# tsnuk/trade-AId-multimodal-transformer

Measured on AMD Instinct MI355X. Metric: training tokens/sec/GPU, 4-modality 1M-row synthetic, at 1/2/4/8 MI355X, higher is better.
Workload: dtype bf16; 1 GPU; C1: 4-modality 1M-row synthetic, d256 L6 T256 (BASELINE configs[1]); model=multimodal-transformer, global_batch=64, seq_len=256, n_embd=256, n_head=8, n_layer=6, modalities=4, parallelism=dp1

## Files before the change

### include/mmt.h

```cpp
#ifndef MMT_H_
#define MMT_H_
#include <stdint.h>

#ifdef __cplusplus
extern "C" {
#endif

#define MMT_MAX_MODALITIES 8

enum mmt_status {
  MMT_OK = 0,
  MMT_ERR_INVALID = -1,
  MMT_ERR_UNSUPPORTED = -2,
  MMT_ERR_HIP = -3,
  MMT_ERR_STATE = -4
};

typedef struct mmt_config {
  int32_t num_modalities;
  int32_t n_embd;
  int32_t n_head;
  int32_t n_layer;
  int32_t block_size;
  int32_t vocab_sizes[MMT_MAX_MODALITIES];
// ... 126 lines not shown
                    int32_t ldb, const float* bias, void* h1, int32_t ldh1, const float* w2, int32_t hh, void* out,
                    int32_t ld_out);
int mmt_op_gemm_wgrad(void* stream, int32_t M, int32_t N, int32_t K, const void* A, int32_t lda, const void* B,
                      int32_t ldb, float* out, int32_t ldc, float alpha, void* slab, int64_t slab_bytes);
int mmt_op_mlp2(void* stream, int32_t M, int32_t C, const void* x, int32_t ldx, const void* w0, int32_t ldw0,
                const float* b0, const void* w2, int32_t ldw2, const float* b2, void* h, int32_t ldh, const float* resid,
                float* out, void* out16, uint32_t drop_key, uint32_t drop_thr, float drop_scale, const float* lnf_gamma,
                const float* lnf_beta, void* lnf_y, float* lnf_mean, float* lnf_rstd);
int mmt_op_mlp2_bwd(void* stream, int32_t M, int32_t C, const void* dy, int32_t lddy, const void* w2, int32_t ldw2,
                    const void* h, int32_t ldh, float alpha, const void* w0, int32_t ldw0, void* dh, int32_t lddh,
                    float* db0, void* dx);
int mmt_op_layernorm_fwd(void* stream, int32_t R, int32_t C, const float* x, const float* gamma, const float* beta,
                         void* y16, float* mean, float* rstd);
int mmt_op_layernorm_bwd(void* stream, int32_t R, int32_t C, const float* x, const float* gamma, const float* mean,
                         const float* rstd, const float* dy, float* dx, void* dx16, float* dgamma, float* dbeta);
int mmt_op_gemm_ln_bwd(void* stream, int32_t M, int32_t N, int32_t K, const void* A, int32_t lda, const void* B,
                       int32_t ldb, float alpha, const float* x, const float* gamma, const float* mean,
                       const float* rstd, float* dx, void* dx16, float* dgamma, float* dbeta, float* dsum,
                       uint32_t drop_key, uint32_t drop_thr, float drop_scale);
int mmt_op_attention_fwd(void* stream, int32_t B, int32_t T, int32_t H, int32_t hs, int32_t nstreams,
                         const void* q, int32_t q_ld, const void* const* k, const void* const* v, int32_t kv_ld,
                         int32_t kv_hstride, void* o, int32_t o_ld, void* const* oj, float* const* lse);
int mmt_op_attention_bwd(void* stream, int32_t B, int32_t T, int32_t H, int32_t hs, int32_t nstreams,
                         const void* q, int32_t q_ld, const void* const* k, const void* const* v, int32_t kv_ld,
                         int32_t kv_hstride, const void* o, int32_t o_ld, const void* const* oj,
                         const float* const* lse, const void* dout, int32_t dout_ld, float* const* dvec, void* dq,
                         int32_t dq_ld, void* const* dk, void* const* dv, int32_t dkv_ld, int32_t dkv_hstride);
int mmt_op_attention_bwd_ws(void* stream, int32_t B, int32_t T, int32_t H, int32_t hs, int32_t nstreams,
                            const void* q, int32_t q_ld, const void* const* k, const void* const* v, int32_t kv_ld,
                            int32_t kv_hstride, const void* o, int32_t o_ld, const void* const* oj,
                            const float* const* lse, const void* dout, int32_t dout_ld, float* const* dvec, void* dq,
                            int32_t dq_ld, void* const* dk, void* const* dv, int32_t dkv_ld, int32_t dkv_hstride,
                            float* dq32, int32_t dq32_ld);
int mmt_op_qkv2_fwd(void* stream, int32_t R, int32_t nblk, int32_t hs, const void* h1, int32_t ld_h1,
                    const float* w2, void* out, int32_t ld_out);
int mmt_op_qkv2_bwd(void* stream, int32_t R, int32_t nblk, int32_t hs, const void* h1, int32_t ld_h1,
                    const float* w2, const void* dout, int32_t ld_out, void* dh1, float* dw2);
int mmt_op_colsum(void* stream, int32_t R, int32_t N, const void* x, int32_t ld, float* out, float alpha);
int mmt_op_ordered_sum(void* stream, int32_t nparts, int32_t n, const float* parts, int64_t ld, float* dst);
int mmt_op_cross_entropy(void* stream, int32_t R, int32_t V, const float* logits, const int64_t* tgt,
                         void* dlogits, int32_t ld_d, float* loss);
int mmt_op_embedding_fwd(void* stream, int32_t B, int32_t T, int32_t C, int32_t V, const int64_t* idx,
                         const float* tok, const float* pos, float* x);
int mmt_op_embedding_bwd(void* stream, int32_t B, int32_t T, int32_t C, int32_t V, const int64_t* idx,
                         const float* dx, float* dtok, float* dpos);
int mmt_op_embedding_bwd_ws(void* stream, int32_t B, int32_t T, int32_t C, int32_t V, const int64_t* idx,
                            const float* dx, float* dtok, float* dpos, float* scratch);
int mmt_emb_set_sort(int on);
int mmt_qkv2_set_coal(int on);
int mmt_set_relu_bits(int on);
int mmt_set_drop_copy_fuse(int on);
int mmt_set_attn_qkv2(int on);
int mmt_mlp2_set_bm(int bm);

int mmt_op_mx_quant(void* stream, int32_t rows, int32_t cols, const float* src, int32_t ld_src, void* dst8,
                    int32_t ld8, void* s8, int32_t lds8);
int mmt_op_gemm_f8(void* stream, int32_t epi, int32_t M, int32_t N, int32_t K, const void* A8, int32_t lda,
                   const void* sa, int32_t lds_a, const void* B8, int32_t ldb, const void* sb, int32_t lds_b,
                   const float* bias, const float* resid, int32_t ldres, float* o32, int32_t ldc, void* o16,
                   int32_t ldo16, void* o8, int32_t ld8, void* s8, int32_t lds8);
int mmt_op_layernorm_fwd_f8(void* stream, int32_t R, int32_t C, const float* x, const float* gamma, const float* beta,
                            void* y16, float* mean, float* rstd, void* y8, int32_t ld8, void* s8, int32_t lds8);

#ifdef __cplusplus
}
#endif
#endif
```

### trade-aid-multimodal-transformer_amd/csrc/mmt_attn.hip

```cpp
#include <stdlib.h>

#include <algorithm>

#include <type_traits>

#include "mmt_common.h"
#include "mmt_kernels.h"

namespace {

__device__ __forceinline__ bf16x8 zero8() {
  const u32x4 z = {0u, 0u, 0u, 0u};
  return __builtin_bit_cast(bf16x8, z);
}

__device__ __forceinline__ bf16x8 ld8(const bf16_t* p, bool ok) {
  if (!ok) return zero8();
  return *reinterpret_cast<const bf16x8*>(p);
}

template <int HS>
struct Geo {
  static constexpr int NKS = (HS + 15) / 16;
  static constexpr int ND = (HS + 31) / 32;
  static constexpr int W = ND * 32;
  static constexpr int RW = W + 8;
  static constexpr int TW = (W == 64) ? 96 : W;
  static constexpr int CH = HS / 8;
};

__device__ __forceinline__ u32x4 tile_chunk(const bf16_t* base, int64_t rowbase, int r0, int row, int col, int T,
                                            int ld) {
  u32x4 v = {0u, 0u, 0u, 0u};
  if (r0 + row < T) v = *reinterpret_cast<const u32x4*>(base + (rowbase + r0 + row) * ld + col);
  return v;
}

__device__ __forceinline__ bf16x8 tr_frag(const bf16_t* lds, int stride, int dt, int s, int lane) {
  const int g = lane >> 4, i = lane & 15;
  const int q = i >> 2, p = i & 3;
  const int col = dt * 32 + 16 * (g & 1) + 4 * p;
  const int kb = 16 * s + 4 * (g >> 1) + q;
  return join4(lds_tr16(lds + kb * stride + col), lds_tr16(lds + (kb + 8) * stride + col));
}

constexpr int SL_SUB = 1152, SL_SLICE = 2 * SL_SUB;
template <int HS>
struct SliceImg {
  static constexpr bool on = HS == 32;
};
__device__ __forceinline__ int sl_off(int row, int chunk) {
  return (row >> 5) * SL_SLICE + (chunk >> 1) * SL_SUB + (row & 31) * 32 + (((chunk & 1) ^ ((row >> 3) & 1)) << 4);
}
__device__ __forceinline__ bf16x8 sl_row(const bf16_t* img, int row0, int r, int s, int h) {
  const int o = (row0 >> 5) * SL_SLICE + s * SL_SUB + r * 32 + ((h ^ ((r >> 3) & 1)) << 4);
  return *reinterpret_cast<const bf16x8*>(reinterpret_cast<const char*>(img) + o);
}
__device__ __forceinline__ bf16x8 sl_tr(const bf16_t* img, int row0, int s, int lane) {
  const int g = lane >> 4, q = (lane >> 2) & 3, p = lane & 3;
  const int L = (g & 1) * SL_SUB + (p & 1) * 8 + (4 * (g >> 1) + q) * 32;
  const char* b = reinterpret_cast<const char*>(img) + (row0 >> 5) * SL_SLICE + 512 * s;
  return join4(lds_tr16(b + L + ((p >> 1) << 4)), lds_tr16(b + L + 256 + (((p >> 1) ^ 1) << 4)));
}

__device__ __forceinline__ bf16x8 acc_frag(const f32x16& a, int s) {
  const u32x4 v = {pack2bf(a[8 * s], a[8 * s + 1]), pack2bf(a[8 * s + 2], a[8 * s + 3]),
                   pack2bf(a[8 * s + 4], a[8 * s + 5]), pack2bf(a[8 * s + 6], a[8 * s + 7])};
  return __builtin_bit_cast(bf16x8, v);
}

__device__ __forceinline__ void zero16(f32x16& a) {
#pragma unroll
  for (int e = 0; e < 16; ++e) a[e] = 0.f;
}

__device__ __forceinline__ float keep_f(float v, int m) { return __int_as_float(__float_as_int(v) & m); }

__device__ __forceinline__ int key_dword(int r) { return 2 * ((r & 3) + 4 * (r >> 3)) + ((r >> 2) & 1); }

}

template <int HS>
struct Chunk {
  static constexpr int ROWS = (HS <= 32) ? 256 : 128;
  static constexpr int HALF = ROWS * Geo<HS>::CH;
  static constexpr int NSTG = 2 * HALF / 256;
};

template <int HS>
struct Stager {
  u32x4 v[Chunk<HS>::NSTG];
  __device__ __forceinline__ void load(const bf16_t* a, int lda, const bf16_t* b, int ldb, int64_t rowbase, int r0,
                                       int T, int tid) {
    constexpr int CH = Geo<HS>::CH, HALF = Chunk<HS>::HALF;
#pragma unroll
    for (int u = 0; u < Chunk<HS>::NSTG; ++u) {
      const int c = tid + 256 * u;
      const bool isb = c >= HALF;
      const int cc = isb ? c - HALF : c;
      v[u] = tile_chunk(isb ? b : a, rowbase, r0, cc / CH, (cc % CH) * 8, T, isb ? ldb : lda);
    }
  }
  __device__ __forceinline__ void store_a(bf16_t* la, int sa, int tid) const {
    constexpr int CH = Geo<HS>::CH, HALF = Chunk<HS>::HALF;
#pragma unroll
    for (int u = 0; u < Chunk<HS>::NSTG; ++u) {
      const int c = tid + 256 * u;
      if (c < HALF) *reinterpret_cast<u32x4*>(la + (c / CH) * sa + (c % CH) * 8) = v[u];
    }
  }
  __device__ __forceinline__ void store(bf16_t* la, int sa, bf16_t* lb, int sb, int tid) const {
    constexpr int CH = Geo<HS>::CH, HALF = Chunk<HS>::HALF;
#pragma unroll
    for (int u = 0; u < Chunk<HS>::NSTG; ++u) {
      const int c = tid + 256 * u;
      const bool isb = c >= HALF;
      const int cc = isb ? c - HALF : c;
      const int row = cc / CH, col = (cc % CH) * 8;
      *reinterpret_cast<u32x4*>(isb ? lb + row * sb + col : la + row * sa + col) = v[u];
    }
  }
  __device__ __forceinline__ void store_slices(bf16_t* la, bf16_t* lb, int tid) const {
    constexpr int CH = Geo<HS>::CH, HALF = Chunk<HS>::HALF;
    static_assert(CH == 4, "slice images hold 32 columns");
#pragma unroll
    for (int u = 0; u < Chunk<HS>::NSTG; ++u) {
      const int c = tid + 256 * u;
      const bool isb = c >= HALF;
      const int cc = isb ? c - HALF : c;
      *reinterpret_cast<u32x4*>(reinterpret_cast<char*>(isb ? lb : la) + sl_off(cc / CH, cc % CH)) = v[u];
    }
  }
};

template <int HS, int KT_ = Chunk<HS>::ROWS / 32>
struct MaskStager {
  static constexpr int KT = KT_;
  static constexpr int N4 = 8 * KT * 8;
  static constexpr int PER = (N4 + 255) / 256;
  static constexpr int DWORDS = 8 * KT * 32;
  u32x4 v[PER];
  __device__ __forceinline__ void load(const uint32_t* base, int bh, int nt, int b0, int c0, bool blk_q, int tid) {
    const int64_t ntri = (int64_t)nt * (nt + 1) / 2;
#pragma unroll
    for (int u = 0; u < PER; ++u) {
      const int c = tid + 256 * u;
      v[u] = u32x4{0u, 0u, 0u, 0u};
      if (N4 % 256 == 0 || c < N4) {
        const int i = c / (KT * 8), k = (c / 8) % KT, p = c % 8;
        const int qt = blk_q ? b0 + i : c0 + k, kt = blk_q ? c0 + k : b0 + i;
        if (qt < nt && kt <= qt)
          v[u] = *reinterpret_cast<const u32x4*>(base + ((int64_t)bh * ntri + qt * (qt + 1) / 2 + kt) * 32 + p * 4);
      }
    }
  }
  __device__ __forceinline__ void store(uint32_t* lds, int tid) const {
#pragma unroll
    for (int u = 0; u < PER; ++u) {
      const int c = tid + 256 * u;
      if (N4 % 256 == 0 || c < N4) *reinterpret_cast<u32x4*>(lds + 4 * c) = v[u];
    }
  }
};

__device__ __forceinline__ float ex2(float x) { return __builtin_amdgcn_exp2f(x); }


constexpr float kLog2e = 1.4426950408889634f;
constexpr float kTau = 8.0f;

#ifndef MMT_FWD_MINB
#define MMT_FWD_MINB(hs) 2
#endif
#ifndef MMT_DQ_MINB
#define MMT_DQ_MINB(hs) 2
#endif
#ifndef MMT_DKDV1_MINB
#define MMT_DKDV1_MINB(hs) ((hs) <= 32 ? 1 : 2)
#endif

__device__ __forceinline__ float xhalf_max(float v) {
  const auto r = __builtin_amdgcn_permlane32_swap(__float_as_uint(v), __float_as_uint(v), false, false);
  float m;
  asm("v_max_f32 %0, %1, %2" : "=v"(m) : "v"(__uint_as_float(r[0])), "v"(__uint_as_float(r[1])));
  return m;
}
__device__ __forceinline__ float xhalf_sum(float v) {
  const auto r = __builtin_amdgcn_permlane32_swap(__float_as_uint(v), __float_as_uint(v), false, false);
  return __uint_as_float(r[0]) + __uint_as_float(r[1]);
}

typedef short s16x2 __attribute__((ext_vector_type(2)));
__device__ __forceinline__ uint32_t keep_spread(uint32_t w16) { return __builtin_amdgcn_perm(0u, w16, 0x0c010c00u); }
__device__ __forceinline__ uint32_t pair_keep(uint32_t w32, int i) {
  s16x2 v = __builtin_bit_cast(s16x2, w32 << (15 - i));
  v = v >> (s16x2){15, 15};
  return __builtin_bit_cast(uint32_t, v);
}
__device__ __forceinline__ int elem_keep(uint32_t w16, int e) {
  return __builtin_amdgcn_sbfe((int)w16, (e & 1) * 8 + (e >> 1), 1);
}

__device__ __forceinline__ bf16x8 acc_frag_keep(const f32x16& a, int s, uint32_t w32) {
  const u32x4 v = {pack2bf(a[8 * s], a[8 * s + 1]) & pair_keep(w32, 4 * s),
                   pack2bf(a[8 * s + 2], a[8 * s + 3]) & pair_keep(w32, 4 * s + 1),
                   pack2bf(a[8 * s + 4], a[8 * s + 5]) & pair_keep(w32, 4 * s + 2),
                   pack2bf(a[8 * s + 6], a[8 * s + 7]) & pair_keep(w32, 4 * s + 3)};
  return __builtin_bit_cast(bf16x8, v);
}

template <int HS>
struct FwdQ {
  bf16x8 qf[Geo<HS>::NKS];
  f32x16 o[Geo<HS>::ND];
  float m, l;
  int tq;
};

template <int HS, bool diag>
__device__ __forceinline__ void fwd_softmax(f32x16& sacc, FwdQ<HS>& q, int k0, float c2, int h) {
  using G = Geo<HS>;
  float tmax = -INFINITY;
  if (diag) {
#pragma unroll
    for (int e = 0; e < 16; ++e) {
      const int key = k0 + (e & 3) + 8 * (e >> 2) + 4 * h;
      if (key > q.tq) sacc[e] = -INFINITY;
    }
  }
#pragma unroll
  for (int e = 0; e < 16; ++e) tmax = fmaxf(tmax, sacc[e]);
  tmax = xhalf_max(tmax) * c2;
  const bool up = tmax > q.m + kTau;
  if (__builtin_amdgcn_ballot_w64(up)) {
    const float alpha = up ? ex2(q.m - tmax) : 1.f;
    q.m = up ? tmax : q.m;
    q.l *= alpha;
#pragma unroll
    for (int dt = 0; dt < G::ND; ++dt)
#pragma unroll
      for (int e = 0; e < 16; ++e) q.o[dt][e] *= alpha;
  }
  const float nm = -q.m;
#pragma unroll
  for (int e = 0; e < 16; ++e) sacc[e] = ex2(__builtin_fmaf(sacc[e], c2, nm));
  float r0 = sacc[0] + sacc[1], r1 = sacc[2] + sacc[3], r2 = sacc[4] + sacc[5], r3 = sacc[6] + sacc[7];
  r0 += sacc[8] + sacc[9]; r1 += sacc[10] + sacc[11]; r2 += sacc[12] + sacc[13]; r3 += sacc[14] + sacc[15];
  q.l += (r0 + r1) + (r2 + r3);
}

template <int HS, int NQ, bool DA, bool DB, bool DROP>
__device__ __forceinline__ void fwd_step(const bf16_t* ks, const bf16_t* vs, int kl, int k0, FwdQ<HS>& a, FwdQ<HS>& b,
                                         const uint32_t* mta, const uint32_t* mtb, float c2, int lane) {
  using G = Geo<HS>;
  const int r = lane & 31, h = lane >> 5;
  const uint32_t wa = DROP ? keep_spread(reinterpret_cast<const uint16_t*>(mta)[lane]) : 0u;
  const uint32_t wb = (DROP && NQ == 2) ? keep_spread(reinterpret_cast<const uint16_t*>(mtb)[lane]) : 0u;
  f32x16 sa, sb;
  zero16(sa);
  if (NQ == 2) zero16(sb);
#pragma unroll
  for (int s = 0; s < G::NKS; ++s) {
    const bf16x8 kf = *reinterpret_cast<const bf16x8*>(ks + (kl + r) * G::RW + 16 * s + 8 * h);
    sa = mfma32(kf, a.qf[s], sa);
    if (NQ == 2) sb = mfma32(kf, b.qf[s], sb);
  }
  bf16x8 vf[2][G::ND];
#pragma unroll
  for (int s = 0; s < 2; ++s)
#pragma unroll
    for (int dt = 0; dt < G::ND; ++dt) vf[s][dt] = tr_frag(vs + kl * G::TW, G::TW, dt, s, lane);
  fwd_softmax<HS, DA>(sa, a, k0, c2, h);
  if (NQ == 2) fwd_softmax<HS, DB>(sb, b, k0, c2, h);
#pragma unroll
  for (int s = 0; s < 2; ++s) {
    const bf16x8 pa = DROP ? acc_frag_keep(sa, s, wa) : acc_frag(sa, s);
#pragma unroll
    for (int dt = 0; dt < G::ND; ++dt) a.o[dt] = mfma32(vf[s][dt], pa, a.o[dt]);
    if (NQ == 2) {
      const bf16x8 pb = DROP ? acc_frag_keep(sb, s, wb) : acc_frag(sb, s);
#pragma unroll
      for (int dt = 0; dt < G::ND; ++dt) b.o[dt] = mfma32(vf[s][dt], pb, b.o[dt]);
    }
  }
}

template <int HS, bool DROP>
__global__ __launch_bounds__(256, MMT_FWD_MINB(HS)) void attn_fwd_kernel(AttnBatch batch, int T, int H, float scale) {
  using G = Geo<HS>;
  constexpr int ROWS = Chunk<HS>::ROWS;
  constexpr int MKT = ROWS / 32;
  constexpr int MDW = 8 * MKT * 32;
  const AttnProblem& P = batch.p[blockIdx.z];
  const int nb = ((T + 31) / 32 + 7) / 8;
  const int tile = xcd_tile(blockIdx.x, gridDim.x);
  const int bh = tile / nb, b = bh / H, head = bh % H;
  const int bx = tile % nb;
  const int tid = threadIdx.x, lane = tid & 63, w = __builtin_amdgcn_readfirstlane(tid >> 6);
  const int r = lane & 31, h = lane >> 5;
  const int nt = (T + 31) / 32;
  const int qt0 = bx * 8;
  const int qmax = min(qt0 + 7, nt - 1);
  const int nch = (min((qmax + 1) * 32, T) + ROWS - 1) / ROWS;
  const int64_t rowbase = (int64_t)b * T;
  const float c2 = scale * kLog2e;
  __shared__ __attribute__((aligned(16))) bf16_t ks[ROWS * G::RW];
  __shared__ __attribute__((aligned(16))) bf16_t vs[ROWS * G::TW];
  using MS = MaskStager<HS>;
  __shared__ __attribute__((aligned(16))) uint32_t msk[DROP ? MDW : 4];
  const int BH = gridDim.x / nb;
  const int64_t lw_off = (int64_t)BH * (nt * (nt + 1) / 2) * 32;
  Stager<HS> st;
  MS mst;
  if (HS % 32 != 0) {
    for (int q = tid; q < ROWS * G::RW; q += 256) if (q % G::RW >= HS) ks[q] = 0;
    for (int q = tid; q < ROWS * G::TW; q += 256) if (q % G::TW >= HS) vs[q] = 0;
  }
  st.load(P.k[0] + head * P.kv_hstride, P.kv_ld, P.v[0] + head * P.kv_hstride, P.kv_ld, rowbase, 0, T, tid);
// ... 613 lines not shown
}
__device__ __forceinline__ void a_bst16(const ai32x4& rsrc, int voff, f32x4 v) {
  asm volatile("buffer_store_dwordx4 %0, %1, %2, 0 offen" : : "v"(v), "v"(voff), "s"(rsrc) : "memory");
}
__device__ __forceinline__ void a_wait_vm(int n) {
  switch (n) {
    case 0: asm volatile("s_waitcnt vmcnt(0)" ::: "memory"); break;
    case 1: asm volatile("s_waitcnt vmcnt(1)" ::: "memory"); break;
    case 2: asm volatile("s_waitcnt vmcnt(2)" ::: "memory"); break;
    case 3: asm volatile("s_waitcnt vmcnt(3)" ::: "memory"); break;
    case 4: asm volatile("s_waitcnt vmcnt(4)" ::: "memory"); break;
    case 5: asm volatile("s_waitcnt vmcnt(5)" ::: "memory"); break;
    case 6: asm volatile("s_waitcnt vmcnt(6)" ::: "memory"); break;
    case 7: asm volatile("s_waitcnt vmcnt(7)" ::: "memory"); break;
    default: asm volatile("s_waitcnt vmcnt(8)" ::: "memory"); break;
  }
}
constexpr int A_OOB = 0x7fffffff;
__device__ __forceinline__ float a_dpp(float v, int ctl) {
  return __builtin_bit_cast(float, ctl == 0xB1 ? __builtin_amdgcn_mov_dpp(__builtin_bit_cast(int, v), 0xB1, 0xF, 0xF, true)
                                  : ctl == 0x4E ? __builtin_amdgcn_mov_dpp(__builtin_bit_cast(int, v), 0x4E, 0xF, 0xF, true)
                                  : ctl == 0x124 ? __builtin_amdgcn_mov_dpp(__builtin_bit_cast(int, v), 0x124, 0xF, 0xF, true)
                                                 : __builtin_amdgcn_mov_dpp(__builtin_bit_cast(int, v), 0x128, 0xF, 0xF, true));
}
__device__ __forceinline__ float a_sum32(float v) {
  v += a_dpp(v, 0xB1);
  v += a_dpp(v, 0x4E);
  v += a_dpp(v, 0x124);
  v += a_dpp(v, 0x128);
  return v + __shfl_xor(v, 16, 64);
}
}

template <bool DROP, bool MS, bool Q2, bool DET = false>
__global__ __launch_bounds__(256, 2) void attn_bwd_fused32(AttnBatch batch, int T, int H, float scale) {
  static_assert(!(MS && Q2), "the stage-2 backward follows the self-attention only");
  static_assert(!DET || Q2, "only the stage-2 epilogue has sums to store");
  constexpr int IMG = 8 * SL_SLICE;
  constexpr int OFF_DO = IMG, OFF_TAB = 2 * IMG;
  constexpr int OFF_DS = OFF_TAB + 2048;
  constexpr int OFF_DQ = OFF_DS + 4 * 2048;
  constexpr int BYTES = OFF_DQ + 8 * 4096;
  static_assert(2 * BYTES <= 160 * 1024, "two workgroups per CU");
  constexpr int EPW = 40;
  static_assert(4 * 32 * EPW * 2 <= 4 * 4096, "epilogue transposes alias one parity of the dQ partials");
  __shared__ __attribute__((aligned(1024))) char lds[BYTES];
  const AttnProblem& P = batch.p[blockIdx.z];
  const int nt = (T + 31) / 32;
  const int bh = xcd_tile(blockIdx.x, gridDim.x);
  const int b = bh / H, head = bh % H;
  const int tid = threadIdx.x, lane = tid & 63, w = __builtin_amdgcn_readfirstlane(tid >> 6);
  const int r = lane & 31, h = lane >> 5;
  const int64_t rowbase = (int64_t)b * T;
  const float c2 = scale * kLog2e;
  const int kts[2] = {w, 7 - w};
  auto in_flight = [&](int qt) { return Q2 ? nt - 2 - qt : nt - 2; };

  const int64_t ntri = (int64_t)nt * (nt + 1) / 2;
  const int ns = MS ? P.nstreams : 1;
  const ai32x4 rdq32 = a_rsrc(MS ? P.dq32 + rowbase * P.dq32_ld + head * 32 : nullptr, MS ? (int64_t)T * P.dq32_ld * 4 : 0);
#pragma unroll 1
  for (int j = 0; j < ns; ++j) {
  const bf16_t* const oj = MS ? P.oj[j] : P.o;
  uint32_t mwq[2][8];
#pragma unroll
  for (int t = 0; t < 2; ++t)
#pragma unroll
    for (int q = 0; q < 8; ++q) {
      mwq[t][q] = 0u;
      if (DROP && q < nt && kts[t] <= q)
        mwq[t][q] = P.dmask[j][((int64_t)bh * ntri + q * (q + 1) / 2 + kts[t]) * 32 + key_dword(r)];
    }
  bf16x8 kf[2][2], vf[2][2];
#pragma unroll
  for (int t = 0; t < 2; ++t) {
    const int tk = kts[t] * 32 + r;
    const bool ok = kts[t] < nt && tk < T;
    const bf16_t* kp = P.k[j] + head * P.kv_hstride + (rowbase + tk) * P.kv_ld;
    const bf16_t* vp = P.v[j] + head * P.kv_hstride + (rowbase + tk) * P.kv_ld;
#pragma unroll
    for (int s = 0; s < 2; ++s) {
      kf[t][s] = ld8(kp + 16 * s + 8 * h, ok);
      vf[t][s] = ld8(vp + 16 * s + 8 * h, ok);
    }
  }
  float lse_t = 0.f;
  u32x4 ov[4], dv4[4];
  {
    const bool ok = tid < T;
    const int64_t t0 = ok ? tid : 0;
    lse_t = P.lse[j][(int64_t)bh * T + t0];
    const bf16_t* orow = oj + (rowbase + t0) * P.o_ld + head * 32;
    const bf16_t* drow = P.dout + (rowbase + t0) * P.dout_ld + head * 32;
#pragma unroll
    for (int c = 0; c < 4; ++c) {
      ov[c] = *reinterpret_cast<const u32x4*>(orow + 8 * c);
      dv4[c] = *reinterpret_cast<const u32x4*>(drow + 8 * c);
    }
  }
  bf16x8 w2t[3][2];
  const MMT_AS1 float* const w2p = Q2 ? sgpr_gptr(P.q2_w2) + head * 512 + (r & 15) + 8 * h * 16 : nullptr;
#pragma unroll
  for (int kd = 0; kd < 3; ++kd)
#pragma unroll
    for (int s = 0; s < 2; ++s) {
      float wv[8];
#pragma unroll
      for (int e = 0; e < 8; ++e) {
        wv[e] = Q2 ? w2p[(kd * H * 32 + 16 * s + e) * 16] : 0.f;
        wv[e] = r < 16 ? wv[e] : 0.f;
      }
      w2t[kd][s] = __builtin_bit_cast(bf16x8, u32x4{pack2bf(wv[0], wv[1]), pack2bf(wv[2], wv[3]), pack2bf(wv[4], wv[5]),
                                                   pack2bf(wv[6], wv[7])});
    }
#pragma unroll
  for (int t = 0; t < 2; ++t) {
#pragma unroll
    for (int q = 0; q < 8; ++q) asm volatile("" : "+v"(mwq[t][q]));
#pragma unroll
    for (int s = 0; s < 2; ++s) {
      asm volatile("" : "+v"(kf[t][s]));
      asm volatile("" : "+v"(vf[t][s]));
    }
  }
#pragma unroll
  for (int c = 0; c < 4; ++c) {
    asm volatile("" : "+v"(ov[c]));
    asm volatile("" : "+v"(dv4[c]));
  }
  asm volatile("" : "+v"(lse_t));
  if (Q2) {
#pragma unroll
    for (int kd = 0; kd < 3; ++kd) {
      asm volatile("" : "+v"(w2t[kd][0]));
      asm volatile("" : "+v"(w2t[kd][1]));
    }
  }
  asm volatile("s_waitcnt vmcnt(0)" ::: "memory");
  if (j == 0) {
    const int op = w & 1, cb = w >> 1;
    const int ld = op ? P.dout_ld : P.q_ld;
    const ai32x4 rs = a_rsrc((op ? P.dout : P.q) + rowbase * ld + head * 32, (int64_t)T * ld * 2);
    const int prow = lane >> 1, pcol = 8 * ((lane & 1) ^ ((prow >> 3) & 1));
    char* dst = lds + op * OFF_DO + cb * SL_SUB;
    for (int sl = 0; sl < nt; ++sl) {
      const int grow = sl * 32 + prow;
      const int voff = grow < T ? (grow * ld + cb * 16 + pcol) * 2 : A_OOB;
      a_dma16(rs, __builtin_amdgcn_readfirstlane(a_lds_u32(dst + sl * SL_SLICE)), voff);
    }
  }
  float* tab = reinterpret_cast<float*>(lds + OFF_TAB);
  {
    float dsum = 0.f;
#pragma unroll
    for (int c = 0; c < 4; ++c)
#pragma unroll
      for (int e = 0; e < 4; ++e) {
        dsum += bf2f(ov[c][e] & 0xffff) * bf2f(dv4[c][e] & 0xffff);
        dsum += bf2f(ov[c][e] >> 16) * bf2f(dv4[c][e] >> 16);
      }
    const bool ok = tid < T;
    tab[tid] = ok ? -lse_t : -INFINITY;
    tab[256 + tid] = ok ? (DROP ? -dsum / P.drop_scale : -dsum) : 0.f;
  }
  char* slot = lds + OFF_DS + w * 2048;
  const int g4 = lane >> 4, qq = (lane >> 2) & 3, p4 = lane & 3;
  const int ra0 = 4 * (g4 >> 1) + qq, ra1 = ra0 + 8;
  const int o_da0 = ra0 * 64 + (((4 * (g4 & 1) + p4) ^ ((ra0 >> 1) & 7)) << 3);
  const int o_da1 = ra1 * 64 + (((4 * (g4 & 1) + p4) ^ ((ra1 >> 1) & 7)) << 3);
  auto sw = [&](int c) { return r * 64 + ((c ^ ((r >> 1) & 7)) << 3); };
  bf16x8 ktf[2][2];
#pragma unroll
  for (int t = 0; t < 2; ++t) {
#pragma unroll
    for (int s = 0; s < 2; ++s) {
      const u32x4 v = __builtin_bit_cast(u32x4, kf[t][s]);
      *reinterpret_cast<u32x2*>(slot + sw(4 * s + 2 * h)) = u32x2{v[0], v[1]};
      *reinterpret_cast<u32x2*>(slot + sw(4 * s + 2 * h + 1)) = u32x2{v[2], v[3]};
    }
    asm volatile("s_waitcnt lgkmcnt(0)" ::: "memory");
#pragma unroll
// ... 290 lines not shown
      asm volatile("s_waitcnt lgkmcnt(0)" ::: "memory");
      bf16_t* dst = (mtx ? P.dv[j] : P.dk[j]) + head * P.dkv_hstride;
#pragma unroll
      for (int i = 0; i < 2; ++i) {
        const int row = i * 16 + (lane >> 2), d0 = (lane & 3) * 8;
        const u32x4 v = *reinterpret_cast<const u32x4*>(et + row * EPW + d0);
        if (k0 + row < T) *reinterpret_cast<u32x4*>(dst + (rowbase + k0 + row) * P.dkv_ld + d0) = v;
      }
    }
  }
  }
  }
}

static int g_attn_ring = mmt_env_int("MMT_ATTN_RING", 15 | 64);
extern "C" int mmt_attn_set_ring(int v) {
  const int old = g_attn_ring;
  g_attn_ring = v;
  return old;
}

static bool ring64_fits(const AttnBatch& bt, int T) {
  const int64_t lim = (int64_t)1 << 31;
  const int64_t nt = (T + 31) / 32, ntri = nt * (nt + 1) / 2;
  if (ntri * 128 >= lim) return false;
  for (int g = 0; g < bt.count; ++g) {
    const AttnProblem& P = bt.p[g];
    if ((int64_t)T * P.q_ld * 2 >= lim || (int64_t)T * P.dout_ld * 2 >= lim || (int64_t)T * P.kv_ld * 2 >= lim)
      return false;
  }
  return true;
}

static bool fused32_ok(const AttnBatch& bt, int T, int ns) {
  if (!(g_attn_ring & 64) || T > 256 || bt.count < 1) return false;
  const bool q2 = bt.p[0].q2_w2 != nullptr;
  if (q2 && ns > 1) return false;
  bool ok = true;
  for (int g = 0; g < bt.count; ++g) {
    const AttnProblem& P = bt.p[g];
    ok = ok && !(P.q_ld & 7) && !(P.dout_ld & 7) && !((uintptr_t)P.q & 15) && !((uintptr_t)P.dout & 15) &&
         !(P.kv_ld & 7) && !(P.kv_hstride & 7) && (int64_t)T * std::max(P.q_ld, P.dout_ld) * 2 < ((int64_t)1 << 31);
    if (ns > 1)
      ok = ok && (g_attn_ring & 128) && P.dq32 && !(P.dq32_ld & 3) && !((uintptr_t)P.dq32 & 15) &&
           (int64_t)T * P.dq32_ld * 4 < ((int64_t)1 << 31);
    if (ns == 1 && !q2) ok = ok && !(P.dq_ld & 3) && !((uintptr_t)P.dq & 7);
    if ((P.q2_w2 != nullptr) != q2) return false;
    if (q2)
      ok = ok && P.q2_h1 && P.q2_dh1 && P.q2_dw2 && P.q2_db1 && !(P.q2_ld & 7) && !((uintptr_t)P.q2_h1 & 15) &&
           !((uintptr_t)P.q2_dh1 & 7);
  }
  return ok;
}

bool mmt_attn_bwd_fuses_qkv2(const AttnBatch& bt, int T, int hs) {
  if (hs != 32 || bt.count < 1) return false;
  for (int g = 0; g < bt.count; ++g)
    if (bt.p[g].nstreams != 1) return false;
  AttnBatch t = bt;
  for (int g = 0; g < t.count; ++g) {
    AttnProblem& P = t.p[g];
    P.q2_w2 = reinterpret_cast<const float*>(16); P.q2_h1 = reinterpret_cast<const bf16_t*>(16);
    P.q2_dh1 = reinterpret_cast<bf16_t*>(16); P.q2_dw2 = reinterpret_cast<float*>(16); P.q2_db1 = P.q2_dw2;
    P.q2_ld = 8;
  }
  return fused32_ok(t, T, 1);
}

int64_t mmt_attn_q2_det_floats(int count, int B, int H) { return (int64_t)count * B * 3 * H * (512 + 16); }

template <int HS>
static hipError_t attn_launch(const AttnBatch& bt, int B, int T, int H, float scale, bool bwd, hipStream_t s) {
  const int nb = ((T + 31) / 32 + 7) / 8;
  if (!bwd) {
    bool drop = false;
    for (int g = 0; g < bt.count; ++g) drop = drop || bt.p[g].drop_thr != 0;
    if (HS == 64 && (g_attn_ring & 8) && ring64_fits(bt, T)) return mmt_attn_fwd_ring64(bt, B, T, H, scale, drop, s);
    const dim3 grid(nb * B * H, 1, bt.count);
    if (drop) hipLaunchKernelGGL((attn_fwd_kernel<HS, true>), grid, dim3(256), 0, s, bt, T, H, scale);
    else hipLaunchKernelGGL((attn_fwd_kernel<HS, false>), grid, dim3(256), 0, s, bt, T, H, scale);
  } else {
    const int ns = bt.p[0].nstreams;
    bool drop = false;
    for (int g = 0; g < bt.count; ++g) drop = drop || bt.p[g].drop_thr != 0;
    for (int g = 0; g < bt.count; ++g)
      if (bt.p[g].q2_w2 && (HS != 32 || !fused32_ok(bt, T, ns))) return hipErrorInvalidValue;
    const bool ring = HS == 64 && ring64_fits(bt, T);
    if (ring && (g_attn_ring & 32) && T <= 512 && ns == 1) return mmt_attn_bwd_fused64(bt, B, T, H, scale, drop, s);
    if (HS == 32 && fused32_ok(bt, T, ns)) {
      const dim3 grid(B * H, 1, bt.count);
      const bool q2 = bt.p[0].q2_w2 != nullptr;
      if (ns > 1) {
        if (drop) hipLaunchKernelGGL((attn_bwd_fused32<true, true, false>), grid, dim3(256), 0, s, bt, T, H, scale);
        else hipLaunchKernelGGL((attn_bwd_fused32<false, true, false>), grid, dim3(256), 0, s, bt, T, H, scale);
      } else if (q2 && bt.det.base) {
        AttnBatch d = bt;
        d.det.stride = mmt_attn_q2_det_floats(1, B, H);
        DetLaunch L;
        hipError_t e = L.begin(d.det, d.count, d.det.stride, s);
        if (e != hipSuccess) return e;
        if (drop) hipLaunchKernelGGL((attn_bwd_fused32<true, false, true, true>), grid, dim3(256), 0, s, d, T, H, scale);
        else hipLaunchKernelGGL((attn_bwd_fused32<false, false, true, true>), grid, dim3(256), 0, s, d, T, H, scale);
        e = hipGetLastError();
        if (e != hipSuccess) return e;
        for (int g = 0; g < d.count; ++g) {
          L.seg(g, d.det.stride, 0, d.p[g].q2_dw2, B, 3 * H * 512);
          L.seg(g, d.det.stride, (int64_t)B * 3 * H * 512, d.p[g].q2_db1, B, 3 * H * 16);
        }
        return L.finish();
      } else if (q2) {
        if (drop) hipLaunchKernelGGL((attn_bwd_fused32<true, false, true>), grid, dim3(256), 0, s, bt, T, H, scale);
        else hipLaunchKernelGGL((attn_bwd_fused32<false, false, true>), grid, dim3(256), 0, s, bt, T, H, scale);
      } else {
        if (drop) hipLaunchKernelGGL((attn_bwd_fused32<true, false, false>), grid, dim3(256), 0, s, bt, T, H, scale);
        else hipLaunchKernelGGL((attn_bwd_fused32<false, false, false>), grid, dim3(256), 0, s, bt, T, H, scale);
      }
      return hipGetLastError();
    }
    if (ring && (g_attn_ring & 2)) {
      const hipError_t e = mmt_attn_bwd_dq_ring64(bt, B, T, H, scale, drop, s);
      if (e != hipSuccess) return e;
    } else if (drop) hipLaunchKernelGGL((attn_bwd_dq_kernel<HS, true>), dim3(nb * B * H, 1, bt.count), dim3(256), 0, s, bt, T, H, scale);
    else hipLaunchKernelGGL((attn_bwd_dq_kernel<HS, false>), dim3(nb * B * H, 1, bt.count), dim3(256), 0, s, bt, T, H, scale);
    if (ring && (g_attn_ring & 1)) return mmt_attn_bwd_dkdv_ring64(bt, B, T, H, scale, drop, g_attn_ring, s);
    if (drop)
      hipLaunchKernelGGL((attn_bwd_dkdv1_kernel<HS, true>), dim3(nb * B * H * ns, 1, bt.count), dim3(256), 0, s, bt, T, H,
                         scale);
    else
      hipLaunchKernelGGL((attn_bwd_dkdv1_kernel<HS, false>), dim3(nb * B * H * ns, 1, bt.count), dim3(256), 0, s, bt, T,
                         H, scale);
  }
  return hipGetLastError();
}

static hipError_t attn_dispatch(const AttnBatch& b, int B, int T, int H, int hs, float scale, bool bwd,
                                hipStream_t s) {
  if (b.count == 0 || B == 0 || T == 0) return hipSuccess;
  for (int g = 0; g < b.count; ++g) {
    if (b.p[g].nstreams < 1 || b.p[g].nstreams > MMT_MAX_STREAMS) return hipErrorInvalidValue;
    for (int j = 0; j < b.p[g].nstreams && b.p[g].nstreams > 1; ++j)
      if (!b.p[g].oj[j]) return hipErrorInvalidValue;
    if (b.p[g].drop_thr)
      for (int j = 0; j < b.p[g].nstreams; ++j)
        if (!b.p[g].dmask[j]) return hipErrorInvalidValue;
// ... 143 lines not shown
```

### trade-aid-multimodal-transformer_amd/csrc/mmt_engine.hip

```cpp
#include <hip/hip_runtime.h>

#include <algorithm>
#include <cmath>
#include <cstdio>
#include <cstdlib>
#include <cstring>
#include <string>
#include <vector>

#include "mmt.h"
#include "mmt_common.h"
#include "mmt_kernels.h"

namespace {

constexpr int MAXM = MMT_MAX_MODALITIES;

inline int64_t rup(int64_t x, int64_t a) { return (x + a - 1) / a * a; }
inline int r8(int x) { return (int)rup(x < 1 ? 1 : x, 8); }

struct Mat {
  int64_t off = -1;
  int rows = 0, cols = 0;
  int64_t pk = 0;
// ... 50 lines not shown
  size_t dvec[MAXM][MAXM];
  size_t dkv[2][MAXM][MAXM];
  size_t celoss[MAXM];
  const void* gh1_pad_ws = nullptr;
  size_t eperm[MAXM];
  size_t det = 0;
  int64_t det_floats = 0;
  struct Dec {
    size_t x0, a16, mean, rstd, h1, qkv, o16, p1, f, x2h, d16, qc, oc, pc, lnf16, hh;
    size_t kv[MAXM];
  } dec[MAXM];
  std::vector<size_t> dec_x;
};

}

static int g_relu_bits = mmt_env_int("MMT_RELU_BITS", 0);
extern "C" int mmt_set_relu_bits(int on) {
  const int old = g_relu_bits;
  g_relu_bits = on;
  return old;
}
static int g_drop_copy_fuse = mmt_env_int("MMT_DROP_COPY_FUSE", 1);
extern "C" int mmt_set_drop_copy_fuse(int on) {
  const int old = g_drop_copy_fuse;
  g_drop_copy_fuse = on;
  return old;
}

static int g_attn_qkv2 = mmt_env_int("MMT_ATTN_QKV2", 1);
extern "C" int mmt_set_attn_qkv2(int on) {
  const int old = g_attn_qkv2;
  g_attn_qkv2 = on;
  return old;
}

struct mmt_ctx {
  mmt_config cfg;
  int M, C, H, L, T, hs, hh;
  int V[MAXM];
  bool any_cross = false;
  int ncross = 0;
  std::vector<TensorInfo> tensors;
  std::vector<LM> lm;
  PostM post[MAXM];
  int64_t pos_off = 0;
  int64_t nparams = 0, nactive = 0;
  int64_t emb_begin = 0, emb_end = 0, post_begin = 0, post_end = 0;
  std::vector<int64_t> layer_begin, layer_end;
  std::vector<PackSeg> segs;
  std::vector<int> tasks;
  std::vector<MxSeg> mxsegs;
  int64_t pack8_bytes = 0;
  int mx_units = 0;
  MxSeg* d_mxsegs = nullptr;
  int tables_device = -1;
  bool fp8 = false;
  bool relu_bits = false;
  hipEvent_t emb_ev = nullptr;
  bool emb_sorted = false;
  int64_t pack_elems = 0;
  PackSeg* d_segs = nullptr;
  int* d_tasks = nullptr;
  Plan plan;
  int last_B = -1;
  bool fwd_ready = false;
  bool cache_ready = false;
  bool last_training = false;
  uint64_t step_counter = 0;
  uint64_t next_seed = 0;
  bool next_seed_set = false;
  uint64_t fwd_seed = 0;
  bool fwd_drop = false;
  const int64_t* last_idx[MAXM] = {};
  std::string err;
  struct ProbeEv {
    hipEvent_t a, b;
    int pat;
    double flops, bytes;
  };
  std::vector<std::string> probe_pats;
  bool probe_on = true;
  std::vector<ProbeEv> probe_events;
  std::vector<std::pair<hipEvent_t, hipEvent_t>> probe_pool;
  int ldv[MAXM], ldvh[MAXM];
  hipStream_t side = nullptr;
  int side_device = -1;
  bool side_off = false;
  bool side_off_req = false;
  bool defer_join = false;
  hipEvent_t stage_ev[2] = {nullptr, nullptr};
  std::vector<hipEvent_t> evpool;
  size_t evnext = 0;
  int d16 = 0;
  bool det = false;
  bool det_req = false;
  bool grad_accum = false;
};

namespace {

thread_local std::string g_create_err;

int fail(mmt_ctx* c, int code, const std::string& msg) {
  if (c) c->err = msg;
  return code;
}

#define HIPCHK(ctx, expr)                                                                             \
  do {                                                                                                \
    hipError_t e_ = (expr);                                                                           \
    if (e_ != hipSuccess) return fail(ctx, MMT_ERR_HIP, std::string(#expr) + ": " + hipGetErrorString(e_)); \
  } while (0)

struct Builder {
  mmt_ctx* c;
  int64_t cur = 0;
  int64_t alloc(int64_t n) {
    const int64_t o = cur;
    cur += rup(n > 0 ? n : 0, 16);
    return o;
  }
  void tensor(const std::string& name, int64_t off, int nd, int64_t s0, int64_t s1, int kind) {
    TensorInfo t;
    t.name = name; t.off = off; t.nd = nd; t.shape[0] = s0; t.shape[1] = s1; t.kind = kind;
    c->tensors.push_back(t);
  }
  Mat mat(const std::string& name, int rows, int cols, bool emit = true) {
    Mat m;
    m.rows = rows; m.cols = cols;
// ... 305 lines not shown
      if (std::strncmp(what, p.c_str(), p.size() - 1) == 0) return (int)i;
    } else if (p == what) {
      return (int)i;
    }
  }
  return -1;
}
int probe_match(const mmt_ctx* c, const char* what) {
  std::string w(what);
  size_t b = 0;
  while (true) {
    const size_t e = w.find('+', b);
    const int r = probe_match_one(c, w.substr(b, e == std::string::npos ? std::string::npos : e - b).c_str());
    if (r >= 0 || e == std::string::npos) return r;
    b = e + 1;
  }
}

void gemm_cost(const GemmBatch& b, int epi, double* fl, double* by) {
  for (int g = 0; g < b.count; ++g) {
    const GemmProblem& P = b.p[g];
    const double M = P.M, N = P.N, K = P.K;
    *fl += 2.0 * M * N * K;
    double x = (M * K + N * K) * 2.0;
    if (P.bias) x += N * 4.0;
    const bool f32_out = epi == EPI_BIAS_RESID_F32 || epi == EPI_STORE_F32 || epi == EPI_ACC_F32;
    x += M * N * (f32_out ? 4.0 : 2.0);
    if (epi == EPI_BIAS_RESID_F32) x += M * N * 4.0 + (P.o16 ? M * N * 2.0 : 0.0);
    if (epi == EPI_ACC_F32) x += M * N * 4.0;
    if (epi == EPI_DTANH_BF16 || epi == EPI_DRELU_BF16) x += (epi == EPI_DRELU_BF16 && P.mask8) ? M * N / 8.0 : M * N * 2.0;
    if (epi == EPI_BIAS_RELU_BF16 && P.mask8) x += M * N / 8.0;
    if (P.o8) x += M * N * (1.0 + 1.0 / 32.0);
    if (epi == EPI_LN_BWD_F32) x += M * N * 8.0 + (P.o16 ? M * N * 2.0 : 0.0) + M * 8.0;
    *by += x;
  }
}

void wgrad_cost(const GemmBatch& b, double* fl, double* by) {
  for (int g = 0; g < b.count; ++g) {
    const GemmProblem& P = b.p[g];
    const double M = P.M, N = P.N, K = P.K;
    *fl += 2.0 * M * N * K;
    *by += (M * K + N * K) * 2.0 + M * N * 4.0;
  }
}

void attn_cost(const AttnBatch& ab, int B, int T, int H, int hs, bool bwd, bool drop, double* fl, double* by) {
  const double C = (double)H * hs, rows = (double)B * T, bhT = (double)B * H * T;
  const double mask = drop ? (double)mmt_attn_mask_dwords(B, H, T) * 4.0 : 0.0;
  for (int g = 0; g < ab.count; ++g) {
    const double ns = ab.p[g].nstreams;
    const double f = 2.0 * (double)B * H * ns * (double)T * T * hs;
    *fl += bwd ? 2.5 * f : f;
    double x = rows * C * 2.0 * (2.0 + 2.0 * ns) + ns * (bhT * 4.0 + mask);
    if (ns > 1) x += ns * rows * C * 2.0;
    if (bwd) x += rows * C * 2.0 * (2.0 + 2.0 * ns) + ns * bhT * 4.0;
    if (bwd && ab.p[g].q2_w2) {
      const double hh = hs / 2;
      x += -rows * C * 2.0 * 3.0 + 2.0 * rows * 3.0 * H * hh * 2.0 + 3.0 * H * hs * hh * 4.0 * 2.0;
      *fl += 2.0 * 2.0 * rows * 3.0 * C * hh;
    }
    *by += x;
  }
}

GemmProblem gp_f8(const uint8_t* X8, int ldx, const uint8_t* Xs, int ldxs, const uint8_t* w8, const Mat& W, int R) {
  GemmProblem g{};
  g.A = reinterpret_cast<const bf16_t*>(X8); g.lda = ldx; g.sa = Xs; g.lds_a = ldxs;
  g.B = reinterpret_cast<const bf16_t*>(w8 + W.pk8); g.ldb = W.ld8; g.sb = w8 + W.ps8; g.lds_b = W.lds8;
  g.M = R; g.N = W.rows; g.K = W.cols; g.alpha = 1.f;
  return g;
}

enum DropSite { DS_SA_PROB = 0, DS_SA_PROJ = 1, DS_FFN = 2, DS_CA_PROB = 3, DS_CA_PROJ = 4 };

struct Runner {
  mmt_ctx* c;
  hipStream_t s;
  void* ws;
  const float* params;
  const bf16_t* wpk;
  int B, R;
  int rc = MMT_OK;
  bool drop = false;
  uint64_t seed = 0;

  template <class Pm>
  void set_drop(Pm& p, int l, int i, int site) const {
    if (!drop) { p.drop_key = 0; p.drop_thr = 0; p.drop_scale = 1.f; return; }
    const double pr = c->cfg.dropout;
    p.drop_key = mmt_hash((uint32_t)seed, (uint32_t)(seed >> 32), (uint32_t)((l * MAXM + i) * 8 + site));
    p.drop_thr = (uint32_t)std::min(65535.0, std::max(1.0, std::floor(pr * 65536.0)));
    p.drop_scale = (float)(1.0 / (1.0 - pr));
// ... 284 lines not shown
      eb.p[i].idx = idx[i]; eb.p[i].tok = r.P(c->post[i].tok); eb.p[i].pos = r.P(c->pos_off);
      eb.p[i].x = r.W<float>(p.xemb[i]); eb.p[i].V = c->V[i];
    }
    r.ok(mmt_launch_embed_fwd(eb, B, T, C, r.s), "embed_fwd");
  }
  std::vector<const float*> xin(M);
  for (int i = 0; i < M; ++i) xin[i] = r.W<float>(p.xemb[i]);
  static const int ln_fuse = mmt_env_int("MMT_LN_FUSE", 1) != 0 ? mmt_env_int("MMT_LN_FUSE_FWD", 1) : 0;
  const bool fuse_fwd = ln_fuse && !f8 && (C == 256 || (C == 512 && ln_fuse == 2));
  std::vector<char> ln1_done(M, 0), lnf_done(M, 0);
  for (int l = 0; l < c->L && r.rc == MMT_OK; ++l) {
    const LM* x = &c->lm[(size_t)l * M];
    const ActLM* a = &p.act[(size_t)l * M];
    if (r.drop && l == 0) gen_masks(0);
    LnBatch lb{}; lb.count = 0;
    for (int i = 0; i < M; ++i) {
      if (ln1_done[i]) continue;
      LnProblem& q = lb.p[lb.count++];
      q.x = xin[i]; q.gamma = r.P(x[i].ln1w); q.beta = r.P(x[i].ln1b);
      q.y = r.W<bf16_t>(a[i].a); q.mean = r.W<float>(a[i].mean1); q.rstd = r.W<float>(a[i].rstd1);
      ln8(q, a[i].a8, a[i].as8);
    }
    if (lb.count) r.ok(mmt_launch_ln_fwd(lb, R, C, r.s), "ln1_fwd");
    std::fill(ln1_done.begin(), ln1_done.end(), 0);
    lb.count = M;
    GemmBatch g{}; g.count = M;
    static const bool qkv2_fuse = mmt_env_int("MMT_QKV2_FUSE", 1) != 0;
    for (int i = 0; i < M; ++i) {
      g.p[i] = f8 ? gp_f8(r.W<uint8_t>(a[i].a8), C, r.W<uint8_t>(a[i].as8), ldsC, w8, x[i].W1, R)
                  : gp_fwd(r.W<bf16_t>(a[i].a), C, wpk, x[i].W1, R);
      g.p[i].bias = r.P(x[i].b1); g.p[i].o16 = r.W<bf16_t>(a[i].h1); g.p[i].ldo16 = ldh1;
    }
    const bool fuse_qkv2 = qkv2_fuse && (c->hh == 16 || c->hh == 32) && !f8 && !mmt_gemm_wgrad_big(g);
    for (int i = 0; i < M; ++i) {
      if (fuse_qkv2) {
        g.p[i].qkv2_w2 = r.P(x[i].w2); g.p[i].qkv2_out = r.W<bf16_t>(a[i].qkv);
        g.p[i].qkv2_ld = 3 * C; g.p[i].qkv2_hh = c->hh;
      }
    }
    if (f8) r.gemm8(g, EPI_BIAS_TANH_BF16, "qkv1");
    else r.gemm(g, true, true, EPI_BIAS_TANH_BF16, 1, "qkv1");
    for (int i = 0; i < M; ++i) g.p[i].qkv2_out = nullptr;
    if (!fuse_qkv2) {
      Qkv2Batch qb{}; qb.count = M;
      for (int i = 0; i < M; ++i) {
        qb.p[i].h1 = r.W<bf16_t>(a[i].h1); qb.p[i].w2 = r.P(x[i].w2); qb.p[i].out = r.W<bf16_t>(a[i].qkv);
      }
      r.ok(mmt_launch_qkv2_fwd(qb, R, 3 * H, hs, ldh1, 3 * C, r.s), "qkv2_fwd");
    }
    AttnBatch ab{}; ab.count = M;
    for (int i = 0; i < M; ++i) {
      AttnProblem& q = ab.p[i];
      bf16_t* qkv = r.W<bf16_t>(a[i].qkv);
      q.q = qkv + C; q.q_ld = 3 * C; q.k[0] = qkv; q.v[0] = qkv + 2 * C; q.kv_ld = 3 * C; q.kv_hstride = hs;
      q.o = r.W<bf16_t>(a[i].o); q.o_ld = C; q.lse[0] = r.W<float>(a[i].lse); q.nstreams = 1;
      r.set_drop(q, l, i, DS_SA_PROB);
      if (r.drop) q.dmask[0] = r.W<uint32_t>(a[i].dm);
    }
    if (r.drop && (l <= 1 || mask_ahead)) {
      r.join();
      r.gemm_hint = 0;
      if (mask_ahead) {
        if (ahead_mode == 1 && l + 1 < c->L) gen_masks(l + 1);
      } else if (l == 0) {
        for (int ll = 1; ll < c->L; ++ll) gen_masks(ll);
        if (mask_t2) r.gemm_hint = 1;
      }
    }
    r.attn(ab, false, scale, "attn_fwd");
    if (r.drop && ahead_mode == 2 && l + 1 < c->L) {
      gen_masks(l + 1);
      if (mask_t2) r.gemm_hint = 1;
    }
    static const bool ln2_env = mmt_env_int("MMT_LN2_FUSE", 1) != 0;
    const bool ln2_fuse = ln2_env && !f8;
    bool ln2_done = false;
    {
      GemmProblem pg1[MAXM], pg2[MAXM];
      for (int i = 0; i < M; ++i) {
        GemmProblem& g1 = pg1[i];
        g1 = gp_fwd(r.W<bf16_t>(a[i].o), C, wpk, x[i].P0, R);
        g1.bias = r.P(x[i].bp0); g1.o16 = r.W<bf16_t>(a[i].p1); g1.ldo16 = ldp;
        GemmProblem& g2 = pg2[i];
        g2 = gp_fwd(r.W<bf16_t>(a[i].p1), ldp, wpk, x[i].P2, R);
        g2.bias = r.P(x[i].bp2); g2.resid = xin[i]; g2.ldres = C;
        g2.o32 = r.W<float>(a[i].x1); g2.ldc = C;
        r.set_drop(g2, l, i, DS_SA_PROJ);
        if (ln2_fuse) {
          g2.lnf_gamma = r.P(x[i].ln2w); g2.lnf_beta = r.P(x[i].ln2b); g2.lnf_y = r.W<bf16_t>(a[i].c);
          g2.lnf_mean = r.W<float>(a[i].mean2); g2.lnf_rstd = r.W<float>(a[i].rstd2);
// ... 594 lines not shown
      const bf16_t* g = r.W<bf16_t>(p.gp[par][i]);
      pdx0[i] = gp_dx(g, ldp, wpk, x[i].P0, R);
      pdx0[i].o16 = r.W<bf16_t>(p.gdo[i]); pdx0[i].ldo16 = C;
    }
    const bool fused = r.mlp2(dx.p, pdx0, M, "proj_dx", true);
    if (!fused) r.gemm(dx, true, false, EPI_DTANH_BF16, 1, "proj2_dx");
    for (int i = 0; i < M; ++i) {
      const bf16_t* g = r.W<bf16_t>(p.gp[par][i]);
      dw.p[i] = gp_dw(g, ldp, r.W<bf16_t>(a[i].o), C, grads, x[i].P0, R);
      dx.p[i] = pdx0[i];
    }
    r.dwgemm(dw, "proj0_dw");
    if (!fused) r.gemm(dx, true, false, EPI_STORE_BF16, 1, "proj0_dx");
  }
  r.flush();
  AttnBatch ab{}; ab.count = M;
  for (int i = 0; i < M; ++i) {
    AttnProblem& q = ab.p[i];
    bf16_t* qkv = r.W<bf16_t>(a[i].qkv);
    bf16_t* gq = r.W<bf16_t>(p.gqkv[i]);
    q.q = qkv + C; q.q_ld = 3 * C; q.k[0] = qkv; q.v[0] = qkv + 2 * C; q.kv_ld = 3 * C; q.kv_hstride = hs;
    q.o = r.W<bf16_t>(a[i].o); q.o_ld = C; q.lse[0] = r.W<float>(a[i].lse); q.nstreams = 1;
    q.dout = r.W<bf16_t>(p.gdo[i]); q.dout_ld = C; q.dvec[0] = r.W<float>(p.dvec[i][0]);
    q.dq = gq + C; q.dq_ld = 3 * C; q.dk[0] = gq; q.dv[0] = gq + 2 * C; q.dkv_ld = 3 * C; q.dkv_hstride = hs;
    r.set_drop(q, l, i, DS_SA_PROB);
    if (r.drop) q.dmask[0] = r.W<uint32_t>(a[i].dm);
  }
  const bool q2 = g_attn_qkv2 && mmt_attn_bwd_fuses_qkv2(ab, T, hs);
  if (q2)
    for (int i = 0; i < M; ++i) {
      AttnProblem& q = ab.p[i];
      q.q2_h1 = r.W<bf16_t>(a[i].h1); q.q2_dh1 = r.W<bf16_t>(p.gh1[par][i]); q.q2_ld = ldh1;
      q.q2_w2 = r.P(x[i].w2); q.q2_dw2 = grads + x[i].w2; q.q2_db1 = grads + x[i].b1;
    }
  Qkv2Batch qb{}; qb.count = M;
  for (int i = 0; i < M; ++i) {
    qb.p[i].h1 = r.W<bf16_t>(a[i].h1); qb.p[i].w2 = r.P(x[i].w2); qb.p[i].dout = r.W<bf16_t>(p.gqkv[i]);
    qb.p[i].dh1 = r.W<bf16_t>(p.gh1[par][i]); qb.p[i].dw2 = grads + x[i].w2;
    qb.p[i].db1 = grads + x[i].b1;
  }
  if (p.gh1_pad_ws != r.ws && ldh1 > 3 * H * c->hh) {
    const size_t cols = 3 * (size_t)H * c->hh;
    for (int k = 0; k < 2; ++k)
      for (int i = 0; i < M; ++i)
        r.ok(hipMemset2DAsync(r.W<bf16_t>(p.gh1[k][i]) + cols, (size_t)ldh1 * 2, 0, ((size_t)ldh1 - cols) * 2, (size_t)R, r.s),
             "gh1 pad");
    p.gh1_pad_ws = r.ws;
  }
  r.attn(ab, true, scale, "attn_bwd");
  r.det_arm(qb);
  if (!q2) r.ok(mmt_launch_qkv2_bwd(qb, R, 3 * H, hs, ldh1, 3 * C, r.s), "qkv2_bwd");
  for (int i = 0; i < M; ++i) {
    const bf16_t* g = r.W<bf16_t>(p.gh1[par][i]);
    dw.p[i] = gp_dw(g, ldh1, r.W<bf16_t>(a[i].a), C, grads, x[i].W1, R);
    dx.p[i] = gp_dx(g, ldh1, wpk, x[i].W1, R);
    dx.p[i].o32 = r.W<float>(p.dln[i]); dx.p[i].ldc = C;
  }
  r.dwgemm(dw, "qkv1_dw");
  r.flush();
  d16_advance(c);
  for (int i = 0; i < M; ++i) {
    lb.p[i].x = xin[i]; lb.p[i].gamma = r.P(x[i].ln1w); lb.p[i].mean = r.W<float>(a[i].mean1);
    lb.p[i].rstd = r.W<float>(a[i].rstd1); lb.p[i].dy = r.W<float>(p.dln[i]); lb.p[i].dx = r.W<float>(p.dres[i]);
    lb.p[i].dgamma = grads + x[i].ln1w; lb.p[i].dbeta = grads + x[i].ln1b;
    set_dres16_consumer(c, r, lb.p[i], i, l - 1, grads);
  }
  r.gemm_ln_bwd(dx, lb, R, C, "qkv1_dx", "ln1_bwd");
// ... 132 lines not shown
    std::strncpy(name, t.name.c_str(), cap - 1);
    name[cap - 1] = 0;
  }
  if (off) *off = t.off;
  if (nd) *nd = t.nd;
  if (shape) { shape[0] = t.shape[0]; shape[1] = t.shape[1]; }
  if (kind) *kind = t.kind;
  return MMT_OK;
}

int64_t mmt_loss_flag_offset(mmt_ctx* c, int32_t batch) {
  if (!c || batch < 1) return -1;
  return (int64_t)flag_offset(c);
}

int64_t mmt_workspace_bytes(mmt_ctx* c, int32_t batch) {
  if (!c || batch < 1) return -1;
  make_plan(c, batch);
  c->last_B = batch;
  c->fwd_ready = false;
  c->cache_ready = false;
  return (int64_t)c->plan.total;
}

int mmt_forward(mmt_ctx* c, void* stream, int32_t batch, const int64_t* const* idx, const int64_t* const* tgt,
                const float* params, float* const* logits, float* losses, void* workspace, int32_t training) {
  if (!c) return MMT_ERR_INVALID;
  if (batch < 1 || !idx || !params || !logits || !workspace) return fail(c, MMT_ERR_INVALID, "mmt_forward: null argument");
  if (c->plan.B != batch) make_plan(c, batch);
  int rc = ensure_device_tables(c);
  if (rc) return rc;
  c->side_off = c->side_off_req;
  c->det = c->det_req;
  Runner r{c, (hipStream_t)stream, workspace, params, nullptr, batch, batch * c->T};
  r.drop = training && c->cfg.dropout > 0.f;
  if (r.drop) {
    if (c->next_seed_set) r.seed = c->next_seed;
    else r.seed = ((uint64_t)mmt_hash((uint32_t)c->cfg.seed, (uint32_t)(c->cfg.seed >> 32), (uint32_t)c->step_counter) << 32) |
                  mmt_hash((uint32_t)(c->cfg.seed >> 32), (uint32_t)c->cfg.seed, (uint32_t)(c->step_counter >> 32) ^ 0xA5A5A5A5u);
    c->next_seed_set = false;
    ++c->step_counter;
  }
  if (r.drop) ensure_side(c);
  c->fwd_drop = r.drop;
  c->fwd_seed = r.seed;
  c->fwd_ready = false;
  for (int i = 0; i < c->M; ++i) c->last_idx[i] = idx[i];
  rc = run_forward(c, r, idx, tgt, logits, losses);
  if (rc == MMT_OK && tgt) c->fwd_ready = true;
  c->cache_ready = rc == MMT_OK;
  c->last_training = training != 0;
  return rc;
}

int mmt_decode_step(mmt_ctx* c, void* stream, int32_t batch, int32_t pos, const int64_t* const* idx,
                    const float* params, float* const* logits, void* workspace) {
  if (!c) return MMT_ERR_INVALID;
  if (!idx || !params || !logits || !workspace) return fail(c, MMT_ERR_INVALID, "mmt_decode_step: null argument");
  if (c->plan.B != batch || !c->cache_ready)
    return fail(c, MMT_ERR_STATE, "mmt_decode_step: run mmt_forward (prefill) on this batch and workspace first");
  if (c->fwd_drop)
    return fail(c, MMT_ERR_STATE, "mmt_decode_step: the prefill forward sampled dropout (training mode); decode "
                                  "has eval semantics: run the prefill with training = 0");
  if (c->fp8)
    return fail(c, MMT_ERR_STATE, "mmt_decode_step: precision fp8 prefills with MX-fp8 GEMMs the bf16 decode "
                                  "would not reproduce: re-run mmt_forward per token");
  if (pos < 1 || pos >= c->T) return fail(c, MMT_ERR_INVALID, "mmt_decode_step: position outside 1..block_size-1");
  Runner r{c, (hipStream_t)stream, workspace, params, nullptr, batch, batch};
  return run_decode(c, r, pos, idx, logits);
}

int32_t mmt_backward_stage_count(const mmt_ctx* c) { return c ? c->L + 2 : 0; }

int mmt_backward_stage_range(const mmt_ctx* c, int32_t stage, int64_t* begin, int64_t* end) {
  if (!c || stage < 0 || stage > c->L + 1) return MMT_ERR_INVALID;
  int64_t b, e;
  if (stage == 0) { b = c->post_begin; e = c->post_end; }
  else if (stage == c->L + 1) { b = c->emb_begin; e = c->emb_end; }
  else { const int l = c->L - stage; b = c->layer_begin[l]; e = c->layer_end[l]; }
  if (begin) *begin = b;
  if (end) *end = e;
  return MMT_OK;
}

}

extern "C" {

int mmt_backward_stage(mmt_ctx* c, void* stream, int32_t stage, const float* loss_grads, const float* params,
                       float* grads, void* workspace) {
  if (!c) return MMT_ERR_INVALID;
  if (!c->fwd_ready) return fail(c, MMT_ERR_STATE, "mmt_backward: no forward with targets to differentiate");
  if (stage < 0 || stage > c->L + 1) return fail(c, MMT_ERR_INVALID, "bad backward stage");
// ... 195 lines not shown
```

### trade-aid-multimodal-transformer_amd/csrc/mmt_gemm.hip

```cpp
#include "mmt_common.h"
#include "mmt_kernels.h"

#include <stdlib.h>

#include <algorithm>
#include <type_traits>

#include "mmt_gemm_dev.h"


static int g_gemm_variant = -1;

static int g_gemm_big_variant_rt = 0;
static int g_force_big_rt = 0;
static int g_gemm8_rt = -1;
static int g_gemm_variant_dw = 0;
extern "C" int mmt_gemm_set_variant(int v) {
  if (v < 0) {
    g_gemm_variant = -1; g_gemm_variant_dw = 0; g_gemm_big_variant_rt = 0; g_force_big_rt = 0; g_gemm8_rt = -1;
    return 0;
  }
  if ((v & 15) > 6 || ((v >> 4) & 15) > 6 || ((v >> 8) & 15) > 3) return -1;
  g_gemm_variant = v & 15;
  g_gemm_variant_dw = (v >> 4) & 15;
// ... 146 lines not shown
  }
  if (tile >= ntiles) return;
  GEMM_STAMP(0);
  GEMM_STAMP(5);
  GEMM_STAMP(6);
  const int tm = tile / tiles_n, tn = tile % tiles_n;
  const int m0 = tm * GBM, n0 = tn * GBN;
  const int ksteps = (K + BK - 1) / BK;
  const int kper = (ksteps + nsplit - 1) / nsplit;
  const int ks0 = split * kper;
  const int ks1 = min(ksteps, ks0 + kper);
  if (EPI == EPI_ATOMIC_F32 && ks0 >= ks1) return;

  constexpr int EPI_ROWS = (GBN >= 512 || (GBM == 128 && GBN == 256)) ? 32 : (GBM == 128 && MINB == 1) ? 128 : 64;
  constexpr int RING = ST * STAGE_BYTES, CTILE = EPI_ROWS * (GBN + 4) * 4;
  constexpr int LDS_MAIN = RING > CTILE ? RING : CTILE;
  constexpr int LDS_W2 = (SWAP && EPI == EPI_BIAS_TANH_BF16 && TL::NW == 4 && TL::BN == 128) ? QKV2_W2_LDS : 0;
  __shared__ __attribute__((aligned(1024))) char lds[LDS_MAIN + LDS_W2];

  const int tid = threadIdx.x;
  const int lane = tid & 63;
  const int wave = __builtin_amdgcn_readfirstlane(tid >> 6);
  const int wm = wave / TL::WN, wn = wave % TL::WN;

  f32x16 acc[AI][AJ];
#pragma unroll
  for (int i = 0; i < AI; ++i)
#pragma unroll
    for (int j = 0; j < AJ; ++j)
#pragma unroll
      for (int e = 0; e < 16; ++e) acc[i][j][e] = 0.0f;
  if constexpr (SWAP && EPI == EPI_BIAS_TANH_BF16 && TL::NW == 4 && TL::BN == 128) {
    if (P.qkv2_out) qkv2_stage_w2<TL>(P, lds + LDS_MAIN, n0, tid);
    if (P.qkv2_out && P.bias) {
      const float ia = 1.0f / P.alpha;
      const int hh = (tid & 63) >> 5;
#pragma unroll
      for (int i = 0; i < AI; ++i)
#pragma unroll
        for (int e = 0; e < 16; ++e) {
          const int n = n0 + wn * TL::TN * 32 + 32 * i + (e & 3) + 8 * (e >> 2) + 4 * hh;
          const float bv = n < N ? P.bias[n] * ia : 0.0f;
#pragma unroll
          for (int j = 0; j < AJ; ++j) acc[i][j][e] = bv;
        }
    }
  }

  if (ks0 < ks1) {
    const int lda = __builtin_amdgcn_readfirstlane(P.lda), ldb = __builtin_amdgcn_readfirstlane(P.ldb);
    auto sgpr_ptr = [](const bf16_t* q) {
      const uint64_t v = (uint64_t)(uintptr_t)q;
      const uint32_t lo = __builtin_amdgcn_readfirstlane((uint32_t)v), hi = __builtin_amdgcn_readfirstlane((uint32_t)(v >> 32));
      return (const bf16_t*)(uintptr_t)(((uint64_t)hi << 32) | lo);
    };
    const bf16_t* const Ap = sgpr_ptr(P.A);
    const bf16_t* const Bp = sgpr_ptr(P.B);
    const i32x4 ra_kc = A_KC ? op_rsrc<true>(Ap, lda, M, K, m0, 0) : i32x4{0, 0, 0, 0};
    const i32x4 rb_kc = B_KC ? op_rsrc<true>(Bp, ldb, N, K, n0, 0) : i32x4{0, 0, 0, 0};
    auto ra = [&](int k0) { return A_KC ? ra_kc : op_rsrc<false>(Ap, lda, M, K, m0, k0); };
    auto rb = [&](int k0) { return B_KC ? rb_kc : op_rsrc<false>(Bp, ldb, N, K, n0, k0); };
    const int nk = ks1 - ks0;
    auto step = [&](int tt, auto UC) {
      constexpr int U = decltype(UC)::value;
      wait_vm(PIECES * min(ST - 2, nk - 1 - tt));
      asm volatile("s_waitcnt lgkmcnt(0)" ::: "memory");
      __builtin_amdgcn_s_barrier();
// ... 22 lines not shown
          }
      }
    };
#pragma unroll
    for (int t = 0; t < ST - 1; ++t)
      if (t < nk) {
        char* st = lds + t * STAGE_BYTES;
        const int k0 = (ks0 + t) * BK;
        issue_tile<BK, A_KC, GBM, NW>(ra(k0), st, lda, M, K, m0, k0, wave, lane);
        issue_tile<BK, B_KC, GBN, NW>(rb(k0), st + IMG_A, ldb, N, K, n0, k0, wave, lane);
      }
    GEMM_STAMP(1);
    int t = 0;
    for (; t + ST <= nk; t += ST) {
      step(t, std::integral_constant<int, 0>{});
      step(t + 1, std::integral_constant<int, 1>{});
      if constexpr (ST > 2) step(t + 2, std::integral_constant<int, (ST > 2 ? 2 : 0)>{});
      if constexpr (ST > 3) step(t + 3, std::integral_constant<int, (ST > 3 ? 3 : 0)>{});
    }
    if (t < nk) step(t, std::integral_constant<int, 0>{});
    if (ST > 2 && t + 1 < nk) step(t + 1, std::integral_constant<int, 1>{});
    if constexpr (ST > 3) { if (t + 2 < nk) step(t + 2, std::integral_constant<int, (ST > 3 ? 2 : 0)>{}); }
  }

  GEMM_STAMP(3);
  float alpha = P.alpha;
  if (P.alpha_ptr) alpha *= *P.alpha_ptr;
  float* o32 = P.o32 + (P.split_stride ? (int64_t)split * P.split_stride : (int64_t)0);
  const int h = lane >> 5, r = lane & 31;
  if constexpr (SWAP && EPI == EPI_BIAS_TANH_BF16 && TL::NW == 4 && TL::BN == 128) {
    if (P.qkv2_out) {
      qkv2_fused<TL>(P, acc, lds, lds + LDS_MAIN, alpha, m0, n0, lane, wave);
      epilogue_swap<TL, EPI, EPI_ROWS, true>(P, acc, lds, o32, alpha, m0, n0, tid, lane, wave, det_of(batch, prob));
    } else {
      epilogue_swap<TL, EPI, EPI_ROWS>(P, acc, lds, o32, alpha, m0, n0, tid, lane, wave, det_of(batch, prob));
    }
  } else if constexpr (SWAP) {
    epilogue_swap<TL, EPI, EPI_ROWS>(P, acc, lds, o32, alpha, m0, n0, tid, lane, wave, det_of(batch, prob));
  } else {
#pragma unroll
    for (int i = 0; i < TM; ++i)
#pragma unroll
      for (int j = 0; j < TN; ++j) {
        const int n = n0 + wn * TN * 32 + 32 * j + r;
        if (n >= N) continue;
#pragma unroll
        for (int e = 0; e < 16; ++e) {
          const int m = m0 + wm * TM * 32 + 32 * i + (e & 3) + 8 * (e >> 2) + 4 * h;
          if (m < M) epi_scalar<EPI>(P, o32, alpha, m, n, acc[i][j][e]);
        }
      }
  }
  GEMM_STAMP(4);
}

template <int ROWS, int NW>
__device__ __forceinline__ void issue_tile_f8(const i32x4& rsrc, char* img, int ld, int rows_total, int K, int r0,
                                              int k0, int wave, int lane) {
  constexpr int PPW = ROWS * 128 / 1024 / NW;
#pragma unroll
  for (int u = 0; u < PPW; ++u) {
    const int i = wave * PPW + u;
    const int row = 8 * i + lane / 8;
    const int chunk = kc_swz<64>(lane % 8, row);
    const int grow = r0 + row, gk = k0 + chunk * 16;
    const int voff = (grow < rows_total && gk < K) ? row * ld + gk : 0x7fffffff;
// ... 222 lines not shown
  }
  const int mt = max_tiles<TileS>(b, nullptr);
  if (mt == 0) return hipSuccess;
  dim3 grid(mt, EPI == EPI_ATOMIC_F32 ? auto_splits<TileS>(b, splits) : std::max(1, splits), b.count);
  constexpr bool occ3 = EPI == EPI_STORE_BF16 || EPI == EPI_BIAS_TANH_BF16 || EPI == EPI_BIAS_RELU_BF16;
  static const int env_dw = mmt_env_int("MMT_GEMM_DW_VARIANT", -1);
  const int var = EPI == EPI_ATOMIC_F32 ? g_gemm_variant_dw
                  : (!A_KC && !B_KC && env_dw >= 0) ? env_dw
                  : (g_gemm_variant >= 0 ? g_gemm_variant : occ3 ? MMT_OCC3_VARIANT : MMT_DEF_VARIANT);
  switch (var) {
    case 1: launch_v<TileS, 32, 2, A_KC, B_KC, SWAP, EPI>(b, grid, s); break;
    case 2: launch_v<TileS, 32, 3, A_KC, B_KC, SWAP, EPI>(b, grid, s); break;
    case 3: launch_v<TileS, 32, 4, A_KC, B_KC, SWAP, EPI>(b, grid, s); break;
    case 4: launch_v<TileS, 64, 3, A_KC, B_KC, SWAP, EPI>(b, grid, s); break;
    case 5: launch_v<TileS, 32, 3, A_KC, B_KC, SWAP, EPI, 3>(b, grid, s); break;
    case 6: launch_v<TileS, 32, 2, A_KC, B_KC, SWAP, EPI, 3>(b, grid, s); break;
    default: launch_v<TileS, 64, 2, A_KC, B_KC, SWAP, EPI>(b, grid, s); break;
  }
  return hipGetLastError();
}

static int g_big_mode = mmt_env_int("MMT_GEMM_BIG", 1);

static int g_gemm8_kmin = mmt_env_int("MMT_GEMM8_KMIN", 512);
static int g_gemm8_min_tiles = mmt_env_int("MMT_GEMM8_MIN_TILES", 1024);
static bool use_big(const GemmBatch& b) {
  if (!g_big_mode || b.count == 0) return false;
  bool big = true, qkv2 = false;
  int tiles = 0;
  for (int g = 0; g < b.count; ++g) {
    const GemmProblem& P = b.p[g];
    if (P.M < TileL::BM || P.N < TileL::BN) return false;
    if (P.K < g_big_kmin && !g_force_big_rt) big = false;
    qkv2 = qkv2 || P.qkv2_out != nullptr;
    tiles += ((P.M + 255) / 256) * ((P.N + 255) / 256);
  }
  if (big) return true;
  if (!gemm8_on() || qkv2 || tiles < g_gemm8_min_tiles) return false;
  for (int g = 0; g < b.count; ++g)
    if (b.p[g].K < g_gemm8_kmin) return false;
  return true;
}

static bool qkv2_ok(const GemmProblem& P, int epi, bool fwd) {
  if (!P.qkv2_out) return true;
  return epi == EPI_BIAS_TANH_BF16 && fwd && (P.qkv2_hh == 16 || P.qkv2_hh == 32) && P.N % P.qkv2_hh == 0 &&
         !P.alpha_ptr && P.alpha != 0.0f &&
         P.qkv2_w2 && !(P.qkv2_ld & 7) && !((uintptr_t)P.qkv2_out & 15) && !((uintptr_t)P.qkv2_w2 & 15);
}

static bool gemm_span_ok(const GemmBatch& b) {
  for (int g = 0; g < b.count; ++g) {
    const GemmProblem& P = b.p[g];
    if (P.M < 0 || P.N < 0 || P.K < 0 || P.lda < 0 || P.ldb < 0) return false;
    if ((int64_t)(512 + 1) * std::max(P.lda, P.ldb) * 2 + (int64_t)P.K * 2 >= ((int64_t)1 << 31)) return false;
  }
  return true;
}

static int64_t gemm_det_stride(const GemmBatch& b, bool ln) {
  int64_t st = 0;
  for (int g = 0; g < b.count; ++g) {
    const int64_t nrt = (b.p[g].M + MMT_DET_GEMM_ROWS - 1) / MMT_DET_GEMM_ROWS;
    st = std::max(st, (ln ? 3 : 1) * nrt * (int64_t)b.p[g].N);
  }
  return (st + 3) & ~(int64_t)3;
}
int64_t mmt_gemm_det_floats(int count, int M, int N, bool ln) {
  GemmBatch b{};
  b.count = 1; b.p[0].M = M; b.p[0].N = N;
  return count * gemm_det_stride(b, ln);
}
template <class F>
static hipError_t gemm_det_run(const GemmBatch& b, bool ln, hipStream_t s, F run) {
  bool any = false;
  for (int g = 0; g < b.count; ++g) any = any || b.p[g].dbias || (ln && (b.p[g].ln_dgamma || b.p[g].ln_dbeta));
  GemmBatch d = b;
  if (!any) {
// ... 4 lines not shown
  DetLaunch L;
  hipError_t e = L.begin(d.det, b.count, d.det.stride, s);
  if (e != hipSuccess) return e;
  e = run(d);
  if (e != hipSuccess) return e;
  for (int g = 0; g < b.count; ++g) {
    const GemmProblem& P = b.p[g];
    const int nrt = (P.M + MMT_DET_GEMM_ROWS - 1) / MMT_DET_GEMM_ROWS;
    const int64_t slot = (int64_t)nrt * P.N;
    L.seg(g, d.det.stride, 0, P.dbias, nrt, P.N);
    if (ln) {
      L.seg(g, d.det.stride, slot, P.ln_dgamma, nrt, P.N);
      L.seg(g, d.det.stride, 2 * slot, P.ln_dbeta, nrt, P.N);
    }
  }
  return L.finish();
}

static hipError_t launch_gemm_any(const GemmBatch& b, bool a_kc, bool b_kc, int epi, int splits, hipStream_t s);
hipError_t mmt_launch_gemm(const GemmBatch& b, bool a_kc, bool b_kc, int epi, int splits, hipStream_t s) {
  if (!b.det.base) return launch_gemm_any(b, a_kc, b_kc, epi, splits, s);
  return gemm_det_run(b, false, s, [&](const GemmBatch& d) { return launch_gemm_any(d, a_kc, b_kc, epi, splits, s); });
}

static hipError_t launch_gemm_any(const GemmBatch& b, bool a_kc, bool b_kc, int epi, int splits, hipStream_t s) {
  if (!gemm_span_ok(b)) return hipErrorInvalidValue;
  for (int g = 0; g < b.count; ++g) {
    const GemmProblem& P = b.p[g];
    if ((P.lda & 7) || (P.ldb & 7) || (((uintptr_t)P.A | (uintptr_t)P.B) & 15)) return hipErrorInvalidValue;
    if (!qkv2_ok(P, epi, a_kc && b_kc)) return hipErrorInvalidValue;
  }
  const bool big = use_big(b);
  for (int g = 0; g < b.count; ++g)
    if (big && b.p[g].qkv2_out) return hipErrorInvalidValue;
  if (a_kc && b_kc) {
    switch (epi) {
      case EPI_STORE_BF16: return launch_t<true, true, true, EPI_STORE_BF16>(b, 1, big, s);
      case EPI_BIAS_TANH_BF16: return launch_t<true, true, true, EPI_BIAS_TANH_BF16>(b, 1, big, s);
      case EPI_BIAS_RELU_BF16: return launch_t<true, true, true, EPI_BIAS_RELU_BF16>(b, 1, big, s);
      case EPI_BIAS_RESID_F32: return launch_t<true, true, true, EPI_BIAS_RESID_F32>(b, 1, big, s);
      case EPI_STORE_F32: return launch_t<true, true, true, EPI_STORE_F32>(b, 1, big, s);
      case EPI_ACC_F32: return launch_t<true, true, true, EPI_ACC_F32>(b, 1, big, s);
      default: break;
    }
  } else if (a_kc && !b_kc) {
    switch (epi) {
      case EPI_STORE_BF16: return launch_t<true, false, true, EPI_STORE_BF16>(b, 1, big, s);
      case EPI_DTANH_BF16: return launch_t<true, false, true, EPI_DTANH_BF16>(b, 1, big, s);
      case EPI_DRELU_BF16: return launch_t<true, false, true, EPI_DRELU_BF16>(b, 1, big, s);
      case EPI_STORE_F32: return launch_t<true, false, true, EPI_STORE_F32>(b, 1, big, s);
      case EPI_ACC_F32: return launch_t<true, false, true, EPI_ACC_F32>(b, 1, big, s);
      default: break;
    }
  } else if (!a_kc && !b_kc) {
    switch (epi) {
      case EPI_ATOMIC_F32: return launch_t<false, false, false, EPI_ATOMIC_F32>(b, splits, big, s);
      case EPI_STORE_F32: return launch_t<false, false, true, EPI_STORE_F32>(b, splits, big, s);
      case EPI_ACC_F32: return launch_t<false, false, true, EPI_ACC_F32>(b, 1, big, s);
      default: break;
    }
  } else {
    switch (epi) {
      case EPI_ATOMIC_F32: return launch_t<false, true, false, EPI_ATOMIC_F32>(b, splits, big, s);
      case EPI_STORE_F32: return launch_t<false, true, true, EPI_STORE_F32>(b, 1, big, s);
      default: break;
    }
  }
// ... 164 lines not shown
    if (gemm8_ln_on()) return mmt_launch_gemm8(b, EPI_LN_BWD_F32, true, false, dim3(mt, 1, b.count), s);
    launch_v<TileL, 64, 2, true, false, true, EPI_LN_BWD_F32>(b, dim3(mt, 1, b.count), s);
  }
  return hipGetLastError();
}

template <class TL, int EPI>
static hipError_t launch_f8(const GemmBatch& b, hipStream_t s) {
  int mt = 0;
  for (int g = 0; g < b.count; ++g)
    mt = std::max(mt, ((b.p[g].M + TL::BM - 1) / TL::BM) * ((b.p[g].N + TL::BN - 1) / TL::BN));
  if (mt == 0) return hipSuccess;
  hipLaunchKernelGGL((gemm_f8_kernel<TL, EPI>), dim3(mt, 1, b.count), dim3(TL::NT), 0, s, b);
  return hipGetLastError();
}

template <int EPI>
static hipError_t launch_f8_tile(const GemmBatch& b, hipStream_t s) {
  bool big = g_big_mode != 0 && b.tile_hint != 1;
  for (int g = 0; g < b.count; ++g)
    if (b.p[g].M < TileL::BM || b.p[g].N < TileL::BN || b.p[g].K < g_big_kmin) big = false;
  return big ? launch_f8<TileL, EPI>(b, s) : launch_f8<TileS, EPI>(b, s);
}

hipError_t mmt_launch_gemm_f8(const GemmBatch& b, int epi, hipStream_t s) {
  if (b.count == 0) return hipSuccess;
  if (!gemm_span_ok(b)) return hipErrorInvalidValue;
  for (int g = 0; g < b.count; ++g) {
    const GemmProblem& P = b.p[g];
    if ((P.K & 31) || (P.lda & 15) || (P.ldb & 15) || (((uintptr_t)P.A | (uintptr_t)P.B) & 15) || (P.lds_a & 3) ||
        (P.lds_b & 3) || (((uintptr_t)P.sa | (uintptr_t)P.sb) & 3) || P.lds_a * 32 < P.K || P.lds_b * 32 < P.K)
      return hipErrorInvalidValue;
    if (P.o8 && ((P.N & 31) || (P.ld8 & 7) || ((uintptr_t)P.o8 & 7))) return hipErrorInvalidValue;
    if (P.qkv2_out) return hipErrorInvalidValue;
  }
  switch (epi) {
    case EPI_STORE_BF16: return launch_f8_tile<EPI_STORE_BF16>(b, s);
    case EPI_BIAS_TANH_BF16: return launch_f8_tile<EPI_BIAS_TANH_BF16>(b, s);
    case EPI_BIAS_RELU_BF16: return launch_f8_tile<EPI_BIAS_RELU_BF16>(b, s);
    case EPI_BIAS_RESID_F32: return launch_f8_tile<EPI_BIAS_RESID_F32>(b, s);
    case EPI_STORE_F32: return launch_f8_tile<EPI_STORE_F32>(b, s);
    default: return hipErrorInvalidValue;
  }
}
```

### trade-aid-multimodal-transformer_amd/csrc/mmt_kernels.h

```cpp
#pragma once
#include <hip/hip_runtime.h>
#include <stdint.h>
#include "mmt_det.h"

#ifndef MMT_MAX_GROUP
#define MMT_MAX_GROUP 8
#endif
typedef uint16_t bf16_t;

enum MmtEpi {
  EPI_STORE_BF16 = 0,
  EPI_BIAS_TANH_BF16,
  EPI_BIAS_RELU_BF16,
  EPI_BIAS_RESID_F32,
  EPI_STORE_F32,
  EPI_DTANH_BF16,
  EPI_DRELU_BF16,
  EPI_ACC_F32,
  EPI_ATOMIC_F32,
  EPI_LN_BWD_F32,
  EPI_COUNT
};

struct GemmProblem {
// ... 1 lines not shown
  const bf16_t* B;
  const float* bias;
  const bf16_t* aux;
  const float* resid;
  float* o32;
  bf16_t* o16;
  const float* alpha_ptr;
  float alpha;
  int M, N, K;
  int lda, ldb, ldc, ldaux, ldres, ldo16;
  uint32_t drop_key, drop_thr;
  float drop_scale;
  float* dbias;
  int64_t split_stride;
  const uint8_t* sa;
  const uint8_t* sb;
  int lds_a, lds_b;
  uint8_t* o8;
  uint8_t* s8;
  int ld8, lds8;
  const float* ln_gamma;
  const float* ln_mean;
  const float* ln_rstd;
  float* ln_dgamma;
  float* ln_dbeta;
  const float* lnf_gamma;
  const float* lnf_beta;
  bf16_t* lnf_y;
  float* lnf_mean;
  float* lnf_rstd;
  const float* qkv2_w2;
  bf16_t* qkv2_out;
  int qkv2_ld, qkv2_hh;
  uint8_t* mask8;
  int ldm8;
};

struct GemmBatch {
  GemmProblem p[MMT_MAX_GROUP];
  int count;
  int xcd_plane;
  int tile_hint;
  int dw_blocks;
  unsigned long long* stamps;
  DetScratch det;
};

hipError_t mmt_launch_gemm(const GemmBatch& b, bool a_kc, bool b_kc, int epi, int splits, hipStream_t s);
bool mmt_gemm_ln_bwd_ok(const GemmBatch& b);
bool mmt_gemm_resid_ln_ok(const GemmBatch& b);
hipError_t mmt_launch_gemm_resid_ln(const GemmBatch& b, hipStream_t s);
hipError_t mmt_launch_gemm_ln_bwd(const GemmBatch& b, hipStream_t s);
hipError_t mmt_launch_gemm_wgrad(const GemmBatch& b, float* slab, int64_t slab_bytes, hipStream_t s);

#define MMT_MLP2_GROUP 4
struct Mlp2Batch {
  GemmProblem g1[MMT_MLP2_GROUP];
  GemmProblem g2[MMT_MLP2_GROUP];
  int count;
  DetScratch det;
};
static_assert(sizeof(Mlp2Batch) <= 4096, "Mlp2Batch is a kernel argument");
bool mmt_mlp2_ok(const Mlp2Batch& b);
hipError_t mmt_launch_mlp2(const Mlp2Batch& b, hipStream_t s);
bool mmt_mlp2_bwd_ok(const Mlp2Batch& b);
hipError_t mmt_launch_mlp2_bwd(const Mlp2Batch& b, hipStream_t s);
// ... 21 lines not shown
};
struct LnBatch {
  LnProblem p[MMT_MAX_GROUP];
  int count;
  float* zero_f; int nzero_f;
  int* zero_i; int nzero_i;
  DetScratch det;
};
hipError_t mmt_launch_ln_fwd(const LnBatch& b, int R, int C, hipStream_t s);
hipError_t mmt_launch_ln_bwd(const LnBatch& b, int R, int C, hipStream_t s);

#define MMT_MAX_STREAMS 8
struct AttnProblem {
  const bf16_t* q; int q_ld;
  const bf16_t* k[MMT_MAX_STREAMS];
  const bf16_t* v[MMT_MAX_STREAMS];
  int kv_ld, kv_hstride;
  bf16_t* o; int o_ld;
  bf16_t* oj[MMT_MAX_STREAMS];
  float* lse[MMT_MAX_STREAMS];
  const bf16_t* dout; int dout_ld;
  float* dvec[MMT_MAX_STREAMS];
  bf16_t* dq; int dq_ld;
  float* dq32; int dq32_ld;
  const bf16_t* q2_h1; bf16_t* q2_dh1; int q2_ld;
  const float* q2_w2; float* q2_dw2; float* q2_db1;
  bf16_t* dk[MMT_MAX_STREAMS];
  bf16_t* dv[MMT_MAX_STREAMS];
  int dkv_ld, dkv_hstride;
  int nstreams;
  uint32_t drop_key, drop_thr;
  float drop_scale;
  uint32_t* dmask[MMT_MAX_STREAMS];
};
inline int64_t mmt_attn_mask_tiles(int B, int H, int T) {
  const int64_t nt = (T + 31) / 32;
  return (int64_t)B * H * (nt * (nt + 1) / 2);
}
inline int64_t mmt_attn_mask_dwords(int B, int H, int T) { return 2 * 32 * mmt_attn_mask_tiles(B, H, T); }
struct AttnBatch {
  AttnProblem p[MMT_MAX_GROUP];
  int count;
  DetScratch det;
};
hipError_t mmt_launch_attn_fwd(const AttnBatch& b, int B, int T, int H, int hs, float scale, hipStream_t s);
hipError_t mmt_launch_attn_bwd(const AttnBatch& b, int B, int T, int H, int hs, float scale, hipStream_t s);
bool mmt_attn_bwd_fuses_qkv2(const AttnBatch& b, int T, int hs);
hipError_t mmt_attn_bwd_dkdv_ring64(const AttnBatch& b, int B, int T, int H, float scale, bool drop, int variant,
                                    hipStream_t s);
hipError_t mmt_attn_bwd_dq_ring64(const AttnBatch& b, int B, int T, int H, float scale, bool drop, hipStream_t s);
hipError_t mmt_attn_fwd_ring64(const AttnBatch& b, int B, int T, int H, float scale, bool drop, hipStream_t s);
hipError_t mmt_attn_bwd_fused64(const AttnBatch& b, int B, int T, int H, float scale, bool drop, hipStream_t s);
hipError_t mmt_launch_attn_mask(const AttnBatch& b, int B, int T, int H, hipStream_t s);

struct DecodeAttnProblem {
  const bf16_t* q; int q_ld;
  const bf16_t* k[MMT_MAX_STREAMS];
  const bf16_t* v[MMT_MAX_STREAMS];
  int kv_ld, kv_hstride;
  bf16_t* o; int o_ld;
  int nstreams;
};
struct DecodeAttnBatch { DecodeAttnProblem p[MMT_MAX_GROUP]; int count; };
hipError_t mmt_launch_attn_decode(const DecodeAttnBatch& b, int B, int t, int T, int H, int hs, float scale,
                                  hipStream_t s);

struct Qkv2Problem {
  const bf16_t* h1;
  const float* w2;
  bf16_t* out;
  const bf16_t* dout;
  bf16_t* dh1;
  float* dw2;
  float* db1;
};
struct Qkv2Batch { Qkv2Problem p[MMT_MAX_GROUP]; int count; DetScratch det; };
hipError_t mmt_launch_qkv2_fwd(const Qkv2Batch& b, int R, int nblk, int hs, int ld_h1, int ld_out, hipStream_t s);
hipError_t mmt_launch_qkv2_bwd(const Qkv2Batch& b, int R, int nblk, int hs, int ld_h1, int ld_out, hipStream_t s);

struct EmbProblem {
  const int64_t* idx;
  const float* tok;
  const float* pos;
  float* x;
// ... 81 lines not shown
```

### trade-aid-multimodal-transformer_amd/csrc/mmt_ops.hip

```cpp
#include <hip/hip_runtime.h>

#include "mmt.h"
#include "mmt_kernels.h"

static int st(hipError_t e) { return e == hipSuccess ? MMT_OK : MMT_ERR_HIP; }

extern "C" {

int mmt_op_gemm(void* stream, int32_t a_kc, int32_t b_kc, int32_t epi, int32_t splits, int32_t M, int32_t N,
                int32_t K, const void* A, int32_t lda, const void* B, int32_t ldb, const float* bias, const void* aux,
                int32_t ldaux, const float* resid, int32_t ldres, float* o32, int32_t ldc, void* o16, int32_t ldo16,
                float alpha) {
  if (epi < 0 || epi >= EPI_COUNT || M < 0 || N < 0 || K < 0) return MMT_ERR_INVALID;
  if ((lda & 7) || (ldb & 7)) return MMT_ERR_INVALID;
  GemmBatch b{};
  b.count = 1;
  GemmProblem& p = b.p[0];
  p.A = (const bf16_t*)A; p.lda = lda; p.B = (const bf16_t*)B; p.ldb = ldb; p.bias = bias;
  p.aux = (const bf16_t*)aux; p.ldaux = ldaux; p.resid = resid; p.ldres = ldres; p.o32 = o32; p.ldc = ldc;
  p.o16 = (bf16_t*)o16; p.ldo16 = ldo16; p.alpha = alpha; p.M = M; p.N = N; p.K = K;
  const hipError_t e = mmt_launch_gemm(b, a_kc != 0, b_kc != 0, epi, splits, (hipStream_t)stream);
  if (e == hipErrorInvalidValue) return MMT_ERR_UNSUPPORTED;
  return st(e);
}
// ... 134 lines not shown
                         int32_t dout_ld, float* const* dvec, void* dq, int32_t dq_ld, void* const* dk, void* const* dv,
                         int32_t dkv_ld, int32_t dkv_hstride) {
  return mmt_op_attention_bwd_ws(stream, B, T, H, hs, nstreams, q, q_ld, k, v, kv_ld, kv_hstride, o, o_ld, oj, lse, dout,
                                 dout_ld, dvec, dq, dq_ld, dk, dv, dkv_ld, dkv_hstride, nullptr, 0);
}

int mmt_op_attention_bwd_ws(void* stream, int32_t B, int32_t T, int32_t H, int32_t hs, int32_t nstreams,
                            const void* q, int32_t q_ld, const void* const* k, const void* const* v, int32_t kv_ld,
                            int32_t kv_hstride, const void* o, int32_t o_ld, const void* const* oj,
                            const float* const* lse, const void* dout, int32_t dout_ld, float* const* dvec, void* dq,
                            int32_t dq_ld, void* const* dk, void* const* dv, int32_t dkv_ld, int32_t dkv_hstride,
                            float* dq32, int32_t dq32_ld) {
  if (nstreams < 1 || nstreams > MMT_MAX_STREAMS) return MMT_ERR_INVALID;
  AttnBatch b{};
  b.count = 1;
  AttnProblem& p = b.p[0];
  fill_attn(p, nstreams, q, q_ld, k, v, kv_ld, kv_hstride);
  p.o = (bf16_t*)o; p.o_ld = o_ld;
  for (int j = 0; j < nstreams; ++j) {
    p.oj[j] = oj ? (bf16_t*)oj[j] : nullptr;
    p.lse[j] = (float*)lse[j];
    p.dvec[j] = dvec[j];
    p.dk[j] = (bf16_t*)dk[j];
    p.dv[j] = (bf16_t*)dv[j];
  }
  p.dout = (const bf16_t*)dout; p.dout_ld = dout_ld; p.dq = (bf16_t*)dq; p.dq_ld = dq_ld;
  p.dkv_ld = dkv_ld; p.dkv_hstride = dkv_hstride;
  p.dq32 = dq32; p.dq32_ld = dq32_ld;
  const float scale = 1.0f / __builtin_sqrtf((float)hs);
  const hipError_t e = mmt_launch_attn_bwd(b, B, T, H, hs, scale, (hipStream_t)stream);
  return e == hipErrorInvalidValue ? MMT_ERR_UNSUPPORTED : st(e);
}

int mmt_op_qkv2_fwd(void* stream, int32_t R, int32_t nblk, int32_t hs, const void* h1, int32_t ld_h1, const float* w2,
                    void* out, int32_t ld_out) {
  Qkv2Batch b{};
  b.count = 1;
  b.p[0].h1 = (const bf16_t*)h1; b.p[0].w2 = w2; b.p[0].out = (bf16_t*)out;
  const hipError_t e = mmt_launch_qkv2_fwd(b, R, nblk, hs, ld_h1, ld_out, (hipStream_t)stream);
  return e == hipErrorInvalidValue ? MMT_ERR_UNSUPPORTED : st(e);
}

int mmt_op_qkv2_bwd(void* stream, int32_t R, int32_t nblk, int32_t hs, const void* h1, int32_t ld_h1, const float* w2,
                    const void* dout, int32_t ld_out, void* dh1, float* dw2) {
  Qkv2Batch b{};
  b.count = 1;
  b.p[0].h1 = (const bf16_t*)h1; b.p[0].w2 = w2; b.p[0].dout = (const bf16_t*)dout; b.p[0].dh1 = (bf16_t*)dh1;
  b.p[0].dw2 = dw2;
  const hipError_t e = mmt_launch_qkv2_bwd(b, R, nblk, hs, ld_h1, ld_out, (hipStream_t)stream);
  return e == hipErrorInvalidValue ? MMT_ERR_UNSUPPORTED : st(e);
}

int mmt_op_colsum(void* stream, int32_t R, int32_t N, const void* x, int32_t ld, float* out, float alpha) {
  ColsumBatch b{};
  b.count = 1;
  b.p[0].x = (const bf16_t*)x; b.p[0].ld = ld; b.p[0].out = out; b.p[0].N = N; b.p[0].alpha = alpha;
  return st(mmt_launch_colsum(b, R, (hipStream_t)stream));
}

int mmt_op_ordered_sum(void* stream, int32_t nparts, int32_t n, const float* parts, int64_t ld, float* dst) {
  if (nparts < 1 || n < 0 || ld < n || !parts || !dst) return MMT_ERR_INVALID;
  DetSumBatch b{};
  b.count = 1;
  b.s[0].dst = dst; b.s[0].parts = parts; b.s[0].ld = ld; b.s[0].nparts = nparts; b.s[0].n = n;
  return st(mmt_launch_ordered_sum(b, (hipStream_t)stream));
}
// ... 74 lines not shown
```

### trade-aid-multimodal-transformer_amd/csrc/mmt_qkv2.hip

```cpp

#include <cstdlib>
#include <type_traits>

#include "mmt_common.h"
#include "mmt_kernels.h"

template <int N>
__device__ __forceinline__ void ld4_guarded(const bf16_t* p, int valid, uint32_t& w0, uint32_t& w1) {
  if (valid >= 4) {
    const u32x2 v = *reinterpret_cast<const u32x2*>(p);
    w0 = v[0]; w1 = v[1];
  } else {
    uint16_t e[4];
#pragma unroll
    for (int t = 0; t < 4; ++t) e[t] = t < valid ? p[t] : (uint16_t)0;
    w0 = e[0] | ((uint32_t)e[1] << 16);
    w1 = e[2] | ((uint32_t)e[3] << 16);
  }
}

constexpr int qkv2_strips(int hs) { return hs >= 48 ? 4 : 1; }
template <int HS>
__global__ __launch_bounds__(256) void qkv2_fwd_mfma(Qkv2Batch batch, int R, int ld_h1, int ld_out) {
  constexpr int HH = HS / 2;
  constexpr int NOT = (HS + 31) / 32;
  constexpr int KS = (HH + 15) / 16;
  constexpr int SHW = KS * 16 + 8;
  constexpr int SOW = HS + 8;
  constexpr int BR = 128 * qkv2_strips(HS);
  const Qkv2Problem& P = batch.p[blockIdx.z];
  const int tile = xcd_tile(blockIdx.x, gridDim.x);
  const int nblk = gridDim.x / ((R + BR - 1) / BR);
  const int blk = tile % nblk, rb = tile / nblk;
  const int tid = threadIdx.x, lane = tid & 63, w = tid >> 6;
  const int r = lane & 31, h = lane >> 5;
  __shared__ __attribute__((aligned(16))) bf16_t sh[128 * SHW];
  __shared__ __attribute__((aligned(16))) bf16_t so[128 * SOW];
  constexpr int HPC = HH / 4, PPC = (KS * 16 - HH) / 4;
  constexpr int NL = (128 * HPC + 255) / 256;
  u32x2 hv[NL];
  auto load = [&](int r0) {
#pragma unroll
    for (int u = 0; u < NL; ++u) {
      const int c = tid + 256 * u, row = c / HPC, col = (c % HPC) * 4;
      hv[u] = u32x2{0u, 0u};
      if (c < 128 * HPC && r0 + row < R)
        hv[u] = *reinterpret_cast<const u32x2*>(P.h1 + (int64_t)(r0 + row) * ld_h1 + blk * HH + col);
    }
  };
  if (PPC > 0)
    for (int c = tid; c < 128 * PPC; c += 256) {
      const int row = c / PPC, col = HH + (c % PPC) * 4;
      *reinterpret_cast<u32x2*>(sh + row * SHW + col) = u32x2{0u, 0u};
    }
  const float* w2 = P.w2 + (int64_t)blk * HS * HH;
  bf16x8 wa[NOT][KS];
#pragma unroll
  for (int ot = 0; ot < NOT; ++ot)
#pragma unroll
    for (int s = 0; s < KS; ++s)
#pragma unroll
      for (int j = 0; j < 8; ++j) {
        const int o = ot * 32 + r, i = 16 * s + 8 * h + j;
        wa[ot][s][j] = (__bf16)((o < HS && i < HH) ? w2[o * HH + i] : 0.f);
      }
  const int lr = w * 32;
  const int rend = min(R, rb * BR + BR);
  load(rb * BR);
  for (int r0 = rb * BR; r0 < rend; r0 += 128) {
    if (r0 > rb * BR) __syncthreads();
#pragma unroll
    for (int u = 0; u < NL; ++u) {
      const int c = tid + 256 * u;
      if (c < 128 * HPC) *reinterpret_cast<u32x2*>(sh + (c / HPC) * SHW + (c % HPC) * 4) = hv[u];
    }
    __syncthreads();
    if (r0 + 128 < rend) load(r0 + 128);
#pragma unroll
    for (int ot = 0; ot < NOT; ++ot) {
      f32x16 acc;
#pragma unroll
      for (int e = 0; e < 16; ++e) acc[e] = 0.f;
#pragma unroll
      for (int s = 0; s < KS; ++s) {
        const bf16x8 hb = *reinterpret_cast<const bf16x8*>(sh + (lr + r) * SHW + 16 * s + 8 * h);
        acc = mfma32(wa[ot][s], hb, acc);
      }
#pragma unroll
      for (int g = 0; g < 4; ++g) {
        const int o0 = ot * 32 + 8 * g + 4 * h;
        if (o0 < HS)
          *reinterpret_cast<u32x2*>(so + (lr + r) * SOW + o0) =
              u32x2{pack2bf(acc[4 * g], acc[4 * g + 1]), pack2bf(acc[4 * g + 2], acc[4 * g + 3])};
      }
    }
    __syncthreads();
    constexpr int OPC = HS / 8;
    for (int c = tid; c < 128 * OPC; c += 256) {
      const int row = c / OPC, col = (c % OPC) * 8;
      if (r0 + row < R)
        *reinterpret_cast<u32x4*>(P.out + (int64_t)(r0 + row) * ld_out + blk * HS + col) =
            *reinterpret_cast<const u32x4*>(so + row * SOW + col);
    }
  }
}

__device__ __forceinline__ bf16x8 tr_rows(const bf16_t* img, int ld, int kb, int cb, int lane) {
  const int g = lane >> 4, i = lane & 15;
  const int q = i >> 2, p = i & 3;
  const int col = cb + 16 * (g & 1) + 4 * p;
  const int kr = kb + 8 * (g >> 1) + q;
  return join4(lds_tr16(img + kr * ld + col), lds_tr16(img + (kr + 4) * ld + col));
}

#ifndef QKV2_BWD_ROWS
#define QKV2_BWD_ROWS 2048
#endif
template <int HS>
// ... 422 lines not shown
```

### trade-aid-multimodal-transformer_amd/mmt_build.py

```python
import concurrent.futures as cf
import os
import subprocess
import sys

HERE = os.path.dirname(os.path.abspath(__file__))
REPO = os.path.dirname(HERE)
CSRC = os.path.join(HERE, "csrc")
OBJ = os.path.join(CSRC, "build")
LIB = os.path.join(HERE, "libmmt_hip.so")
HIPCC = os.environ.get("HIPCC", "/opt/rocm/bin/hipcc")
SOURCES = ["mmt_gemm.hip", "mmt_gemm8.hip", "mmt_mlp2.hip", "mmt_attn.hip", "mmt_attn2.hip", "mmt_elem.hip", "mmt_stats.hip", "mmt_qkv2.hip", "mmt_engine.hip", "mmt_ops.hip", "mmt_batch.hip", "mmt_decode.hip"]
FLAGS = ["--offload-arch=gfx950", "-O3", "-std=c++17", "-fPIC", "-I" + os.path.join(REPO, "include"), "-I" + CSRC,
         "-Wall", "-Wno-unused-function", "-Wno-unused-variable", "-Wno-unused-result"]

VGPR_FORM = ["-mllvm", "-amdgpu-mfma-vgpr-form=1"]
FILE_FLAGS = {"mmt_attn.hip": ["-fno-slp-vectorize"] + VGPR_FORM, "mmt_attn2.hip": ["-fno-slp-vectorize"],
              "mmt_qkv2.hip": VGPR_FORM}


def _deps_mtime():
    hdrs = [os.path.join(CSRC, f) for f in os.listdir(CSRC) if f.endswith(".h")]
    hdrs.append(os.path.join(REPO, "include", "mmt.h"))
    return max(os.path.getmtime(h) for h in hdrs)


def _compile(src, force):
    s = os.path.join(CSRC, src)
    o = os.path.join(OBJ, src.replace(".hip", ".o"))
    if not force and os.path.exists(o) and os.path.getmtime(o) >= max(os.path.getmtime(s), _deps_mtime()):
        return o
    cmd = [HIPCC] + FLAGS + FILE_FLAGS.get(src, []) + ["-c", s, "-o", o]
    r = subprocess.run(cmd, capture_output=True, text=True)
    if r.returncode != 0:
        raise RuntimeError(f"hipcc failed for {src}:\n{r.stderr}")
    return o


def build(force=False, verbose=True):
    os.makedirs(OBJ, exist_ok=True)
    with cf.ThreadPoolExecutor(max_workers=min(len(SOURCES), 8)) as ex:
        objs = list(ex.map(lambda s: _compile(s, force), SOURCES))
    if force or not os.path.exists(LIB) or os.path.getmtime(LIB) < max(os.path.getmtime(o) for o in objs):
        tmp = LIB + ".tmp"
        cmd = [HIPCC, "--offload-arch=gfx950", "-shared", "-fPIC", "-o", tmp] + objs
        r = subprocess.run(cmd, capture_output=True, text=True)
        if r.returncode != 0:
            raise RuntimeError(f"link failed:\n{r.stderr}")
        os.replace(tmp, LIB)
    if verbose:
# ... 7 lines not shown
```

### trade-aid-multimodal-transformer_amd/mmt_lib.py

```python
import ctypes
import os

import torch

HERE = os.path.dirname(os.path.abspath(__file__))
LIB_PATH = os.environ.get("MMT_LIB_PATH") or os.path.join(HERE, "libmmt_hip.so")
MAX_MOD = 8

c_i32 = ctypes.c_int32
c_i64 = ctypes.c_int64
c_f32 = ctypes.c_float
c_vp = ctypes.c_void_p
c_cp = ctypes.c_char_p


class MmtConfig(ctypes.Structure):
    _fields_ = [
        ("num_modalities", c_i32),
        ("n_embd", c_i32),
        ("n_head", c_i32),
        ("n_layer", c_i32),
        ("block_size", c_i32),
        ("vocab_sizes", c_i32 * MAX_MOD),
        ("cross_attention", c_i32 * MAX_MOD),
# ... 79 lines not shown
    "mmt_stats_chunk": (c_i64, []),
    "mmt_stats_record_bytes": (c_i64, [c_i32]),
    "mmt_stats_scratch_bytes": (c_i64, [c_i64, c_i32]),
    "mmt_tensor_stats": (c_i32, [c_vp, c_vp, c_i64, c_vp, c_i32, c_i32, c_vp, c_vp, c_vp]),
    "mmt_set_grad_accumulate": (c_i32, [c_vp, c_i32]),
    "mmt_get_grad_accumulate": (c_i32, [c_vp]),
    "mmt_eval_direction": (c_i32, [c_vp, c_vp, c_i32, c_i32, c_i32, c_vp, c_vp, c_vp, c_vp, c_i32, c_vp, c_vp]),
    "mmt_set_dropout_seed": (c_i32, [c_vp, ctypes.c_uint64]),
    "mmt_probe_set": (c_i32, [c_vp, c_cp]),
    "mmt_probe_read": (c_i32, [c_vp, ctypes.POINTER(ctypes.c_double), ctypes.POINTER(c_i64)]),
    "mmt_probe_enable": (c_i32, [c_vp, c_i32]),
    "mmt_set_side_stream": (c_i32, [c_vp, c_i32]),
    "mmt_set_deterministic": (c_i32, [c_vp, c_i32]),
    "mmt_get_deterministic": (c_i32, [c_vp]),
    "mmt_probe_count": (c_i32, [c_vp]),
    "mmt_probe_read_at": (c_i32, [c_vp, c_i32, ctypes.POINTER(ctypes.c_double), ctypes.POINTER(c_i64),
                                  ctypes.POINTER(ctypes.c_double), ctypes.POINTER(ctypes.c_double)]),
    "mmt_batch_jitter":(c_i32, [c_vp, c_vp, c_i64, c_i32, c_i32, ctypes.c_uint64, ctypes.c_uint64]),
    "mmt_batch_indices": (c_i32, [c_vp, c_i32, c_vp, c_vp, c_i32, c_i32, ctypes.c_uint64, ctypes.c_uint64, c_vp]),
    "mmt_batch_gather": (c_i32, [c_vp, c_i32, ctypes.POINTER(c_vp), c_vp, c_i32, c_i32, ctypes.POINTER(c_vp),
                                 ctypes.POINTER(c_vp)]),
    "mmt_exact_words_bytes": (c_i64, [c_i64]),
    "mmt_exact_walk_scratch_bytes": (c_i64, [c_i64, c_i64]),
    "mmt_exact_gen": (c_i32, [c_vp, c_vp, c_vp, c_i64]),
    "mmt_exact_walk": (c_i32, [c_vp, c_i32, ctypes.POINTER(c_vp), ctypes.POINTER(c_i64), ctypes.POINTER(c_i32),
                               ctypes.POINTER(c_i32), c_vp, c_vp, c_i64, c_vp, c_i64, c_vp]),
    "mmt_attn_set_ring": (c_i32, [ctypes.c_int]),
    "mmt_attn_set_mask_g": (c_i32, [ctypes.c_int]),
    "mmt_gemm_set_t2": (c_i32, [ctypes.c_int]),
    "mmt_emb_set_sort": (c_i32, [ctypes.c_int]),
    "mmt_set_relu_bits": (c_i32, [ctypes.c_int]),
    "mmt_set_drop_copy_fuse": (c_i32, [ctypes.c_int]),
    "mmt_set_attn_qkv2": (c_i32, [ctypes.c_int]),
    "mmt_mlp2_set_bm": (c_i32, [ctypes.c_int]),
    "mmt_qkv2_set_coal": (c_i32, [ctypes.c_int]),
    "mmt_gemm_set_variant": (c_i32, [ctypes.c_int]),
    "mmt_op_gemm": (c_i32, [c_vp, c_i32, c_i32, c_i32, c_i32, c_i32, c_i32, c_i32, c_vp, c_i32, c_vp, c_i32, c_vp,
                            c_vp, c_i32, c_vp, c_i32, c_vp, c_i32, c_vp, c_i32, c_f32]),
    "mmt_op_gemm_qkv": (c_i32, [c_vp, c_i32, c_i32, c_i32, c_vp, c_i32, c_vp, c_i32, c_vp, c_vp, c_i32, c_vp, c_i32,
                                c_vp, c_i32]),
    "mmt_op_gemm_wgrad": (c_i32, [c_vp, c_i32, c_i32, c_i32, c_vp, c_i32, c_vp, c_i32, c_vp, c_i32, c_f32, c_vp, c_i64]),
    "mmt_op_gemm_ln_bwd": (c_i32, [c_vp, c_i32, c_i32, c_i32, c_vp, c_i32, c_vp, c_i32, c_f32, c_vp, c_vp, c_vp, c_vp,
                                   c_vp, c_vp, c_vp, c_vp, c_vp, ctypes.c_uint32, ctypes.c_uint32, c_f32]),
    "mmt_op_mlp2": (c_i32, [c_vp, c_i32, c_i32, c_vp, c_i32, c_vp, c_i32, c_vp, c_vp, c_i32, c_vp, c_vp, c_i32, c_vp,
                            c_vp, c_vp, ctypes.c_uint32, ctypes.c_uint32, c_f32, c_vp, c_vp, c_vp, c_vp, c_vp]),
    "mmt_op_mlp2_bwd": (c_i32, [c_vp, c_i32, c_i32, c_vp, c_i32, c_vp, c_i32, c_vp, c_i32, c_f32, c_vp, c_i32, c_vp,
                                c_i32, c_vp, c_vp]),
    "mmt_op_layernorm_fwd": (c_i32, [c_vp, c_i32, c_i32, c_vp, c_vp, c_vp, c_vp, c_vp, c_vp]),
    "mmt_op_layernorm_bwd": (c_i32, [c_vp, c_i32, c_i32, c_vp, c_vp, c_vp, c_vp, c_vp, c_vp, c_vp, c_vp, c_vp]),
    "mmt_op_attention_fwd": (c_i32, [c_vp, c_i32, c_i32, c_i32, c_i32, c_i32, c_vp, c_i32, ctypes.POINTER(c_vp),
                                     ctypes.POINTER(c_vp), c_i32, c_i32, c_vp, c_i32, ctypes.POINTER(c_vp),
                                     ctypes.POINTER(c_vp)]),
    "mmt_op_attention_bwd": (c_i32, [c_vp, c_i32, c_i32, c_i32, c_i32, c_i32, c_vp, c_i32, ctypes.POINTER(c_vp),
                                     ctypes.POINTER(c_vp), c_i32, c_i32, c_vp, c_i32, ctypes.POINTER(c_vp),
                                     ctypes.POINTER(c_vp), c_vp, c_i32, ctypes.POINTER(c_vp), c_vp, c_i32,
                                     ctypes.POINTER(c_vp), ctypes.POINTER(c_vp), c_i32, c_i32]),
    "mmt_op_attention_bwd_ws": (c_i32, [c_vp, c_i32, c_i32, c_i32, c_i32, c_i32, c_vp, c_i32, ctypes.POINTER(c_vp),
                                        ctypes.POINTER(c_vp), c_i32, c_i32, c_vp, c_i32, ctypes.POINTER(c_vp),
                                        ctypes.POINTER(c_vp), c_vp, c_i32, ctypes.POINTER(c_vp), c_vp, c_i32,
                                        ctypes.POINTER(c_vp), ctypes.POINTER(c_vp), c_i32, c_i32, c_vp, c_i32]),
    "mmt_op_qkv2_fwd": (c_i32, [c_vp, c_i32, c_i32, c_i32, c_vp, c_i32, c_vp, c_vp, c_i32]),
    "mmt_op_qkv2_bwd": (c_i32, [c_vp, c_i32, c_i32, c_i32, c_vp, c_i32, c_vp, c_vp, c_i32, c_vp, c_vp]),
    "mmt_op_colsum": (c_i32, [c_vp, c_i32, c_i32, c_vp, c_i32, c_vp, c_f32]),
    "mmt_op_ordered_sum": (c_i32, [c_vp, c_i32, c_i32, c_vp, c_i64, c_vp]),
    "mmt_op_cross_entropy": (c_i32, [c_vp, c_i32, c_i32, c_vp, c_vp, c_vp, c_i32, c_vp]),
    "mmt_op_embedding_fwd": (c_i32, [c_vp, c_i32, c_i32, c_i32, c_i32, c_vp, c_vp, c_vp, c_vp]),
    "mmt_op_embedding_bwd": (c_i32, [c_vp, c_i32, c_i32, c_i32, c_i32, c_vp, c_vp, c_vp, c_vp]),
    "mmt_op_embedding_bwd_ws": (c_i32, [c_vp, c_i32, c_i32, c_i32, c_i32, c_vp, c_vp, c_vp, c_vp, c_vp]),
    "mmt_op_mx_quant": (c_i32, [c_vp, c_i32, c_i32, c_vp, c_i32, c_vp, c_i32, c_vp, c_i32]),
    "mmt_op_gemm_f8": (c_i32, [c_vp, c_i32, c_i32, c_i32, c_i32, c_vp, c_i32, c_vp, c_i32, c_vp, c_i32, c_vp, c_i32,
                               c_vp, c_vp, c_i32, c_vp, c_i32, c_vp, c_i32, c_vp, c_i32, c_vp, c_i32]),
    "mmt_op_layernorm_fwd_f8": (c_i32, [c_vp, c_i32, c_i32, c_vp, c_vp, c_vp, c_vp, c_vp, c_vp, c_vp, c_i32, c_vp,
                                        c_i32]),
}

EXPORTED = sorted(_SIGS)
_lib = None


def lib():
    global _lib
    if _lib is not None:
        return _lib
    if not os.path.exists(LIB_PATH):
        raise RuntimeError(
            f"libmmt_hip.so not found at {LIB_PATH}: build it with "
            f"`python trade-aid-multimodal-transformer_amd/mmt_build.py` (there is no CPU fallback)")
    L = ctypes.CDLL(LIB_PATH)
    for name, (res, args) in _SIGS.items():
        if os.environ.get("MMT_LIB_PATH") and not hasattr(L, name):
            continue
        fn = getattr(L, name)
        fn.restype = res
# ... 30 lines not shown
```

Baseline: 8.261 million tokens/s.

## Compute Q/K/V on-chip from h1 inside attention kernels instead of materializing

Adds an on-chip path where the attention forward and fused stage-2 backward kernels recompute K, V and Q tiles from the first-stage hidden activations h1 and the small w2 weights using MFMA, instead of reading a materialized Q/K/V buffer written by the qkv2 kernel. The GEMM epilogue gains an h1-only mode so the qkv2 output need not be stored. Device helpers are moved into a shared header, a new oc kernel file is added, and a runtime bit switch controls the path. The aim is to cut HBM traffic and a kernel launch per layer, at the cost of redundant recompute and extra register pressure.

New measurement: 8.446 million tokens/s (median of 6 runs). 2.2% higher.

```diff
diff --git a/include/mmt.h b/include/mmt.h
--- a/include/mmt.h
+++ b/include/mmt.h
@@ -182,6 +182,11 @@
                             const float* const* lse, const void* dout, int32_t dout_ld, float* const* dvec, void* dq,
                             int32_t dq_ld, void* const* dk, void* const* dv, int32_t dkv_ld, int32_t dkv_hstride,
                             float* dq32, int32_t dq32_ld);
+int mmt_op_attention_fwd_h1(void* stream, int32_t B, int32_t T, int32_t H, const void* h1, int32_t ld_h1,
+                            const float* w2, void* o, int32_t o_ld, float* lse);
+int mmt_op_attention_bwd_h1(void* stream, int32_t B, int32_t T, int32_t H, const void* h1, int32_t ld_h1,
+                            const float* w2, const void* o, int32_t o_ld, const float* lse, const void* dout,
+                            int32_t dout_ld, void* dh1, float* dw2, float* db1);
 int mmt_op_qkv2_fwd(void* stream, int32_t R, int32_t nblk, int32_t hs, const void* h1, int32_t ld_h1,
                     const float* w2, void* out, int32_t ld_out);
 int mmt_op_qkv2_bwd(void* stream, int32_t R, int32_t nblk, int32_t hs, const void* h1, int32_t ld_h1,
@@ -201,6 +206,7 @@
 int mmt_set_relu_bits(int on);
 int mmt_set_drop_copy_fuse(int on);
 int mmt_set_attn_qkv2(int on);
+int mmt_set_attn_qkv_onchip(int bits);
 int mmt_mlp2_set_bm(int bm);
 
 int mmt_op_mx_quant(void* stream, int32_t rows, int32_t cols, const float* src, int32_t ld_src, void* dst8,
diff --git a/trade-aid-multimodal-transformer_amd/csrc/mmt_attn.hip b/trade-aid-multimodal-transformer_amd/csrc/mmt_attn.hip
--- a/trade-aid-multimodal-transformer_amd/csrc/mmt_attn.hip
+++ b/trade-aid-multimodal-transformer_amd/csrc/mmt_attn.hip
@@ -7,283 +7,7 @@
 #include "mmt_common.h"
 #include "mmt_kernels.h"
 
-namespace {
-
-__device__ __forceinline__ bf16x8 zero8() {
-  const u32x4 z = {0u, 0u, 0u, 0u};
-  return __builtin_bit_cast(bf16x8, z);
-}
-
-__device__ __forceinline__ bf16x8 ld8(const bf16_t* p, bool ok) {
-  if (!ok) return zero8();
-  return *reinterpret_cast<const bf16x8*>(p);
-}
-
-template <int HS>
-struct Geo {
-  static constexpr int NKS = (HS + 15) / 16;
-  static constexpr int ND = (HS + 31) / 32;
-  static constexpr int W = ND * 32;
-  static constexpr int RW = W + 8;
-  static constexpr int TW = (W == 64) ? 96 : W;
-  static constexpr int CH = HS / 8;
-};
-
-__device__ __forceinline__ u32x4 tile_chunk(const bf16_t* base, int64_t rowbase, int r0, int row, int col, int T,
-                                            int ld) {
-  u32x4 v = {0u, 0u, 0u, 0u};
-  if (r0 + row < T) v = *reinterpret_cast<const u32x4*>(base + (rowbase + r0 + row) * ld + col);
-  return v;
-}
-
-__device__ __forceinline__ bf16x8 tr_frag(const bf16_t* lds, int stride, int dt, int s, int lane) {
-  const int g = lane >> 4, i = lane & 15;
-  const int q = i >> 2, p = i & 3;
-  const int col = dt * 32 + 16 * (g & 1) + 4 * p;
-  const int kb = 16 * s + 4 * (g >> 1) + q;
-  return join4(lds_tr16(lds + kb * stride + col), lds_tr16(lds + (kb + 8) * stride + col));
-}
-
-constexpr int SL_SUB = 1152, SL_SLICE = 2 * SL_SUB;
-template <int HS>
-struct SliceImg {
-  static constexpr bool on = HS == 32;
-};
-__device__ __forceinline__ int sl_off(int row, int chunk) {
-  return (row >> 5) * SL_SLICE + (chunk >> 1) * SL_SUB + (row & 31) * 32 + (((chunk & 1) ^ ((row >> 3) & 1)) << 4);
-}
-__device__ __forceinline__ bf16x8 sl_row(const bf16_t* img, int row0, int r, int s, int h) {
-  const int o = (row0 >> 5) * SL_SLICE + s * SL_SUB + r * 32 + ((h ^ ((r >> 3) & 1)) << 4);
-  return *reinterpret_cast<const bf16x8*>(reinterpret_cast<const char*>(img) + o);
-}
-__device__ __forceinline__ bf16x8 sl_tr(const bf16_t* img, int row0, int s, int lane) {
-  const int g = lane >> 4, q = (lane >> 2) & 3, p = lane & 3;
-  const int L = (g & 1) * SL_SUB + (p & 1) * 8 + (4 * (g >> 1) + q) * 32;
-  const char* b = reinterpret_cast<const char*>(img) + (row0 >> 5) * SL_SLICE + 512 * s;
-  return join4(lds_tr16(b + L + ((p >> 1) << 4)), lds_tr16(b + L + 256 + (((p >> 1) ^ 1) << 4)));
-}
-
-__device__ __forceinline__ bf16x8 acc_frag(const f32x16& a, int s) {
-  const u32x4 v = {pack2bf(a[8 * s], a[8 * s + 1]), pack2bf(a[8 * s + 2], a[8 * s + 3]),
-                   pack2bf(a[8 * s + 4], a[8 * s + 5]), pack2bf(a[8 * s + 6], a[8 * s + 7])};
-  return __builtin_bit_cast(bf16x8, v);
-}
-
-__device__ __forceinline__ void zero16(f32x16& a) {
-#pragma unroll
-  for (int e = 0; e < 16; ++e) a[e] = 0.f;
-}
-
-__device__ __forceinline__ float keep_f(float v, int m) { return __int_as_float(__float_as_int(v) & m); }
-
-__device__ __forceinline__ int key_dword(int r) { return 2 * ((r & 3) + 4 * (r >> 3)) + ((r >> 2) & 1); }
-
-}
-
-template <int HS>
-struct Chunk {
-  static constexpr int ROWS = (HS <= 32) ? 256 : 128;
-  static constexpr int HALF = ROWS * Geo<HS>::CH;
-  static constexpr int NSTG = 2 * HALF / 256;
-};
-
-template <int HS>
-struct Stager {
-  u32x4 v[Chunk<HS>::NSTG];
-  __device__ __forceinline__ void load(const bf16_t* a, int lda, const bf16_t* b, int ldb, int64_t rowbase, int r0,
-                                       int T, int tid) {
-    constexpr int CH = Geo<HS>::CH, HALF = Chunk<HS>::HALF;
-#pragma unroll
-    for (int u = 0; u < Chunk<HS>::NSTG; ++u) {
-      const int c = tid + 256 * u;
-      const bool isb = c >= HALF;
-      const int cc = isb ? c - HALF : c;
-      v[u] = tile_chunk(isb ? b : a, rowbase, r0, cc / CH, (cc % CH) * 8, T, isb ? ldb : lda);
-    }
-  }
-  __device__ __forceinline__ void store_a(bf16_t* la, int sa, int tid) const {
-    constexpr int CH = Geo<HS>::CH, HALF = Chunk<HS>::HALF;
-#pragma unroll
-    for (int u = 0; u < Chunk<HS>::NSTG; ++u) {
-      const int c = tid + 256 * u;
-      if (c < HALF) *reinterpret_cast<u32x4*>(la + (c / CH) * sa + (c % CH) * 8) = v[u];
-    }
-  }
-  __device__ __forceinline__ void store(bf16_t* la, int sa, bf16_t* lb, int sb, int tid) const {
-    constexpr int CH = Geo<HS>::CH, HALF = Chunk<HS>::HALF;
-#pragma unroll
-    for (int u = 0; u < Chunk<HS>::NSTG; ++u) {
-      const int c = tid + 256 * u;
-      const bool isb = c >= HALF;
-      const int cc = isb ? c - HALF : c;
-      const int row = cc / CH, col = (cc % CH) * 8;
-      *reinterpret_cast<u32x4*>(isb ? lb + row * sb + col : la + row * sa + col) = v[u];
-    }
-  }
-  __device__ __forceinline__ void store_slices(bf16_t* la, bf16_t* lb, int tid) const {
-    constexpr int CH = Geo<HS>::CH, HALF = Chunk<HS>::HALF;
-    static_assert(CH == 4, "slice images hold 32 columns");
-#pragma unroll
-    for (int u = 0; u < Chunk<HS>::NSTG; ++u) {
-      const int c = tid + 256 * u;
-      const bool isb = c >= HALF;
-      const int cc = isb ? c - HALF : c;
-      *reinterpret_cast<u32x4*>(reinterpret_cast<char*>(isb ? lb : la) + sl_off(cc / CH, cc % CH)) = v[u];
-    }
-  }
-};
-
-template <int HS, int KT_ = Chunk<HS>::ROWS / 32>
-struct MaskStager {
-  static constexpr int KT = KT_;
-  static constexpr int N4 = 8 * KT * 8;
-  static constexpr int PER = (N4 + 255) / 256;
-  static constexpr int DWORDS = 8 * KT * 32;
-  u32x4 v[PER];
-  __device__ __forceinline__ void load(const uint32_t* base, int bh, int nt, int b0, int c0, bool blk_q, int tid) {
-    const int64_t ntri = (int64_t)nt * (nt + 1) / 2;
-#pragma unroll
-    for (int u = 0; u < PER; ++u) {
-      const int c = tid + 256 * u;
-      v[u] = u32x4{0u, 0u, 0u, 0u};
-      if (N4 % 256 == 0 || c < N4) {
-        const int i = c / (KT * 8), k = (c / 8) % KT, p = c % 8;
-        const int qt = blk_q ? b0 + i : c0 + k, kt = blk_q ? c0 + k : b0 + i;
-        if (qt < nt && kt <= qt)
-          v[u] = *reinterpret_cast<const u32x4*>(base + ((int64_t)bh * ntri + qt * (qt + 1) / 2 + kt) * 32 + p * 4);
-      }
-    }
-  }
-  __device__ __forceinline__ void store(uint32_t* lds, int tid) const {
-#pragma unroll
-    for (int u = 0; u < PER; ++u) {
-      const int c = tid + 256 * u;
-      if (N4 % 256 == 0 || c < N4) *reinterpret_cast<u32x4*>(lds + 4 * c) = v[u];
-    }
-  }
-};
-
-__device__ __forceinline__ float ex2(float x) { return __builtin_amdgcn_exp2f(x); }
-
-
-constexpr float kLog2e = 1.4426950408889634f;
-constexpr float kTau = 8.0f;
-
-#ifndef MMT_FWD_MINB
-#define MMT_FWD_MINB(hs) 2
-#endif
-#ifndef MMT_DQ_MINB
-#define MMT_DQ_MINB(hs) 2
-#endif
-#ifndef MMT_DKDV1_MINB
-#define MMT_DKDV1_MINB(hs) ((hs) <= 32 ? 1 : 2)
-#endif
-
-__device__ __forceinline__ float xhalf_max(float v) {
-  const auto r = __builtin_amdgcn_permlane32_swap(__float_as_uint(v), __float_as_uint(v), false, false);
-  float m;
-  asm("v_max_f32 %0, %1, %2" : "=v"(m) : "v"(__uint_as_float(r[0])), "v"(__uint_as_float(r[1])));
-  return m;
-}
-__device__ __forceinline__ float xhalf_sum(float v) {
-  const auto r = __builtin_amdgcn_permlane32_swap(__float_as_uint(v), __float_as_uint(v), false, false);
-  return __uint_as_float(r[0]) + __uint_as_float(r[1]);
-}
-
-typedef short s16x2 __attribute__((ext_vector_type(2)));
-__device__ __forceinline__ uint32_t keep_spread(uint32_t w16) { return __builtin_amdgcn_perm(0u, w16, 0x0c010c00u); }
-__device__ __forceinline__ uint32_t pair_keep(uint32_t w32, int i) {
-  s16x2 v = __builtin_bit_cast(s16x2, w32 << (15 - i));
-  v = v >> (s16x2){15, 15};
-  return __builtin_bit_cast(uint32_t, v);
-}
-__device__ __forceinline__ int elem_keep(uint32_t w16, int e) {
-  return __builtin_amdgcn_sbfe((int)w16, (e & 1) * 8 + (e >> 1), 1);
-}
-
-__device__ __forceinline__ bf16x8 acc_frag_keep(const f32x16& a, int s, uint32_t w32) {
-  const u32x4 v = {pack2bf(a[8 * s], a[8 * s + 1]) & pair_keep(w32, 4 * s),
-                   pack2bf(a[8 * s + 2], a[8 * s + 3]) & pair_keep(w32, 4 * s + 1),
-                   pack2bf(a[8 * s + 4], a[8 * s + 5]) & pair_keep(w32, 4 * s + 2),
-                   pack2bf(a[8 * s + 6], a[8 * s + 7]) & pair_keep(w32, 4 * s + 3)};
-  return __builtin_bit_cast(bf16x8, v);
-}
-
-template <int HS>
-struct FwdQ {
-  bf16x8 qf[Geo<HS>::NKS];
-  f32x16 o[Geo<HS>::ND];
-  float m, l;
-  int tq;
-};
-
-template <int HS, bool diag>
-__device__ __forceinline__ void fwd_softmax(f32x16& sacc, FwdQ<HS>& q, int k0, float c2, int h) {
-  using G = Geo<HS>;
-  float tmax = -INFINITY;
-  if (diag) {
-#pragma unroll
-    for (int e = 0; e < 16; ++e) {
-      const int key = k0 + (e & 3) + 8 * (e >> 2) + 4 * h;
-      if (key > q.tq) sacc[e] = -INFINITY;
-    }
-  }
-#pragma unroll
-  for (int e = 0; e < 16; ++e) tmax = fmaxf(tmax, sacc[e]);
-  tmax = xhalf_max(tmax) * c2;
-  const bool up = tmax > q.m + kTau;
-  if (__builtin_amdgcn_ballot_w64(up)) {
-    const float alpha = up ? ex2(q.m - tmax) : 1.f;
-    q.m = up ? tmax : q.m;
-    q.l *= alpha;
-#pragma unroll
-    for (int dt = 0; dt < G::ND; ++dt)
-#pragma unroll
-      for (int e = 0; e < 16; ++e) q.o[dt][e] *= alpha;
-  }
-  const float nm = -q.m;
-#pragma unroll
-  for (int e = 0; e < 16; ++e) sacc[e] = ex2(__builtin_fmaf(sacc[e], c2, nm));
-  float r0 = sacc[0] + sacc[1], r1 = sacc[2] + sacc[3], r2 = sacc[4] + sacc[5], r3 = sacc[6] + sacc[7];
-  r0 += sacc[8] + sacc[9]; r1 += sacc[10] + sacc[11]; r2 += sacc[12] + sacc[13]; r3 += sacc[14] + sacc[15];
-  q.l += (r0 + r1) + (r2 + r3);
-}
-
-template <int HS, int NQ, bool DA, bool DB, bool DROP>
-__device__ __forceinline__ void fwd_step(const bf16_t* ks, const bf16_t* vs, int kl, int k0, FwdQ<HS>& a, FwdQ<HS>& b,
-                                         const uint32_t* mta, const uint32_t* mtb, float c2, int lane) {
-  using G = Geo<HS>;
-  const int r = lane & 31, h = lane >> 5;
-  const uint32_t wa = DROP ? keep_spread(reinterpret_cast<const uint16_t*>(mta)[lane]) : 0u;
-  const uint32_t wb = (DROP && NQ == 2) ? keep_spread(reinterpret_cast<const uint16_t*>(mtb)[lane]) : 0u;
-  f32x16 sa, sb;
-  zero16(sa);
-  if (NQ == 2) zero16(sb);
-#pragma unroll
-  for (int s = 0; s < G::NKS; ++s) {
-    const bf16x8 kf = *reinterpret_cast<const bf16x8*>(ks + (kl + r) * G::RW + 16 * s + 8 * h);
-    sa = mfma32(kf, a.qf[s], sa);
-    if (NQ == 2) sb = mfma32(kf, b.qf[s], sb);
-  }
-  bf16x8 vf[2][G::ND];
-#pragma unroll
-  for (int s = 0; s < 2; ++s)
-#pragma unroll
-    for (int dt = 0; dt < G::ND; ++dt) vf[s][dt] = tr_frag(vs + kl * G::TW, G::TW, dt, s, lane);
-  fwd_softmax<HS, DA>(sa, a, k0, c2, h);
-  if (NQ == 2) fwd_softmax<HS, DB>(sb, b, k0, c2, h);
-#pragma unroll
-  for (int s = 0; s < 2; ++s) {
-    const bf16x8 pa = DROP ? acc_frag_keep(sa, s, wa) : acc_frag(sa, s);
-#pragma unroll
-    for (int dt = 0; dt < G::ND; ++dt) a.o[dt] = mfma32(vf[s][dt], pa, a.o[dt]);
-    if (NQ == 2) {
-      const bf16x8 pb = DROP ? acc_frag_keep(sb, s, wb) : acc_frag(sb, s);
-#pragma unroll
-      for (int dt = 0; dt < G::ND; ++dt) b.o[dt] = mfma32(vf[s][dt], pb, b.o[dt]);
-    }
-  }
-}
+#include "mmt_attn_dev.h"
 
 template <int HS, bool DROP>
 __global__ __launch_bounds__(256, MMT_FWD_MINB(HS)) void attn_fwd_kernel(AttnBatch batch, int T, int H, float scale) {
@@ -963,10 +687,11 @@
 }
 }
 
-template <bool DROP, bool MS, bool Q2, bool DET = false>
+template <bool DROP, bool MS, bool Q2, bool DET = false, bool OC = false>
 __global__ __launch_bounds__(256, 2) void attn_bwd_fused32(AttnBatch batch, int T, int H, float scale) {
   static_assert(!(MS && Q2), "the stage-2 backward follows the self-attention only");
   static_assert(!DET || Q2, "only the stage-2 epilogue has sums to store");
+  static_assert(!OC || Q2, "on-chip Q/K/V goes with the stage-2 backward");
   constexpr int IMG = 8 * SL_SLICE;
   constexpr int OFF_DO = IMG, OFF_TAB = 2 * IMG;
   constexpr int OFF_DS = OFF_TAB + 2048;
@@ -1003,8 +728,21 @@
         mwq[t][q] = P.dmask[j][((int64_t)bh * ntri + q * (q + 1) / 2 + kts[t]) * 32 + key_dword(r)];
     }
   bf16x8 kf[2][2], vf[2][2];
-#pragma unroll
-  for (int t = 0; t < 2; ++t) {
+  bf16x8 ocw[3], och[2][3];
+  if constexpr (OC) {
+#pragma unroll
+    for (int kd = 0; kd < 3; ++kd) {
+      const int blk = kd * H + head;
+      ocw[kd] = oc_w2frag(P.oc_w2, blk, r, h);
+#pragma unroll
+      for (int t = 0; t < 2; ++t) {
+        const int tk = kts[t] * 32 + r;
+        och[t][kd] = oc_hfrag(P.oc_h1 + (rowbase + tk) * P.oc_ld + blk * 16, h, tk < T);
+      }
+    }
+  }
+#pragma unroll
+  for (int t = 0; t < 2 && !OC; ++t) {
     const int tk = kts[t] * 32 + r;
     const bool ok = kts[t] < nt && tk < T;
     const bf16_t* kp = P.k[j] + head * P.kv_hstride + (rowbase + tk) * P.kv_ld;
@@ -1048,11 +786,20 @@
   for (int t = 0; t < 2; ++t) {
 #pragma unroll
     for (int q = 0; q < 8; ++q) asm volatile("" : "+v"(mwq[t][q]));
-#pragma unroll
-    for (int s = 0; s < 2; ++s) {
-      asm volatile("" : "+v"(kf[t][s]));
-      asm volatile("" : "+v"(vf[t][s]));
-    }
+    if constexpr (OC) {
+#pragma unroll
+      for (int kd = 0; kd < 3; ++kd) asm volatile("" : "+v"(och[t][kd]));
+    } else {
+#pragma unroll
+      for (int s = 0; s < 2; ++s) {
+        asm volatile("" : "+v"(kf[t][s]));
+        asm volatile("" : "+v"(vf[t][s]));
+      }
+    }
+  }
+  if constexpr (OC) {
+#pragma unroll
+    for (int kd = 0; kd < 3; ++kd) asm volatile("" : "+v"(ocw[kd]));
   }
 #pragma unroll
   for (int c = 0; c < 4; ++c) {
@@ -1068,7 +815,7 @@
     }
   }
   asm volatile("s_waitcnt vmcnt(0)" ::: "memory");
-  if (j == 0) {
+  if (j == 0 && (!OC || (w & 1))) {
     const int op = w & 1, cb = w >> 1;
     const int ld = op ? P.dout_ld : P.q_ld;
     const ai32x4 rs = a_rsrc((op ? P.dout : P.q) + rowbase * ld + head * 32, (int64_t)T * ld * 2);
@@ -1078,6 +825,21 @@
       const int grow = sl * 32 + prow;
       const int voff = grow < T ? (grow * ld + cb * 16 + pcol) * 2 : A_OOB;
       a_dma16(rs, __builtin_amdgcn_readfirstlane(a_lds_u32(dst + sl * SL_SLICE)), voff);
+    }
+  }
+  if constexpr (OC) {
+#pragma unroll
+    for (int t = 0; t < 2; ++t) {
+      u32x4 x[2];
+      oc_tile(ocw[0], och[t][0], x);
+#pragma unroll
+      for (int s = 0; s < 2; ++s) kf[t][s] = __builtin_bit_cast(bf16x8, x[s]);
+      oc_tile(ocw[2], och[t][2], x);
+#pragma unroll
+      for (int s = 0; s < 2; ++s) vf[t][s] = __builtin_bit_cast(bf16x8, x[s]);
+      oc_tile(ocw[1], och[t][1], x);
+#pragma unroll
+      for (int pr = 0; pr < 2; ++pr) *reinterpret_cast<u32x4*>(lds + sl_off(kts[t] * 32 + r, 2 * pr + h)) = x[pr];
     }
   }
   float* tab = reinterpret_cast<float*>(lds + OFF_TAB);
@@ -1434,6 +1196,11 @@
   return true;
 }
 
+static bool oc_ok(const AttnProblem& P) {
+  return P.oc_h1 && P.oc_w2 && P.nstreams == 1 && !(P.oc_ld & 7) && !((uintptr_t)P.oc_h1 & 15) &&
+         !((uintptr_t)P.oc_w2 & 15);
+}
+
 static bool fused32_ok(const AttnBatch& bt, int T, int ns) {
   if (!(g_attn_ring & 64) || T > 256 || bt.count < 1) return false;
   const bool q2 = bt.p[0].q2_w2 != nullptr;
@@ -1451,6 +1218,8 @@
     if (q2)
       ok = ok && P.q2_h1 && P.q2_dh1 && P.q2_dw2 && P.q2_db1 && !(P.q2_ld & 7) && !((uintptr_t)P.q2_h1 & 15) &&
            !((uintptr_t)P.q2_dh1 & 7);
+    if ((P.oc_w2 != nullptr) != (bt.p[0].oc_w2 != nullptr)) return false;
+    if (P.oc_w2) ok = ok && q2 && oc_ok(P);
   }
   return ok;
 }
@@ -1479,6 +1248,13 @@
     for (int g = 0; g < bt.count; ++g) drop = drop || bt.p[g].drop_thr != 0;
     if (HS == 64 && (g_attn_ring & 8) && ring64_fits(bt, T)) return mmt_attn_fwd_ring64(bt, B, T, H, scale, drop, s);
     const dim3 grid(nb * B * H, 1, bt.count);
+    bool oc = false;
+    for (int g = 0; g < bt.count; ++g) oc = oc || bt.p[g].oc_w2 != nullptr;
+    if (oc) {
+      for (int g = 0; g < bt.count; ++g)
+        if (HS != 32 || T > 256 || !oc_ok(bt.p[g])) return hipErrorInvalidValue;
+      return mmt_attn_fwd_oc32(bt, B, T, H, scale, drop, s);
+    }
     if (drop) hipLaunchKernelGGL((attn_fwd_kernel<HS, true>), grid, dim3(256), 0, s, bt, T, H, scale);
     else hipLaunchKernelGGL((attn_fwd_kernel<HS, false>), grid, dim3(256), 0, s, bt, T, H, scale);
   } else {
@@ -1486,12 +1262,13 @@
     bool drop = false;
     for (int g = 0; g < bt.count; ++g) drop = drop || bt.p[g].drop_thr != 0;
     for (int g = 0; g < bt.count; ++g)
-      if (bt.p[g].q2_w2 && (HS != 32 || !fused32_ok(bt, T, ns))) return hipErrorInvalidValue;
+      if ((bt.p[g].q2_w2 || bt.p[g].oc_w2) && (HS != 32 || !fused32_ok(bt, T, ns))) return hipErrorInvalidValue;
     const bool ring = HS == 64 && ring64_fits(bt, T);
     if (ring && (g_attn_ring & 32) && T <= 512 && ns == 1) return mmt_attn_bwd_fused64(bt, B, T, H, scale, drop, s);
     if (HS == 32 && fused32_ok(bt, T, ns)) {
       const dim3 grid(B * H, 1, bt.count);
       const bool q2 = bt.p[0].q2_w2 != nullptr;
+      const bool oc = bt.p[0].oc_w2 != nullptr;
       if (ns > 1) {
         if (drop) hipLaunchKernelGGL((attn_bwd_fused32<true, true, false>), grid, dim3(256), 0, s, bt, T, H, scale);
         else hipLaunchKernelGGL((attn_bwd_fused32<false, true, false>), grid, dim3(256), 0, s, bt, T, H, scale);
@@ -1501,7 +1278,9 @@
         DetLaunch L;
         hipError_t e = L.begin(d.det, d.count, d.det.stride, s);
         if (e != hipSuccess) return e;
-        if (drop) hipLaunchKernelGGL((attn_bwd_fused32<true, false, true, true>), grid, dim3(256), 0, s, d, T, H, scale);
+        if (oc && drop) hipLaunchKernelGGL((attn_bwd_fused32<true, false, true, true, true>), grid, dim3(256), 0, s, d, T, H, scale);
+        else if (oc) hipLaunchKernelGGL((attn_bwd_fused32<false, false, true, true, true>), grid, dim3(256), 0, s, d, T, H, scale);
+        else if (drop) hipLaunchKernelGGL((attn_bwd_fused32<true, false, true, true>), grid, dim3(256), 0, s, d, T, H, scale);
         else hipLaunchKernelGGL((attn_bwd_fused32<false, false, true, true>), grid, dim3(256), 0, s, d, T, H, scale);
         e = hipGetLastError();
         if (e != hipSuccess) return e;
@@ -1511,7 +1290,9 @@
         }
         return L.finish();
       } else if (q2) {
-        if (drop) hipLaunchKernelGGL((attn_bwd_fused32<true, false, true>), grid, dim3(256), 0, s, bt, T, H, scale);
+        if (oc && drop) hipLaunchKernelGGL((attn_bwd_fused32<true, false, true, false, true>), grid, dim3(256), 0, s, bt, T, H, scale);
+        else if (oc) hipLaunchKernelGGL((attn_bwd_fused32<false, false, true, false, true>), grid, dim3(256), 0, s, bt, T, H, scale);
+        else if (drop) hipLaunchKernelGGL((attn_bwd_fused32<true, false, true>), grid, dim3(256), 0, s, bt, T, H, scale);
         else hipLaunchKernelGGL((attn_bwd_fused32<false, false, true>), grid, dim3(256), 0, s, bt, T, H, scale);
       } else {
         if (drop) hipLaunchKernelGGL((attn_bwd_fused32<true, false, false>), grid, dim3(256), 0, s, bt, T, H, scale);
diff --git a/trade-aid-multimodal-transformer_amd/csrc/mmt_attn_dev.h b/trade-aid-multimodal-transformer_amd/csrc/mmt_attn_dev.h
--- /dev/null
+++ b/trade-aid-multimodal-transformer_amd/csrc/mmt_attn_dev.h
@@ -0,0 +1,318 @@
+#pragma once
+#include <stdlib.h>
+
+#include <algorithm>
+
+#include <type_traits>
+
+#include "mmt_common.h"
+#include "mmt_kernels.h"
+
+namespace {
+
+__device__ __forceinline__ bf16x8 zero8() {
+  const u32x4 z = {0u, 0u, 0u, 0u};
+  return __builtin_bit_cast(bf16x8, z);
+}
+
+__device__ __forceinline__ bf16x8 ld8(const bf16_t* p, bool ok) {
+  if (!ok) return zero8();
+  return *reinterpret_cast<const bf16x8*>(p);
+}
+
+template <int HS>
+struct Geo {
+  static constexpr int NKS = (HS + 15) / 16;
+  static constexpr int ND = (HS + 31) / 32;
+  static constexpr int W = ND * 32;
+  static constexpr int RW = W + 8;
+  static constexpr int TW = (W == 64) ? 96 : W;
+  static constexpr int CH = HS / 8;
+};
+
+__device__ __forceinline__ u32x4 tile_chunk(const bf16_t* base, int64_t rowbase, int r0, int row, int col, int T,
+                                            int ld) {
+  u32x4 v = {0u, 0u, 0u, 0u};
+  if (r0 + row < T) v = *reinterpret_cast<const u32x4*>(base + (rowbase + r0 + row) * ld + col);
+  return v;
+}
+
+__device__ __forceinline__ bf16x8 tr_frag(const bf16_t* lds, int stride, int dt, int s, int lane) {
+  const int g = lane >> 4, i = lane & 15;
+  const int q = i >> 2, p = i & 3;
+  const int col = dt * 32 + 16 * (g & 1) + 4 * p;
+  const int kb = 16 * s + 4 * (g >> 1) + q;
+  return join4(lds_tr16(lds + kb * stride + col), lds_tr16(lds + (kb + 8) * stride + col));
+}
+
+constexpr int SL_SUB = 1152, SL_SLICE = 2 * SL_SUB;
+template <int HS>
+struct SliceImg {
+  static constexpr bool on = HS == 32;
+};
+__device__ __forceinline__ int sl_off(int row, int chunk) {
+  return (row >> 5) * SL_SLICE + (chunk >> 1) * SL_SUB + (row & 31) * 32 + (((chunk & 1) ^ ((row >> 3) & 1)) << 4);
+}
+__device__ __forceinline__ bf16x8 sl_row(const bf16_t* img, int row0, int r, int s, int h) {
+  const int o = (row0 >> 5) * SL_SLICE + s * SL_SUB + r * 32 + ((h ^ ((r >> 3) & 1)) << 4);
+  return *reinterpret_cast<const bf16x8*>(reinterpret_cast<const char*>(img) + o);
+}
+__device__ __forceinline__ bf16x8 sl_tr(const bf16_t* img, int row0, int s, int lane) {
+  const int g = lane >> 4, q = (lane >> 2) & 3, p = lane & 3;
+  const int L = (g & 1) * SL_SUB + (p & 1) * 8 + (4 * (g >> 1) + q) * 32;
+  const char* b = reinterpret_cast<const char*>(img) + (row0 >> 5) * SL_SLICE + 512 * s;
+  return join4(lds_tr16(b + L + ((p >> 1) << 4)), lds_tr16(b + L + 256 + (((p >> 1) ^ 1) << 4)));
+}
+
+__device__ __forceinline__ bf16x8 acc_frag(const f32x16& a, int s) {
+  const u32x4 v = {pack2bf(a[8 * s], a[8 * s + 1]), pack2bf(a[8 * s + 2], a[8 * s + 3]),
+                   pack2bf(a[8 * s + 4], a[8 * s + 5]), pack2bf(a[8 * s + 6], a[8 * s + 7])};
+  return __builtin_bit_cast(bf16x8, v);
+}
+
+__device__ __forceinline__ void zero16(f32x16& a) {
+#pragma unroll
+  for (int e = 0; e < 16; ++e) a[e] = 0.f;
+}
+
+__device__ __forceinline__ float keep_f(float v, int m) { return __int_as_float(__float_as_int(v) & m); }
+
+__device__ __forceinline__ int key_dword(int r) { return 2 * ((r & 3) + 4 * (r >> 3)) + ((r >> 2) & 1); }
+
+__device__ __forceinline__ bf16x8 oc_w2frag(const float* w2, int blk, int r, int h) {
+  const float* w = w2 + ((int64_t)blk * 32 + r) * 16 + 4 * h;
+  const f32x4 lo = *reinterpret_cast<const f32x4*>(w);
+  const f32x4 hi = *reinterpret_cast<const f32x4*>(w + 8);
+  return __builtin_bit_cast(bf16x8, u32x4{pack2bf(lo[0], lo[1]), pack2bf(lo[2], lo[3]), pack2bf(hi[0], hi[1]),
+                                          pack2bf(hi[2], hi[3])});
+}
+__device__ __forceinline__ bf16x8 oc_hfrag(const bf16_t* p, int h, bool ok) {
+  u32x2 a = {0u, 0u}, b = {0u, 0u};
+  if (ok) {
+    a = *reinterpret_cast<const u32x2*>(p + 4 * h);
+    b = *reinterpret_cast<const u32x2*>(p + 8 + 4 * h);
+  }
+  return __builtin_bit_cast(bf16x8, u32x4{a[0], a[1], b[0], b[1]});
+}
+__device__ __forceinline__ void oc_tile(bf16x8 w2f, bf16x8 hf, u32x4 (&out)[2]) {
+  f32x16 z;
+#pragma unroll
+  for (int e = 0; e < 16; ++e) z[e] = 0.f;
+  const f32x16 d = mfma32(w2f, hf, z);
+#pragma unroll
+  for (int pr = 0; pr < 2; ++pr) {
+    const int ga = 2 * pr, gb = 2 * pr + 1;
+    const auto s0 = __builtin_amdgcn_permlane32_swap(pack2bf(d[4 * ga], d[4 * ga + 1]), pack2bf(d[4 * gb], d[4 * gb + 1]),
+                                                     false, false);
+    const auto s1 = __builtin_amdgcn_permlane32_swap(pack2bf(d[4 * ga + 2], d[4 * ga + 3]),
+                                                     pack2bf(d[4 * gb + 2], d[4 * gb + 3]), false, false);
+    out[pr] = u32x4{s0[0], s1[0], s0[1], s1[1]};
+  }
+}
+
+}
+
+template <int HS>
+struct Chunk {
+  static constexpr int ROWS = (HS <= 32) ? 256 : 128;
+  static constexpr int HALF = ROWS * Geo<HS>::CH;
+  static constexpr int NSTG = 2 * HALF / 256;
+};
+
+template <int HS>
+struct Stager {
+  u32x4 v[Chunk<HS>::NSTG];
+  __device__ __forceinline__ void load(const bf16_t* a, int lda, const bf16_t* b, int ldb, int64_t rowbase, int r0,
+                                       int T, int tid) {
+    constexpr int CH = Geo<HS>::CH, HALF = Chunk<HS>::HALF;
+#pragma unroll
+    for (int u = 0; u < Chunk<HS>::NSTG; ++u) {
+      const int c = tid + 256 * u;
+      const bool isb = c >= HALF;
+      const int cc = isb ? c - HALF : c;
+      v[u] = tile_chunk(isb ? b : a, rowbase, r0, cc / CH, (cc % CH) * 8, T, isb ? ldb : lda);
+    }
+  }
+  __device__ __forceinline__ void store_a(bf16_t* la, int sa, int tid) const {
+    constexpr int CH = Geo<HS>::CH, HALF = Chunk<HS>::HALF;
+#pragma unroll
+    for (int u = 0; u < Chunk<HS>::NSTG; ++u) {
+      const int c = tid + 256 * u;
+      if (c < HALF) *reinterpret_cast<u32x4*>(la + (c / CH) * sa + (c % CH) * 8) = v[u];
+    }
+  }
+  __device__ __forceinline__ void store(bf16_t* la, int sa, bf16_t* lb, int sb, int tid) const {
+    constexpr int CH = Geo<HS>::CH, HALF = Chunk<HS>::HALF;
+#pragma unroll
+    for (int u = 0; u < Chunk<HS>::NSTG; ++u) {
+      const int c = tid + 256 * u;
+      const bool isb = c >= HALF;
+      const int cc = isb ? c - HALF : c;
+      const int row = cc / CH, col = (cc % CH) * 8;
+      *reinterpret_cast<u32x4*>(isb ? lb + row * sb + col : la + row * sa + col) = v[u];
+    }
+  }
+  __device__ __forceinline__ void store_slices(bf16_t* la, bf16_t* lb, int tid) const {
+    constexpr int CH = Geo<HS>::CH, HALF = Chunk<HS>::HALF;
+    static_assert(CH == 4, "slice images hold 32 columns");
+#pragma unroll
+    for (int u = 0; u < Chunk<HS>::NSTG; ++u) {
+      const int c = tid + 256 * u;
+      const bool isb = c >= HALF;
+      const int cc = isb ? c - HALF : c;
+      *reinterpret_cast<u32x4*>(reinterpret_cast<char*>(isb ? lb : la) + sl_off(cc / CH, cc % CH)) = v[u];
+    }
+  }
+};
+
+template <int HS, int KT_ = Chunk<HS>::ROWS / 32>
+struct MaskStager {
+  static constexpr int KT = KT_;
+  static constexpr int N4 = 8 * KT * 8;
+  static constexpr int PER = (N4 + 255) / 256;
+  static constexpr int DWORDS = 8 * KT * 32;
+  u32x4 v[PER];
+  __device__ __forceinline__ void load(const uint32_t* base, int bh, int nt, int b0, int c0, bool blk_q, int tid) {
+    const int64_t ntri = (int64_t)nt * (nt + 1) / 2;
+#pragma unroll
+    for (int u = 0; u < PER; ++u) {
+      const int c = tid + 256 * u;
+      v[u] = u32x4{0u, 0u, 0u, 0u};
+      if (N4 % 256 == 0 || c < N4) {
+        const int i = c / (KT * 8), k = (c / 8) % KT, p = c % 8;
+        const int qt = blk_q ? b0 + i : c0 + k, kt = blk_q ? c0 + k : b0 + i;
+        if (qt < nt && kt <= qt)
+          v[u] = *reinterpret_cast<const u32x4*>(base + ((int64_t)bh * ntri + qt * (qt + 1) / 2 + kt) * 32 + p * 4);
+      }
+    }
+  }
+  __device__ __forceinline__ void store(uint32_t* lds, int tid) const {
+#pragma unroll
+    for (int u = 0; u < PER; ++u) {
+      const int c = tid + 256 * u;
+      if (N4 % 256 == 0 || c < N4) *reinterpret_cast<u32x4*>(lds + 4 * c) = v[u];
+    }
+  }
+};
+
+__device__ __forceinline__ float ex2(float x) { return __builtin_amdgcn_exp2f(x); }
+
+
+constexpr float kLog2e = 1.4426950408889634f;
+constexpr float kTau = 8.0f;
+
+#ifndef MMT_FWD_MINB
+#define MMT_FWD_MINB(hs) 2
+#endif
+#ifndef MMT_DQ_MINB
+#define MMT_DQ_MINB(hs) 2
+#endif
+#ifndef MMT_DKDV1_MINB
+#define MMT_DKDV1_MINB(hs) ((hs) <= 32 ? 1 : 2)
+#endif
+
+__device__ __forceinline__ float xhalf_max(float v) {
+  const auto r = __builtin_amdgcn_permlane32_swap(__float_as_uint(v), __float_as_uint(v), false, false);
+  float m;
+  asm("v_max_f32 %0, %1, %2" : "=v"(m) : "v"(__uint_as_float(r[0])), "v"(__uint_as_float(r[1])));
+  return m;
+}
+__device__ __forceinline__ float xhalf_sum(float v) {
+  const auto r = __builtin_amdgcn_permlane32_swap(__float_as_uint(v), __float_as_uint(v), false, false);
+  return __uint_as_float(r[0]) + __uint_as_float(r[1]);
+}
+
+typedef short s16x2 __attribute__((ext_vector_type(2)));
+__device__ __forceinline__ uint32_t keep_spread(uint32_t w16) { return __builtin_amdgcn_perm(0u, w16, 0x0c010c00u); }
+__device__ __forceinline__ uint32_t pair_keep(uint32_t w32, int i) {
+  s16x2 v = __builtin_bit_cast(s16x2, w32 << (15 - i));
+  v = v >> (s16x2){15, 15};
+  return __builtin_bit_cast(uint32_t, v);
+}
+__device__ __forceinline__ int elem_keep(uint32_t w16, int e) {
+  return __builtin_amdgcn_sbfe((int)w16, (e & 1) * 8 + (e >> 1), 1);
+}
+
+__device__ __forceinline__ bf16x8 acc_frag_keep(const f32x16& a, int s, uint32_t w32) {
+  const u32x4 v = {pack2bf(a[8 * s], a[8 * s + 1]) & pair_keep(w32, 4 * s),
+                   pack2bf(a[8 * s + 2], a[8 * s + 3]) & pair_keep(w32, 4 * s + 1),
+                   pack2bf(a[8 * s + 4], a[8 * s + 5]) & pair_keep(w32, 4 * s + 2),
+                   pack2bf(a[8 * s + 6], a[8 * s + 7]) & pair_keep(w32, 4 * s + 3)};
+  return __builtin_bit_cast(bf16x8, v);
+}
+
+template <int HS>
+struct FwdQ {
+  bf16x8 qf[Geo<HS>::NKS];
+  f32x16 o[Geo<HS>::ND];
+  float m, l;
+  int tq;
+};
+
+template <int HS, bool diag>
+__device__ __forceinline__ void fwd_softmax(f32x16& sacc, FwdQ<HS>& q, int k0, float c2, int h) {
+  using G = Geo<HS>;
+  float tmax = -INFINITY;
+  if (diag) {
+#pragma unroll
+    for (int e = 0; e < 16; ++e) {
+      const int key = k0 + (e & 3) + 8 * (e >> 2) + 4 * h;
+      if (key > q.tq) sacc[e] = -INFINITY;
+    }
+  }
+#pragma unroll
+  for (int e = 0; e < 16; ++e) tmax = fmaxf(tmax, sacc[e]);
+  tmax = xhalf_max(tmax) * c2;
+  const bool up = tmax > q.m + kTau;
+  if (__builtin_amdgcn_ballot_w64(up)) {
+    const float alpha = up ? ex2(q.m - tmax) : 1.f;
+    q.m = up ? tmax : q.m;
+    q.l *= alpha;
+#pragma unroll
+    for (int dt = 0; dt < G::ND; ++dt)
+#pragma unroll
+      for (int e = 0; e < 16; ++e) q.o[dt][e] *= alpha;
+  }
+  const float nm = -q.m;
+#pragma unroll
+  for (int e = 0; e < 16; ++e) sacc[e] = ex2(__builtin_fmaf(sacc[e], c2, nm));
+  float r0 = sacc[0] + sacc[1], r1 = sacc[2] + sacc[3], r2 = sacc[4] + sacc[5], r3 = sacc[6] + sacc[7];
+  r0 += sacc[8] + sacc[9]; r1 += sacc[10] + sacc[11]; r2 += sacc[12] + sacc[13]; r3 += sacc[14] + sacc[15];
+  q.l += (r0 + r1) + (r2 + r3);
+}
+
+template <int HS, int NQ, bool DA, bool DB, bool DROP>
+__device__ __forceinline__ void fwd_step(const bf16_t* ks, const bf16_t* vs, int kl, int k0, FwdQ<HS>& a, FwdQ<HS>& b,
+                                         const uint32_t* mta, const uint32_t* mtb, float c2, int lane) {
+  using G = Geo<HS>;
+  const int r = lane & 31, h = lane >> 5;
+  const uint32_t wa = DROP ? keep_spread(reinterpret_cast<const uint16_t*>(mta)[lane]) : 0u;
+  const uint32_t wb = (DROP && NQ == 2) ? keep_spread(reinterpret_cast<const uint16_t*>(mtb)[lane]) : 0u;
+  f32x16 sa, sb;
+  zero16(sa);
+  if (NQ == 2) zero16(sb);
+#pragma unroll
+  for (int s = 0; s < G::NKS; ++s) {
+    const bf16x8 kf = *reinterpret_cast<const bf16x8*>(ks + (kl + r) * G::RW + 16 * s + 8 * h);
+    sa = mfma32(kf, a.qf[s], sa);
+    if (NQ == 2) sb = mfma32(kf, b.qf[s], sb);
+  }
+  bf16x8 vf[2][G::ND];
+#pragma unroll
+  for (int s = 0; s < 2; ++s)
+#pragma unroll
+    for (int dt = 0; dt < G::ND; ++dt) vf[s][dt] = tr_frag(vs + kl * G::TW, G::TW, dt, s, lane);
+  fwd_softmax<HS, DA>(sa, a, k0, c2, h);
+  if (NQ == 2) fwd_softmax<HS, DB>(sb, b, k0, c2, h);
+#pragma unroll
+  for (int s = 0; s < 2; ++s) {
+    const bf16x8 pa = DROP ? acc_frag_keep(sa, s, wa) : acc_frag(sa, s);
+#pragma unroll
+    for (int dt = 0; dt < G::ND; ++dt) a.o[dt] = mfma32(vf[s][dt], pa, a.o[dt]);
+    if (NQ == 2) {
+      const bf16x8 pb = DROP ? acc_frag_keep(sb, s, wb) : acc_frag(sb, s);
+#pragma unroll
+      for (int dt = 0; dt < G::ND; ++dt) b.o[dt] = mfma32(vf[s][dt], pb, b.o[dt]);
+    }
+  }
+}
diff --git a/trade-aid-multimodal-transformer_amd/csrc/mmt_attn_oc.hip b/trade-aid-multimodal-transformer_amd/csrc/mmt_attn_oc.hip
--- /dev/null
+++ b/trade-aid-multimodal-transformer_amd/csrc/mmt_attn_oc.hip
@@ -0,0 +1,115 @@
+#include "mmt_attn_dev.h"
+
+template <bool DROP>
+__global__ __launch_bounds__(256, MMT_FWD_MINB(32)) void attn_fwd_oc32_kernel(AttnBatch batch, int T, int H, float scale) {
+  constexpr int HS = 32;
+  using G = Geo<HS>;
+  constexpr int ROWS = Chunk<HS>::ROWS;
+  constexpr int MKT = ROWS / 32;
+  constexpr int MDW = 8 * MKT * 32;
+  const AttnProblem& P = batch.p[blockIdx.z];
+  const int bh = xcd_tile(blockIdx.x, gridDim.x), b = bh / H, head = bh % H;
+  const int tid = threadIdx.x, lane = tid & 63, w = __builtin_amdgcn_readfirstlane(tid >> 6);
+  const int r = lane & 31, h = lane >> 5;
+  const int nt = (T + 31) / 32;
+  const int64_t rowbase = (int64_t)b * T;
+  const float c2 = scale * kLog2e;
+  __shared__ __attribute__((aligned(16))) bf16_t ks[ROWS * G::RW];
+  __shared__ __attribute__((aligned(16))) bf16_t vs[ROWS * G::TW];
+  using MS = MaskStager<HS>;
+  __shared__ __attribute__((aligned(16))) uint32_t msk[DROP ? MDW : 4];
+  const int64_t lw_off = (int64_t)gridDim.x * (nt * (nt + 1) / 2) * 32;
+  MS mst;
+  const int qa = w, qb = 7 - w;
+  const bool la = qa < nt, lb = qb < nt;
+  FwdQ<HS> A, Bq;
+  A.tq = qa * 32 + r;
+  Bq.tq = qb * 32 + r;
+  {
+    bf16x8 wf[3], hf[2][3];
+#pragma unroll
+    for (int kd = 0; kd < 3; ++kd) {
+      const int blk = kd * H + head;
+      wf[kd] = oc_w2frag(P.oc_w2, blk, r, h);
+      hf[0][kd] = oc_hfrag(P.oc_h1 + (rowbase + A.tq) * P.oc_ld + blk * 16, h, A.tq < T);
+      hf[1][kd] = oc_hfrag(P.oc_h1 + (rowbase + Bq.tq) * P.oc_ld + blk * 16, h, Bq.tq < T);
+    }
+    if (DROP) mst.load(P.dmask[0] + lw_off, bh, nt, 0, 0, true, tid);
+#pragma unroll
+    for (int t = 0; t < 2; ++t) {
+      const int row = (t ? qb : qa) * 32 + r;
+      u32x4 x[2];
+      oc_tile(wf[0], hf[t][0], x);
+#pragma unroll
+      for (int pr = 0; pr < 2; ++pr) *reinterpret_cast<u32x4*>(ks + row * G::RW + 16 * pr + 8 * h) = x[pr];
+      oc_tile(wf[2], hf[t][2], x);
+#pragma unroll
+      for (int pr = 0; pr < 2; ++pr) *reinterpret_cast<u32x4*>(vs + row * G::TW + 16 * pr + 8 * h) = x[pr];
+      oc_tile(wf[1], hf[t][1], x);
+#pragma unroll
+      for (int pr = 0; pr < 2; ++pr) (t ? Bq : A).qf[pr] = __builtin_bit_cast(bf16x8, x[pr]);
+    }
+    if (DROP) mst.store(msk, tid);
+  }
+  __syncthreads();
+  A.m = -INFINITY; A.l = 0.f; Bq.m = -INFINITY; Bq.l = 0.f;
+  zero16(A.o[0]);
+  zero16(Bq.o[0]);
+  {
+    const uint32_t* mska = msk + (DROP ? w * MKT * 32 : 0);
+    const uint32_t* mskb = msk + (DROP ? (7 - w) * MKT * 32 : 0);
+#define FWD_STEP(NQ, DA, DB, KT) \
+  fwd_step<HS, NQ, DA, DB, DROP>(ks, vs, (KT) * 32, (KT) * 32, A, Bq, mska + (KT) * 32, mskb + (KT) * 32, c2, lane)
+#define FWD_STEP_B(DB, KT) \
+  fwd_step<HS, 1, DB, false, DROP>(ks, vs, (KT) * 32, (KT) * 32, Bq, A, mskb + (KT) * 32, mska, c2, lane)
+    if (lb) {
+      int kt = 0;
+#pragma unroll 1
+      for (; kt <= qa - 1; ++kt) FWD_STEP(2, false, false, kt);
+      FWD_STEP(2, true, false, qa);
+#pragma unroll 1
+      for (kt = qa + 1; kt <= qb - 1; ++kt) FWD_STEP_B(false, kt);
+      FWD_STEP_B(true, qb);
+    } else if (la) {
+#pragma unroll 1
+      for (int kt = 0; kt <= qa - 1; ++kt) FWD_STEP(1, false, false, kt);
+      FWD_STEP(1, true, false, qa);
+    }
+#undef FWD_STEP
+#undef FWD_STEP_B
+  }
+#pragma unroll
+  for (int u = 0; u < 2; ++u) {
+    const bool live = u == 0 ? la : lb;
+    FwdQ<HS>& q = u == 0 ? A : Bq;
+    const float l = xhalf_sum(q.l);
+    const float inv = (l > 0.f) ? (DROP ? P.drop_scale : 1.f) / l : 0.f;
+    u32x4 ov[2];
+#pragma unroll
+    for (int pr = 0; pr < 2; ++pr) {
+      const int ga = 2 * pr, gb = 2 * pr + 1;
+      const uint32_t x0 = pack2bf(q.o[0][4 * ga] * inv, q.o[0][4 * ga + 1] * inv);
+      const uint32_t x1 = pack2bf(q.o[0][4 * ga + 2] * inv, q.o[0][4 * ga + 3] * inv);
+      const uint32_t y0 = pack2bf(q.o[0][4 * gb] * inv, q.o[0][4 * gb + 1] * inv);
+      const uint32_t y1 = pack2bf(q.o[0][4 * gb + 2] * inv, q.o[0][4 * gb + 3] * inv);
+      const auto s0 = __builtin_amdgcn_permlane32_swap(x0, y0, false, false);
+      const auto s1 = __builtin_amdgcn_permlane32_swap(x1, y1, false, false);
+      ov[pr] = u32x4{s0[0], s1[0], s0[1], s1[1]};
+    }
+    if (live && q.tq < T) {
+      if (h == 0) P.lse[0][(int64_t)bh * T + q.tq] = q.m + __log2f(l);
+      bf16_t* dst = P.o + (rowbase + q.tq) * P.o_ld + head * HS;
+#pragma unroll
+      for (int pr = 0; pr < 2; ++pr) *reinterpret_cast<u32x4*>(dst + 16 * pr + 8 * h) = ov[pr];
+    }
+  }
+}
+
+
+hipError_t mmt_attn_fwd_oc32(const AttnBatch& b, int B, int T, int H, float scale, bool drop, hipStream_t s) {
+  if (T > 256 || b.count < 1) return hipErrorInvalidValue;
+  const dim3 grid(B * H, 1, b.count);
+  if (drop) hipLaunchKernelGGL((attn_fwd_oc32_kernel<true>), grid, dim3(256), 0, s, b, T, H, scale);
+  else hipLaunchKernelGGL((attn_fwd_oc32_kernel<false>), grid, dim3(256), 0, s, b, T, H, scale);
+  return hipGetLastError();
+}
diff --git a/trade-aid-multimodal-transformer_amd/csrc/mmt_engine.hip b/trade-aid-multimodal-transformer_amd/csrc/mmt_engine.hip
--- a/trade-aid-multimodal-transformer_amd/csrc/mmt_engine.hip
+++ b/trade-aid-multimodal-transformer_amd/csrc/mmt_engine.hip
@@ -106,6 +106,13 @@
 extern "C" int mmt_set_attn_qkv2(int on) {
   const int old = g_attn_qkv2;
   g_attn_qkv2 = on;
+  return old;
+}
+
+static int g_attn_qkv_onchip = mmt_env_int("MMT_ATTN_QKV_ONCHIP", 3) & 3;
+extern "C" int mmt_set_attn_qkv_onchip(int bits) {
+  const int old = g_attn_qkv_onchip;
+  g_attn_qkv_onchip = bits & 3;
   return old;
 }
 
@@ -170,6 +177,7 @@
   bool det = false;
   bool det_req = false;
   bool grad_accum = false;
+  int onchip_req = 0, onchip = 0;
 };
 
 namespace {
@@ -541,6 +549,10 @@
     if (epi == EPI_BIAS_RELU_BF16 && P.mask8) x += M * N / 8.0;
     if (P.o8) x += M * N * (1.0 + 1.0 / 32.0);
     if (epi == EPI_LN_BWD_F32) x += M * N * 8.0 + (P.o16 ? M * N * 2.0 : 0.0) + M * 8.0;
+    if (P.qkv2_out) {
+      x += M * 2.0 * N * 2.0 + 2.0 * N * P.qkv2_hh * 4.0;
+      *fl += 2.0 * M * 2.0 * N * P.qkv2_hh;
+    }
     *by += x;
   }
 }
@@ -568,6 +580,12 @@
       const double hh = hs / 2;
       x += -rows * C * 2.0 * 3.0 + 2.0 * rows * 3.0 * H * hh * 2.0 + 3.0 * H * hs * hh * 4.0 * 2.0;
       *fl += 2.0 * 2.0 * rows * 3.0 * C * hh;
+    }
+    if (ab.p[g].oc_w2) {
+      const double hh = hs / 2;
+      x -= rows * C * 2.0 * 3.0;
+      if (!bwd) x += rows * 3.0 * H * hh * 2.0 + 3.0 * H * hs * hh * 4.0;
+      *fl += 2.0 * rows * 3.0 * C * hh;
     }
     *by += x;
   }
@@ -918,22 +936,6 @@
       g.p[i].bias = r.P(x[i].b1); g.p[i].o16 = r.W<bf16_t>(a[i].h1); g.p[i].ldo16 = ldh1;
     }
     const bool fuse_qkv2 = qkv2_fuse && (c->hh == 16 || c->hh == 32) && !f8 && !mmt_gemm_wgrad_big(g);
-    for (int i = 0; i < M; ++i) {
-      if (fuse_qkv2) {
-        g.p[i].qkv2_w2 = r.P(x[i].w2); g.p[i].qkv2_out = r.W<bf16_t>(a[i].qkv);
-        g.p[i].qkv2_ld = 3 * C; g.p[i].qkv2_hh = c->hh;
-      }
-    }
-    if (f8) r.gemm8(g, EPI_BIAS_TANH_BF16, "qkv1");
-    else r.gemm(g, true, true, EPI_BIAS_TANH_BF16, 1, "qkv1");
-    for (int i = 0; i < M; ++i) g.p[i].qkv2_out = nullptr;
-    if (!fuse_qkv2) {
-      Qkv2Batch qb{}; qb.count = M;
-      for (int i = 0; i < M; ++i) {
-        qb.p[i].h1 = r.W<bf16_t>(a[i].h1); qb.p[i].w2 = r.P(x[i].w2); qb.p[i].out = r.W<bf16_t>(a[i].qkv);
-      }
-      r.ok(mmt_launch_qkv2_fwd(qb, R, 3 * H, hs, ldh1, 3 * C, r.s), "qkv2_fwd");
-    }
     AttnBatch ab{}; ab.count = M;
     for (int i = 0; i < M; ++i) {
       AttnProblem& q = ab.p[i];
@@ -942,6 +944,35 @@
       q.o = r.W<bf16_t>(a[i].o); q.o_ld = C; q.lse[0] = r.W<float>(a[i].lse); q.nstreams = 1;
       r.set_drop(q, l, i, DS_SA_PROB);
       if (r.drop) q.dmask[0] = r.W<uint32_t>(a[i].dm);
+    }
+    int oc = 0;
+    if (c->onchip_req && fuse_qkv2 && g_attn_qkv2 && mmt_attn_bwd_fuses_qkv2(ab, T, hs) && !(ldh1 & 7)) {
+      oc = c->onchip_req;
+      for (int i = 0; i < M; ++i)
+        if (((uintptr_t)r.W<bf16_t>(a[i].h1) | (uintptr_t)r.P(x[i].w2)) & 15) oc = 0;
+    }
+    if (l == 0) c->onchip = oc;
+    else if (oc != c->onchip) {
+      r.rc = fail(c, MMT_ERR_STATE, "mmt_forward: the layers disagree on the on-chip Q/K/V path");
+      break;
+    }
+    for (int i = 0; i < M; ++i) {
+      if (fuse_qkv2 && oc != 3) {
+        g.p[i].qkv2_w2 = r.P(x[i].w2); g.p[i].qkv2_out = r.W<bf16_t>(a[i].qkv);
+        g.p[i].qkv2_ld = 3 * C; g.p[i].qkv2_hh = c->hh;
+      }
+      if (oc == 3) g.p[i].qkv2_h1_only = 1;
+      if (oc & 1) { ab.p[i].oc_h1 = r.W<bf16_t>(a[i].h1); ab.p[i].oc_ld = ldh1; ab.p[i].oc_w2 = r.P(x[i].w2); }
+    }
+    if (f8) r.gemm8(g, EPI_BIAS_TANH_BF16, "qkv1");
+    else r.gemm(g, true, true, EPI_BIAS_TANH_BF16, 1, "qkv1");
+    for (int i = 0; i < M; ++i) { g.p[i].qkv2_out = nullptr; g.p[i].qkv2_h1_only = 0; }
+    if (!fuse_qkv2) {
+      Qkv2Batch qb{}; qb.count = M;
+      for (int i = 0; i < M; ++i) {
+        qb.p[i].h1 = r.W<bf16_t>(a[i].h1); qb.p[i].w2 = r.P(x[i].w2); qb.p[i].out = r.W<bf16_t>(a[i].qkv);
+      }
+      r.ok(mmt_launch_qkv2_fwd(qb, R, 3 * H, hs, ldh1, 3 * C, r.s), "qkv2_fwd");
     }
     if (r.drop && (l <= 1 || mask_ahead)) {
       r.join();
@@ -1602,7 +1633,11 @@
       AttnProblem& q = ab.p[i];
       q.q2_h1 = r.W<bf16_t>(a[i].h1); q.q2_dh1 = r.W<bf16_t>(p.gh1[par][i]); q.q2_ld = ldh1;
       q.q2_w2 = r.P(x[i].w2); q.q2_dw2 = grads + x[i].w2; q.q2_db1 = grads + x[i].b1;
-    }
+      if (c->onchip & 2) { q.oc_h1 = q.q2_h1; q.oc_ld = ldh1; q.oc_w2 = q.q2_w2; }
+    }
+  if (c->onchip == 3 && !q2)
+    return fail(c, MMT_ERR_STATE, "mmt_backward: the forward kept Q/K/V on chip (mmt_set_attn_qkv_onchip) and the "
+                                  "backward that makes them again (mmt_set_attn_qkv2, mmt_attn_set_ring bit 6) is off");
   Qkv2Batch qb{}; qb.count = M;
   for (int i = 0; i < M; ++i) {
     qb.p[i].h1 = r.W<bf16_t>(a[i].h1); qb.p[i].w2 = r.P(x[i].w2); qb.p[i].dout = r.W<bf16_t>(p.gqkv[i]);
@@ -1801,6 +1836,8 @@
   if (rc) return rc;
   c->side_off = c->side_off_req;
   c->det = c->det_req;
+  c->onchip_req = training ? g_attn_qkv_onchip : 0;
+  c->onchip = 0;
   Runner r{c, (hipStream_t)stream, workspace, params, nullptr, batch, batch * c->T};
   r.drop = training && c->cfg.dropout > 0.f;
   if (r.drop) {
@@ -1828,6 +1865,10 @@
   if (!idx || !params || !logits || !workspace) return fail(c, MMT_ERR_INVALID, "mmt_decode_step: null argument");
   if (c->plan.B != batch || !c->cache_ready)
     return fail(c, MMT_ERR_STATE, "mmt_decode_step: run mmt_forward (prefill) on this batch and workspace first");
+  if (c->onchip == 3)
+    return fail(c, MMT_ERR_INVALID, "mmt_decode_step: the last forward (training != 0) kept the self-attention Q/K/V on "
+                                    "chip (mmt_set_attn_qkv_onchip), so the workspace holds no K/V cache: run the "
+                                    "prefill with training = 0");
   if (c->fwd_drop)
     return fail(c, MMT_ERR_STATE, "mmt_decode_step: the prefill forward sampled dropout (training mode); decode "
                                   "has eval semantics: run the prefill with training = 0");
diff --git a/trade-aid-multimodal-transformer_amd/csrc/mmt_gemm.hip b/trade-aid-multimodal-transformer_amd/csrc/mmt_gemm.hip
--- a/trade-aid-multimodal-transformer_amd/csrc/mmt_gemm.hip
+++ b/trade-aid-multimodal-transformer_amd/csrc/mmt_gemm.hip
@@ -202,7 +202,7 @@
       for (int e = 0; e < 16; ++e) acc[i][j][e] = 0.0f;
   if constexpr (SWAP && EPI == EPI_BIAS_TANH_BF16 && TL::NW == 4 && TL::BN == 128) {
     if (P.qkv2_out) qkv2_stage_w2<TL>(P, lds + LDS_MAIN, n0, tid);
-    if (P.qkv2_out && P.bias) {
+    if ((P.qkv2_out || P.qkv2_h1_only) && P.bias) {
       const float ia = 1.0f / P.alpha;
       const int hh = (tid & 63) >> 5;
 #pragma unroll
@@ -291,6 +291,14 @@
     if (P.qkv2_out) {
       qkv2_fused<TL>(P, acc, lds, lds + LDS_MAIN, alpha, m0, n0, lane, wave);
       epilogue_swap<TL, EPI, EPI_ROWS, true>(P, acc, lds, o32, alpha, m0, n0, tid, lane, wave, det_of(batch, prob));
+    } else if (P.qkv2_h1_only) {
+#pragma unroll
+      for (int i = 0; i < AI; ++i)
+#pragma unroll
+        for (int j = 0; j < AJ; ++j)
+#pragma unroll
+          for (int e = 0; e < 16; ++e) acc[i][j][e] = fast_tanh(alpha * acc[i][j][e]);
+      epilogue_swap<TL, EPI, EPI_ROWS, true>(P, acc, lds, o32, alpha, m0, n0, tid, lane, wave, det_of(batch, prob));
     } else {
       epilogue_swap<TL, EPI, EPI_ROWS>(P, acc, lds, o32, alpha, m0, n0, tid, lane, wave, det_of(batch, prob));
     }
@@ -579,7 +587,7 @@
     const GemmProblem& P = b.p[g];
     if (P.M < TileL::BM || P.N < TileL::BN) return false;
     if (P.K < g_big_kmin && !g_force_big_rt) big = false;
-    qkv2 = qkv2 || P.qkv2_out != nullptr;
+    qkv2 = qkv2 || P.qkv2_out != nullptr || P.qkv2_h1_only;
     tiles += ((P.M + 255) / 256) * ((P.N + 255) / 256);
   }
   if (big) return true;
@@ -590,7 +598,7 @@
 }
 
 static bool qkv2_ok(const GemmProblem& P, int epi, bool fwd) {
-  if (!P.qkv2_out) return true;
+  if (!P.qkv2_out) return !P.qkv2_h1_only || (epi == EPI_BIAS_TANH_BF16 && fwd && !P.alpha_ptr && P.alpha != 0.0f);
   return epi == EPI_BIAS_TANH_BF16 && fwd && (P.qkv2_hh == 16 || P.qkv2_hh == 32) && P.N % P.qkv2_hh == 0 &&
          !P.alpha_ptr && P.alpha != 0.0f &&
          P.qkv2_w2 && !(P.qkv2_ld & 7) && !((uintptr_t)P.qkv2_out & 15) && !((uintptr_t)P.qkv2_w2 & 15);
@@ -661,7 +669,7 @@
   }
   const bool big = use_big(b);
   for (int g = 0; g < b.count; ++g)
-    if (big && b.p[g].qkv2_out) return hipErrorInvalidValue;
+    if (big && (b.p[g].qkv2_out || b.p[g].qkv2_h1_only)) return hipErrorInvalidValue;
   if (a_kc && b_kc) {
     switch (epi) {
       case EPI_STORE_BF16: return launch_t<true, true, true, EPI_STORE_BF16>(b, 1, big, s);
@@ -892,7 +900,7 @@
         (P.lds_b & 3) || (((uintptr_t)P.sa | (uintptr_t)P.sb) & 3) || P.lds_a * 32 < P.K || P.lds_b * 32 < P.K)
       return hipErrorInvalidValue;
     if (P.o8 && ((P.N & 31) || (P.ld8 & 7) || ((uintptr_t)P.o8 & 7))) return hipErrorInvalidValue;
-    if (P.qkv2_out) return hipErrorInvalidValue;
+    if (P.qkv2_out || P.qkv2_h1_only) return hipErrorInvalidValue;
   }
   switch (epi) {
     case EPI_STORE_BF16: return launch_f8_tile<EPI_STORE_BF16>(b, s);
diff --git a/trade-aid-multimodal-transformer_amd/csrc/mmt_kernels.h b/trade-aid-multimodal-transformer_amd/csrc/mmt_kernels.h
--- a/trade-aid-multimodal-transformer_amd/csrc/mmt_kernels.h
+++ b/trade-aid-multimodal-transformer_amd/csrc/mmt_kernels.h
@@ -57,6 +57,7 @@
   const float* qkv2_w2;
   bf16_t* qkv2_out;
   int qkv2_ld, qkv2_hh;
+  int qkv2_h1_only;
   uint8_t* mask8;
   int ldm8;
 };
@@ -144,6 +145,8 @@
   uint32_t drop_key, drop_thr;
   float drop_scale;
   uint32_t* dmask[MMT_MAX_STREAMS];
+  const bf16_t* oc_h1; int oc_ld;
+  const float* oc_w2;
 };
 inline int64_t mmt_attn_mask_tiles(int B, int H, int T) {
   const int64_t nt = (T + 31) / 32;
@@ -162,6 +165,7 @@
                                     hipStream_t s);
 hipError_t mmt_attn_bwd_dq_ring64(const AttnBatch& b, int B, int T, int H, float scale, bool drop, hipStream_t s);
 hipError_t mmt_attn_fwd_ring64(const AttnBatch& b, int B, int T, int H, float scale, bool drop, hipStream_t s);
+hipError_t mmt_attn_fwd_oc32(const AttnBatch& b, int B, int T, int H, float scale, bool drop, hipStream_t s);
 hipError_t mmt_attn_bwd_fused64(const AttnBatch& b, int B, int T, int H, float scale, bool drop, hipStream_t s);
 hipError_t mmt_launch_attn_mask(const AttnBatch& b, int B, int T, int H, hipStream_t s);
 
diff --git a/trade-aid-multimodal-transformer_amd/csrc/mmt_ops.hip b/trade-aid-multimodal-transformer_amd/csrc/mmt_ops.hip
--- a/trade-aid-multimodal-transformer_amd/csrc/mmt_ops.hip
+++ b/trade-aid-multimodal-transformer_amd/csrc/mmt_ops.hip
@@ -190,6 +190,36 @@
   return e == hipErrorInvalidValue ? MMT_ERR_UNSUPPORTED : st(e);
 }
 
+int mmt_op_attention_fwd_h1(void* stream, int32_t B, int32_t T, int32_t H, const void* h1, int32_t ld_h1, const float* w2,
+                            void* o, int32_t o_ld, float* lse) {
+  if (!h1 || !w2 || !o || !lse) return MMT_ERR_INVALID;
+  AttnBatch b{};
+  b.count = 1;
+  AttnProblem& p = b.p[0];
+  p.nstreams = 1;
+  p.oc_h1 = (const bf16_t*)h1; p.oc_ld = ld_h1; p.oc_w2 = w2;
+  p.o = (bf16_t*)o; p.o_ld = o_ld; p.lse[0] = lse;
+  const hipError_t e = mmt_launch_attn_fwd(b, B, T, H, 32, 1.0f / __builtin_sqrtf(32.f), (hipStream_t)stream);
+  return e == hipErrorInvalidValue ? MMT_ERR_UNSUPPORTED : st(e);
+}
+
+int mmt_op_attention_bwd_h1(void* stream, int32_t B, int32_t T, int32_t H, const void* h1, int32_t ld_h1, const float* w2,
+                            const void* o, int32_t o_ld, const float* lse, const void* dout, int32_t dout_ld, void* dh1,
+                            float* dw2, float* db1) {
+  if (!h1 || !w2 || !o || !lse || !dout || !dh1 || !dw2 || !db1) return MMT_ERR_INVALID;
+  AttnBatch b{};
+  b.count = 1;
+  AttnProblem& p = b.p[0];
+  p.nstreams = 1;
+  p.oc_h1 = (const bf16_t*)h1; p.oc_ld = ld_h1; p.oc_w2 = w2;
+  p.q2_h1 = (const bf16_t*)h1; p.q2_ld = ld_h1; p.q2_w2 = w2;
+  p.q2_dh1 = (bf16_t*)dh1; p.q2_dw2 = dw2; p.q2_db1 = db1;
+  p.o = (bf16_t*)o; p.o_ld = o_ld; p.lse[0] = (float*)lse;
+  p.dout = (const bf16_t*)dout; p.dout_ld = dout_ld;
+  const hipError_t e = mmt_launch_attn_bwd(b, B, T, H, 32, 1.0f / __builtin_sqrtf(32.f), (hipStream_t)stream);
+  return e == hipErrorInvalidValue ? MMT_ERR_UNSUPPORTED : st(e);
+}
+
 int mmt_op_qkv2_fwd(void* stream, int32_t R, int32_t nblk, int32_t hs, const void* h1, int32_t ld_h1, const float* w2,
                     void* out, int32_t ld_out) {
   Qkv2Batch b{};
diff --git a/trade-aid-multimodal-transformer_amd/csrc/mmt_qkv2.hip b/trade-aid-multimodal-transformer_amd/csrc/mmt_qkv2.hip
--- a/trade-aid-multimodal-transformer_amd/csrc/mmt_qkv2.hip
+++ b/trade-aid-multimodal-transformer_amd/csrc/mmt_qkv2.hip
@@ -28,6 +28,7 @@
   constexpr int SHW = KS * 16 + 8;
   constexpr int SOW = HS + 8;
   constexpr int BR = 128 * qkv2_strips(HS);
+  constexpr bool PERM = HS == 32;
   const Qkv2Problem& P = batch.p[blockIdx.z];
   const int tile = xcd_tile(blockIdx.x, gridDim.x);
   const int nblk = gridDim.x / ((R + BR - 1) / BR);
@@ -61,7 +62,7 @@
     for (int s = 0; s < KS; ++s)
 #pragma unroll
       for (int j = 0; j < 8; ++j) {
-        const int o = ot * 32 + r, i = 16 * s + 8 * h + j;
+        const int o = ot * 32 + r, i = PERM ? (j < 4 ? 4 * h + j : 8 + 4 * h + j - 4) : 16 * s + 8 * h + j;
         wa[ot][s][j] = (__bf16)((o < HS && i < HH) ? w2[o * HH + i] : 0.f);
       }
   const int lr = w * 32;
@@ -83,7 +84,14 @@
       for (int e = 0; e < 16; ++e) acc[e] = 0.f;
 #pragma unroll
       for (int s = 0; s < KS; ++s) {
-        const bf16x8 hb = *reinterpret_cast<const bf16x8*>(sh + (lr + r) * SHW + 16 * s + 8 * h);
+        bf16x8 hb;
+        if (PERM) {
+          const u32x2 lo = *reinterpret_cast<const u32x2*>(sh + (lr + r) * SHW + 4 * h);
+          const u32x2 hi = *reinterpret_cast<const u32x2*>(sh + (lr + r) * SHW + 8 + 4 * h);
+          hb = __builtin_bit_cast(bf16x8, u32x4{lo[0], lo[1], hi[0], hi[1]});
+        } else {
+          hb = *reinterpret_cast<const bf16x8*>(sh + (lr + r) * SHW + 16 * s + 8 * h);
+        }
         acc = mfma32(wa[ot][s], hb, acc);
       }
 #pragma unroll
diff --git a/trade-aid-multimodal-transformer_amd/mmt_build.py b/trade-aid-multimodal-transformer_amd/mmt_build.py
--- a/trade-aid-multimodal-transformer_amd/mmt_build.py
+++ b/trade-aid-multimodal-transformer_amd/mmt_build.py
@@ -9,12 +9,13 @@
 OBJ = os.path.join(CSRC, "build")
 LIB = os.path.join(HERE, "libmmt_hip.so")
 HIPCC = os.environ.get("HIPCC", "/opt/rocm/bin/hipcc")
-SOURCES = ["mmt_gemm.hip", "mmt_gemm8.hip", "mmt_mlp2.hip", "mmt_attn.hip", "mmt_attn2.hip", "mmt_elem.hip", "mmt_stats.hip", "mmt_qkv2.hip", "mmt_engine.hip", "mmt_ops.hip", "mmt_batch.hip", "mmt_decode.hip"]
+SOURCES = ["mmt_gemm.hip", "mmt_gemm8.hip", "mmt_mlp2.hip", "mmt_attn.hip", "mmt_attn_oc.hip", "mmt_attn2.hip", "mmt_elem.hip", "mmt_stats.hip", "mmt_qkv2.hip", "mmt_engine.hip", "mmt_ops.hip", "mmt_batch.hip", "mmt_decode.hip"]
 FLAGS = ["--offload-arch=gfx950", "-O3", "-std=c++17", "-fPIC", "-I" + os.path.join(REPO, "include"), "-I" + CSRC,
          "-Wall", "-Wno-unused-function", "-Wno-unused-variable", "-Wno-unused-result"]
 
 VGPR_FORM = ["-mllvm", "-amdgpu-mfma-vgpr-form=1"]
-FILE_FLAGS = {"mmt_attn.hip": ["-fno-slp-vectorize"] + VGPR_FORM, "mmt_attn2.hip": ["-fno-slp-vectorize"],
+FILE_FLAGS = {"mmt_attn.hip": ["-fno-slp-vectorize"] + VGPR_FORM, "mmt_attn_oc.hip": ["-fno-slp-vectorize"] + VGPR_FORM,
+              "mmt_attn2.hip": ["-fno-slp-vectorize"],
               "mmt_qkv2.hip": VGPR_FORM}
 
 
diff --git a/trade-aid-multimodal-transformer_amd/mmt_lib.py b/trade-aid-multimodal-transformer_amd/mmt_lib.py
--- a/trade-aid-multimodal-transformer_amd/mmt_lib.py
+++ b/trade-aid-multimodal-transformer_amd/mmt_lib.py
@@ -135,6 +135,7 @@
     "mmt_set_relu_bits": (c_i32, [ctypes.c_int]),
     "mmt_set_drop_copy_fuse": (c_i32, [ctypes.c_int]),
     "mmt_set_attn_qkv2": (c_i32, [ctypes.c_int]),
+    "mmt_set_attn_qkv_onchip": (c_i32, [ctypes.c_int]),
     "mmt_mlp2_set_bm": (c_i32, [ctypes.c_int]),
     "mmt_qkv2_set_coal": (c_i32, [ctypes.c_int]),
     "mmt_gemm_set_variant": (c_i32, [ctypes.c_int]),
@@ -162,6 +163,9 @@
                                         ctypes.POINTER(c_vp), c_i32, c_i32, c_vp, c_i32, ctypes.POINTER(c_vp),
                                         ctypes.POINTER(c_vp), c_vp, c_i32, ctypes.POINTER(c_vp), c_vp, c_i32,
                                         ctypes.POINTER(c_vp), ctypes.POINTER(c_vp), c_i32, c_i32, c_vp, c_i32]),
+    "mmt_op_attention_fwd_h1": (c_i32, [c_vp, c_i32, c_i32, c_i32, c_vp, c_i32, c_vp, c_vp, c_i32, c_vp]),
+    "mmt_op_attention_bwd_h1": (c_i32, [c_vp, c_i32, c_i32, c_i32, c_vp, c_i32, c_vp, c_vp, c_i32, c_vp, c_vp, c_i32,
+                                        c_vp, c_vp, c_vp]),
     "mmt_op_qkv2_fwd": (c_i32, [c_vp, c_i32, c_i32, c_i32, c_vp, c_i32, c_vp, c_vp, c_i32]),
     "mmt_op_qkv2_bwd": (c_i32, [c_vp, c_i32, c_i32, c_i32, c_vp, c_i32, c_vp, c_vp, c_i32, c_vp, c_vp]),
     "mmt_op_colsum": (c_i32, [c_vp, c_i32, c_i32, c_vp, c_i32, c_vp, c_f32]),
```
